# kornelski/cavif-rs

Measured on AMD Instinct MI355X. Metric: MPix/s encoded at speed=4 q=80, 1080p batch; bit-exact vs CPU oracle, higher is better.
Workload: dtype u16 samples / i32 transform / i64 RD cost

## Files before the change

### __graft_entry__.py

```python
import os
import subprocess
import sys

ROOT = os.path.dirname(os.path.abspath(__file__))
sys.path.insert(0, ROOT)

HIPCC_FLAGS = ['--offload-arch=gfx950', '-O2', '-mllvm', '-sink-insts-to-avoid-spills', '-mllvm', '-inline-threshold=1000', '-mllvm', '-disable-machine-licm', '-mllvm', '-phi-node-folding-threshold=1', '-std=c++17', '-ffp-contract=off', '-fPIC', '-shared', '-Wno-unused-variable']


def _digest(sources, flags):
    import hashlib
    h = hashlib.sha256(' '.join(flags).encode())
    for s in sorted(sources):
        with open(s, 'rb') as fh:
            h.update(os.path.basename(s).encode() + b'\0' + fh.read())
    return h.hexdigest()


def _stale(target, sources):
    if not os.path.exists(target):
        return True
    t = os.path.getmtime(target)
    return any(os.path.getmtime(s) > t for s in sources)

# ... 9 lines not shown
        subprocess.check_call([hipcc] + HIPCC_FLAGS + ['-o', out, os.path.join(csrc, 'mi_avif.hip'), '-lz'])
        with open(stamp, 'w') as fh:
            fh.write(want + '\n')
    cli_src = os.path.join(ROOT, 'cavif_rs_amd', 'cli', 'cavif_mi.cpp')
    cli = os.path.join(ROOT, 'cavif_rs_amd', 'cavif_mi')
    if force or _stale(cli, [cli_src, out, os.path.join(ROOT, 'include', 'mi_avif.h')]):
        subprocess.check_call(['g++', '-O2', '-std=c++17', '-o', cli, cli_src, '-L' + os.path.join(ROOT, 'cavif_rs_amd'), '-lmi_avif', '-lpthread', '-Wl,-rpath,$ORIGIN'])
    subprocess.check_call(['make', '-s', '-C', os.path.join(ROOT, 'oracle')])
    try:
        from tests import emu
        emu.build(force=force)
    except Exception as e:
        print('warning: tests/emu build failed (%s); the -m "not gpu" emulator tests will fail, the product library is unaffected' % e, file=sys.stderr)
    try:
        from tests.helpers import k4_harness
        k4_harness.build_all(force=force)
    except Exception as e:
        print('warning: tests/kernels harness build failed (%s); tests/test_k4_coder.py will fail, the product library is unaffected' % e, file=sys.stderr)
    try:
        from tests.helpers import filters_harness
        filters_harness.build_all(force=force)
    except Exception as e:
        print('warning: tests/kernels filter harness build failed (%s); tests/test_loopfilter_kernels.py will fail, the product library is unaffected' % e, file=sys.stderr)
    try:
        from tests.helpers import predict_harness
        predict_harness.build_all(force=force)
    except Exception as e:
        print('warning: tests/kernels prediction harness build failed (%s); tests/test_predict_kernels.py will fail, the product library is unaffected' % e, file=sys.stderr)
    try:
        from tests.helpers import k1_lookups_harness
        k1_lookups_harness.build_all(force=force)
    except Exception as e:
        print('warning: tests/kernels lookup harness build failed (%s); tests/test_k1_lookups.py will fail, the product library is unaffected' % e, file=sys.stderr)
    import cavif_rs_amd
    cavif_rs_amd.load_library()


def smoke():
    import numpy as np
    import cavif_rs_amd as m
    from cavif_rs_amd.synth import synth_image
    from tests.helpers import oracle
    assert m.device_count() >= 1, 'no HIP device visible'
    img = synth_image(256, 192, index=3)
    enc = m.Encoder().with_quality(80).with_speed(4).with_bit_depth(10)
    got = enc.encode_rgb(img)
    ref, cs, _ = oracle.ravif_encode(img, quality=80, speed=4, depth=10)
    assert got.avif_file[4:12] == b'ftypavif'
    assert got.avif_file == ref, 'HIP path and CPU oracle disagree (%d vs %d bytes)' % (len(got.avif_file), len(ref))
    print('smoke ok: %dx%d -> %d bytes (colour %d), identical to the oracle' % (img.shape[1], img.shape[0], len(got.avif_file), got.color_byte_size))


if __name__ == '__main__':
    build(force='--force' in sys.argv)
    if '--smoke' in sys.argv:
        smoke()
```

### cavif_rs_amd/csrc/dev_blk64.h

```cpp
#pragma once

struct Blk64Hbm {
  uint16_t lrec[4][64 * 64]; int32_t lqc[4][32 * 32];
  uint16_t trec[64 * 64]; int32_t tqc[64 * 64];
  uint16_t crec4[4][64 * 64]; int32_t cqc4[4][64 * 64];
  uint16_t crec[2][2][2][64 * 64]; int32_t cqc[2][2][2][4 * 32 * 32];
};
typedef unsigned int v2u_t __attribute__((vector_size(8)));
typedef unsigned int v4u_t __attribute__((vector_size(16)));
#define MI_BLK64_HBM_BYTES ((sizeof(Blk64Hbm) + 255) & ~(size_t)255)

__device__ inline void fwd_txfm64_dev(const LDS uint16_t *src, const LDS uint16_t *pred, LDS int32_t *tbuf, LDS int32_t *coef) {
  constexpr int P = 65;
  {
    const int c = LANE;
    int32_t x[64];
#pragma unroll
    for (int r = 0; r < 64; r++) x[r] = (int)src[r * 64 + c] - (int)pred[r * 64 + c];
    av1_fdct64(x);
#pragma unroll
    for (int r = 0; r < 32; r++) tbuf[r * P + c] = rshift_round_(x[r], 2);
  }
  WAVE_SYNC();
  if (LANE < 32) {
// ... 122 lines not shown
  const int ncand = Tools<TS>::FULL ? 7 : 3;
  auto dl_of = [](int q) { const int a = (q >> 1) + 1; return (q & 1) ? a : -a; };
  const int refine = Tools<TS>::fine_directional(f);
  if (refine) {
#pragma unroll 1
    for (int u = W; u < ncand * 6; u += NW) {
      const int ci = u / 6, q = u - ci * 6, m = SH->order[ci];
      if (m >= V_PRED && m <= D67_PRED) {
        predict_block(f, x, y, log2w, availL, availU, m, dl_of(q), ftype_y, ra, rl, wa, wl, S->etmp, B->pred);
        const long long sd = satd_dev(SH->x64.src64, B->pred, n);
        if (LANE == 0) SH->dsd[ci][q] = sd;
      }
    }
    PH(5);
    WG_SYNC();
    PH(2);
  }
  const bool tx_trial = Tools<TS>::tx_mode_select(f) && Tools<TS>::rdo_tx(f);
  long long my_j = J_INF; int my_e = 1 << 30, my_mode = DC_PRED, my_delta = 0; TxRes my_tr = { 0, 0, 0, 0, 0 };
  uint32_t my_mrate = 0;
#pragma unroll 1
  for (int e = W; e < ncand; e += NW) {
    const int m = SH->order[e];
    const int directional = m >= V_PRED && m <= D67_PRED;
    int delta = 0;
    if (directional && refine) {
      long long bsd = SH->satd[m];
      for (int q = 0; q < 6; q++) { const long long sd = SH->dsd[e][q]; if (sd < bsd) { bsd = sd; delta = dl_of(q); } }
    }
    predict_block(f, x, y, log2w, availL, availU, m, delta, ftype_y, ra, rl, wa, wl, S->etmp, B->pred);
    const uint32_t mode_rate = y_mode_rate(k.cost(), ycost, m, directional, delta);
    TxRes tr;
    fwd_txfm64_dev(SH->x64.src64, B->pred, B->tbuf, B->cbuf);
    const int eob = quant_rate_dev<32>(k.cc(), k.cost(), k.ls(), B->cbuf, B->qc, S->lev, 0, BS, DCT_DCT, f->dc_q[0], f->ac_q[0], f->dc_recip[0], f->ac_recip[0],
                                       f->bd, sctx_y, dctx_y, -1, 0, &tr.rate, &tr.cul, &tr.dcc);
    if (eob > 0) inv_txfm64_add_dev(B->cbuf, B->tbuf, B->pred, f->bd);
    tr.eob = eob;
    if (!Tools<TS>::tune_psnr(f)) tr.sse = psy_dist_wave<64>(SH->x64.src64, B->pred, (const LDS int *)SH->psv, (const LDS int *)SH->pact, f->bd);
    else tr.sse = sse_dev(SH->x64.src64, B->pred, nn);
    long long j = ((tr.sse * f->wq[0]) >> 5) + (((long long)tr.rate * f->rdmult + 256) >> 9);
    j += ((long long)mode_rate * f->rdmult + 256) >> 9;
    if (j < my_j) {
      my_j = j; my_e = e; my_mode = m; my_delta = delta; my_tr = tr; my_mrate = mode_rate;
      for (int i = LANE; i < nn / 4; i += 64) ((v2u_t *)H->lrec[W])[i] = ((const LDS v2u_t *)B->pred)[i];
      for (int i = LANE; i < 256; i += 64) ((v4u_t *)H->lqc[W])[i] = ((const LDS v4u_t *)B->qc)[i];
      WAVE_SYNC();
    }
  }
  if (LANE == 0) { SH->wbest_j[W] = my_j; SH->wbest_e[W] = my_e; }
  PH(6);
  WG_SYNC();
  PH(2);
  int win = 0;
  for (int w2 = 1; w2 < NW; w2++) if (SH->wbest_j[w2] < SH->wbest_j[win] || (SH->wbest_j[w2] == SH->wbest_j[win] && SH->wbest_e[w2] < SH->wbest_e[win])) win = w2;
  const long long best_j = SH->wbest_j[win];
  {
    uint16_t *gr = f->rec[0] + (size_t)y * f->stride + x;
    int32_t *gc = f->coef[0] + (size_t)y * f->stride + x;
    const uint2 *sr = (const uint2 *)H->lrec[win]; const uint4 *sq = (const uint4 *)H->lqc[win];
    for (int u = threadIdx.x; u < nn / 4; u += 64 * NW) *(uint2 *)(gr + (u >> 4) * f->stride + 4 * (u & 15)) = sr[u];
    for (int u = threadIdx.x; u < 256; u += 64 * NW) *(uint4 *)(gc + (u >> 3) * f->stride + 4 * (u & 7)) = sq[u];
  }
  if (W == win) {
    fill_map_dev(f->m_lvl[0], ms, r, c, n4, my_tr.cul);
    fill_map_dev(f->m_dc[0], ms, r, c, n4, my_tr.dcc);
    if (LANE == 0) f->m_eob[0][mi] = (uint16_t)my_tr.eob;
    fill_map_dev(f->m_ymode, ms, r, c, n4, my_mode);
// ... 309 lines not shown
```

### cavif_rs_amd/csrc/dev_common.h

```cpp
#pragma once
#include <hip/hip_runtime.h>
#include <stdint.h>
#include <stddef.h>
#include "av1_tables.h"

#define MI_TX_DEPTH_MAX 2
#define MI_MAX_TILE_COLS 64
#define MI_MAX_TILE_ROWS 64

enum { BS_4 = 0, BS_8 = 1, BS_16 = 2, BS_32 = 3, BS_64 = 4 };
enum { BS_4X8 = 5, BS_8X4 = 6 };
enum { DC_PRED = 0, V_PRED, H_PRED, D45_PRED, D135_PRED, D113_PRED, D157_PRED, D203_PRED, D67_PRED,
       SMOOTH_PRED, SMOOTH_V_PRED, SMOOTH_H_PRED, PAETH_PRED, UV_CFL_PRED };
enum { DCT_DCT = 0, ADST_DCT, DCT_ADST, ADST_ADST, FLIPADST_DCT, DCT_FLIPADST, FLIPADST_FLIPADST,
       ADST_FLIPADST, FLIPADST_ADST, IDTX, V_DCT, H_DCT, V_ADST, H_ADST, V_FLIPADST, H_FLIPADST };
enum { TXC_2D = 0, TXC_HORIZ = 1, TXC_VERT = 2 };

#define MI_SEG_BINS 4096
struct SegTab {
  int n, mean, thr[7], qidx[8], pad_[3];
  struct Q { int dc_q[3], ac_q[3]; uint32_t dc_recip[3], ac_recip[3]; } q[8];
};
struct FrameDev {
  int w, h, bd, np;
// ... 124 lines not shown
  return d;
}

__device__ __forceinline__ uint32_t psy_isqrt46(unsigned long long n, float nf) {
  uint32_t x = (uint32_t)__builtin_amdgcn_sqrtf(nf);
  while ((unsigned long long)x * x > n) x--;
  while ((unsigned long long)(x + 1) * (x + 1) <= n) x++;
  return x;
}
__device__ inline uint32_t psy_boost_q14(uint32_t sv, uint32_t dv) {
  const unsigned long long num = 4033ull * ((unsigned long long)sv + dv + 16384);
  const uint32_t den = psy_isqrt46(16265089ull + (unsigned long long)sv * dv, __builtin_fmaf((float)sv, (float)dv, 16265089.0f));
  const unsigned long long t = num + den / 2;
  const float tf = __builtin_fmaf(4033.0f, (float)sv + (float)dv + 16384.0f, (float)(den >> 1));
  uint32_t q = (uint32_t)(tf * __builtin_amdgcn_rcpf((float)den));
  while ((unsigned long long)q * den > t) q--;
  while ((unsigned long long)(q + 1) * den <= t) q++;
  return q;
}
__device__ __forceinline__ uint32_t psy_cell_var(uint32_t sum, uint32_t sum2, int w, int bd) {
  int v = w == 8 ? (int)sum2 - (int)((sum * sum + 32u) >> 6) : ((int)sum2 - (int)((sum * sum + 8u) >> 4)) << 2;
  if (v < 0) v = 0;
  return (uint32_t)v >> (2 * (bd - 8));
}
__device__ __forceinline__ int psy_cell_dist(uint32_t sse, uint32_t sd, uint32_t qd, uint32_t svar, uint32_t act, int w, int bd) {
  const uint32_t b = psy_boost_q14(svar, psy_cell_var(sd, qd, w, bd));
  unsigned long long d = ((unsigned long long)sse * b + 8192) >> 14;
  d = (d * act + 8192) >> 14;
  return (int)d;
}

template <typename FP> __device__ __forceinline__ long long rd_dist32(FP f, int plane, int sse) { return (long long)(((unsigned long long)(uint32_t)sse * (unsigned long long)f->wq[plane]) >> 5); }
template <typename FP> __device__ __forceinline__ long long rd_rate32(FP f, uint32_t rate) { return (long long)(((unsigned long long)rate * (unsigned long long)f->rdmult + 256) >> 9); }
__device__ __forceinline__ int tx_set_of(int txs, int reduced) { return txs >= 3 ? 0 : (reduced ? 2 : (txs == 2 ? 2 : 1)); }
__device__ __forceinline__ int tx_set_count(int set) { return set == 0 ? 1 : (set == 1 ? 7 : 5); }
__device__ __forceinline__ int sym_to_txtype(int set, int s) {
  if (set == 0) return DCT_DCT;
  if (set == 1) return lut4(0x213ba09ULL, s);
  return lut4(0x21309ULL, s);
}
__device__ __forceinline__ int txtype_to_sym(int set, int t) {
  const unsigned long long inv12 = set == 1 ? 0xffff320fffff4651ULL : 0xffffff0fffff2431ULL, inv = set == 0 ? 0xfffffffffffffff0ULL : inv12;
  const int s = lut4(inv, t);
  return s == 15 ? -1 : s;
}
__device__ __forceinline__ int mode_to_txtype(int m) {
  return lut4(0x3213122130210ULL, m);
}
__device__ __forceinline__ int tx_class_of(int t) {
  if (t == V_DCT || t == V_ADST || t == V_FLIPADST) return TXC_VERT;
  if (t == H_DCT || t == H_ADST || t == H_FLIPADST) return TXC_HORIZ;
  return TXC_2D;
}
#define SCAN_LDS_ENTRIES(maxn) ((maxn) >= 32 ? 1360 : 336)
__device__ inline void load_scans_to_lds(LDS uint16_t *ls, int maxn) {
  for (int i = LANE; i < 16; i += 64) ls[i] = av1_default_scan_4x4[i];
  for (int i = LANE; i < 64; i += 64) ls[16 + i] = av1_default_scan_8x8[i];
  for (int i = LANE; i < 256; i += 64) ls[80 + i] = av1_default_scan_16x16[i];
  if (maxn >= 32) for (int i = LANE; i < 1024; i += 64) ls[336 + i] = av1_default_scan_32x32[i];
}
__device__ __forceinline__ int scan_pos(const LDS uint16_t *ls, int n, int cls, int i) {
  if (cls == TXC_2D) return ls[(n == 4 ? 0 : n == 8 ? 16 : n == 16 ? 80 : 336) + i];
  if (cls == TXC_VERT) return i;
  const int c = i / n, r = i - c * n; return r * n + c;
}
static __device__ const uint8_t rect_scan_4x8[32] = { 0, 1, 4, 2, 5, 8, 3, 6, 9, 12, 7, 10, 13, 16, 11, 14, 17, 20, 15, 18, 21, 24, 19, 22, 25, 28, 23, 26, 29, 27, 30, 31 };
static __device__ const uint8_t rect_scan_8x4[32] = { 0, 8, 1, 16, 9, 2, 24, 17, 10, 3, 25, 18, 11, 4, 26, 19, 12, 5, 27, 20, 13, 6, 28, 21, 14, 7, 29, 22, 15, 30, 23, 31 };
__device__ __forceinline__ int rect_scan_pos(int wl, int hl, int cls, int i) {
  const int w = 1 << wl, h = 1 << hl;
  if (cls == TXC_2D) return hl > wl ? rect_scan_4x8[i] : rect_scan_8x4[i];
  if (cls == TXC_VERT) return i;
  const int c = i / h, r = i - c * h; return r * w + c;
}
template <typename FP> __device__ __forceinline__ int intra_tx_cdf_r(FP f, bool reduced, int txs, int ymode, int *nsyms, int *set_out) {
  const int set = tx_set_of(txs, reduced);
  *set_out = set;
  if (set == 0 || f->base_q_idx == 0) { *nsyms = 0; return -1; }
  if (set == 1) { *nsyms = 7; return CDF_INTRA_TX1 + (txs * 13 + ymode) * CDF_INTRA_TX1_STRIDE; }
  *nsyms = 5; return CDF_INTRA_TX2 + (txs * 13 + ymode) * CDF_INTRA_TX2_STRIDE;
}
template <typename FP> __device__ __forceinline__ int intra_tx_cdf(FP f, int txs, int ymode, int *nsyms, int *set_out) { return intra_tx_cdf_r(f, f->reduced_tx_set != 0, txs, ymode, nsyms, set_out); }
template <typename FP> __device__ __forceinline__ int rect_tx_cdf(FP f, bool reduced, int ymode, int *nsyms, int *set_out) {
  const int set = reduced ? 2 : 1;
  *set_out = set;
  if (f->base_q_idx == 0) { *nsyms = 0; return -1; }
  if (set == 1) { *nsyms = 7; return CDF_INTRA_TX1 + ymode * CDF_INTRA_TX1_STRIDE; }
  *nsyms = 5; return CDF_INTRA_TX2 + ymode * CDF_INTRA_TX2_STRIDE;
}
```

### cavif_rs_amd/csrc/dev_group.h

```cpp
#pragma once
#include "dev_predict.h"
#include "dev_txfm.h"
#include "dev_rate.h"

struct GroupBuf8 {
  int32_t tbuf[8 * 9];
  int32_t cbuf[64];
  int32_t qc[64];
  uint16_t rec[64];
  uint8_t lev[144];
};
#define GROUP_LANE (LANE & 15)
#define GROUP_ID (LANE >> 4)

template <int CTRL> __device__ __forceinline__ int dpp_row_(int v) { return __builtin_amdgcn_update_dpp(0, v, CTRL, 0xF, 0xF, false); }
__device__ __forceinline__ int row_sum_i32(int v) { v += dpp_row_<0x128>(v); v += dpp_row_<0x124>(v); v += dpp_row_<0x122>(v); v += dpp_row_<0x121>(v); return v; }
__device__ __forceinline__ int row_max_i32(int v) {
  v = imax_(v, dpp_row_<0x128>(v)); v = imax_(v, dpp_row_<0x124>(v)); v = imax_(v, dpp_row_<0x122>(v)); v = imax_(v, dpp_row_<0x121>(v)); return v;
}

static __device__ const int tx4_tab[2][3][4][8] = {
  { { { 2896, 2896, 2896, 2896, 0, 0, 0, 0 }, { 3784, 1567, -1567, -3784, 0, 0, 0, 0 }, { 2896, -2896, -2896, 2896, 0, 0, 0, 0 }, { 1567, -3784, 3784, -1567, 0, 0, 0, 0 } },
    { { 1321, 2482, 3344, 3803, 0, 0, 0, 0 }, { 3344, 3344, 0, -3344, 0, 0, 0, 0 }, { 3803, -1321, -3344, 2482, 0, 0, 0, 0 }, { 2482, -3803, 3344, -1321, 0, 0, 0, 0 } },
    { { 5793, 0, 0, 0, 0, 0, 0, 0 }, { 0, 5793, 0, 0, 0, 0, 0, 0 }, { 0, 0, 5793, 0, 0, 0, 0, 0 }, { 0, 0, 0, 5793, 0, 0, 0, 0 } } },
  { { { 2896, 0, 2896, 0, 0, 3784, 0, 1567 }, { 2896, 0, -2896, 0, 0, 1567, 0, -3784 }, { 2896, 0, -2896, 0, 0, 1567, 0, -3784 }, { 2896, 0, 2896, 0, 0, 3784, 0, 1567 } },
    { { 1321, 3344, 3803, 2482, 0, 0, 0, 0 }, { 2482, 3344, -1321, -3803, 0, 0, 0, 0 }, { 3344, 0, -3344, 3344, 0, 0, 0, 0 }, { 3803, -3344, 2482, -1321, 0, 0, 0, 0 } },
    { { 5793, 0, 0, 0, 0, 0, 0, 0 }, { 0, 5793, 0, 0, 0, 0, 0, 0 }, { 0, 0, 5793, 0, 0, 0, 0, 0 }, { 0, 0, 0, 5793, 0, 0, 0, 0 } } } };
__device__ __forceinline__ int tx4_dot(int v, const int *m) {
  int acc = __mul24(m[0], dpp_row_<0x00>(v)) + 2048;
  acc += __mul24(m[1], dpp_row_<0x55>(v));
  acc += __mul24(m[2], dpp_row_<0xAA>(v));
  acc += __mul24(m[3], dpp_row_<0xFF>(v));
  return acc >> 12;
}
__device__ __forceinline__ int tx4_fwd(int v, int kind) { return tx4_dot(v, tx4_tab[0][kind][LANE & 3]); }
__device__ __forceinline__ int tx4_inv(int v, int kind) {
  const int *m = tx4_tab[1][kind][LANE & 3];
  const int e = tx4_dot(v, m), o = tx4_dot(v, m + 4);
  return (LANE & 2) ? e - o : e + o;
}
__device__ __forceinline__ int group_transpose4(int v) { return __shfl(v, (LANE & 48) | ((LANE & 3) << 2) | ((LANE >> 2) & 3)); }

struct GroupRes { int eob, cul, dcc, sse; uint32_t rate; };

template <int CTRL> __device__ __forceinline__ int dpp_row_z(int v) { return __builtin_amdgcn_update_dpp(0, v, CTRL, 0xF, 0xF, false); }
template <typename FP>
__device__ __forceinline__ void eval_group4_tail(const CoefCost &cc, FP f, LDS GroupBuf8 *gb, int coef, int t_src, int t_rec, int tidx, int plane, int txs, int txtype, int ck, int rk,
                                                 int skip_ctx, int dc_ctx, int tx_off, uint32_t tx_cost, int psy_sv, int psy_act, GroupRes *res) {
  constexpr int N = 4, nc = 16;
  const int gl = GROUP_LANE, row = gl >> 2, col = gl & 3, bd = f->bd;
  const int dcq = f->dc_q[plane], acq = f->ac_q[plane];
  const uint32_t dc_recip = f->dc_recip[plane], ac_recip = f->ac_recip[plane];
  const int cls = tx_class_of(txtype), pt = plane > 0, txs_ctx = txs;
  const uint32_t dc_off = (uint32_t)(dcq * 109 / 256), off0 = (uint32_t)(acq * 98 / 256), off1 = (uint32_t)(acq * 109 / 256), off_eob = (uint32_t)(acq * 88 / 256);
  const uint32_t thr = (uint32_t)acq - off_eob, uq = (uint32_t)acq;
  const int c = cls == TXC_2D ? lut4(0xFEA9DB83C7426510ULL, gl) : (cls == TXC_VERT ? gl : col * 4 + row);
  const uint32_t mag = (uint32_t)iabs_(coef); const int neg = coef < 0;
  const int last = row_max_i32((c >= 1 && mag >= thr) ? c + 1 : 0);
  int l0 = 0;
  if (gl == 0) {
    const uint32_t x0 = mag + dc_off;
    uint32_t l0u = __umulhi(x0, dc_recip);
    if (x0 - l0u * (uint32_t)dcq >= (uint32_t)dcq) l0u++;
    l0 = (int)l0u;
  }
  l0 = row_max_i32(l0);
  int eob = last;
  if (eob == 0) eob = l0 ? 1 : 0;
  int lv = 0;
  if (c < eob) {
    if (c == 0) lv = l0;
    else {
      uint32_t lv0 = __umulhi(mag, ac_recip);
      if (mag - lv0 * uq >= uq) lv0++;
      const uint32_t off = lv0 > 0 ? off1 : off0;
      lv = (int)lv0 + ((mag + off) >= (lv0 + 1) * uq);
    }
  }
  gb->qc[gl] = neg ? -lv : lv;
  int dq;
  {
    const int dmx = (1 << (7 + bd)) - 1, dmn = -(1 << (7 + bd));
    uint32_t m = (uint32_t)lv * (uint32_t)(gl == 0 ? dcq : acq);
    m &= 0xFFFFFF;
    const int v = neg ? -(int)m : (int)m;
    dq = v < dmn ? dmn : (v > dmx ? dmx : v);
  }
  const int l15 = imin_(lv, 15);
  const int s1 = dpp_row_z<0x101>(l15), s2 = dpp_row_z<0x102>(l15), s3 = dpp_row_z<0x103>(l15), s5 = dpp_row_z<0x105>(l15);
  const int b1 = dpp_row_z<0x104>(l15), b2 = dpp_row_z<0x108>(l15), b3 = dpp_row_z<0x10C>(l15);
  const int r1 = col < 3 ? s1 : 0, r2 = col < 2 ? s2 : 0, r3 = col < 1 ? s3 : 0, d1 = col < 3 ? s5 : 0;
  uint32_t head = cc.txb[(txs_ctx * 13 + skip_ctx) * CDF_TXB_SKIP_STRIDE + (eob == 0)];
  int bits = 0, cul = 0, dcc = 0;
  if (eob > 0) {
    if (tx_off >= 0) head += tx_cost;
    const int eob_pt = eob_to_pt(eob);
    head += cc.eobpt[0][(pt * 2 + (cls == TXC_2D ? 0 : 1)) * CDF_EOB_PT_16_STRIDE + eob_pt - 1];
    if (eob_pt >= 3) {
      const int nb = eob_pt - 2, rem = eob - ((1 << (eob_pt - 2)) + 1), hi = (rem >> (nb - 1)) & 1;
      head += cc.eobx[((txs_ctx * 2 + pt) * 9 + (eob_pt - 3)) * CDF_EOB_EXTRA_STRIDE + hi];
      head += 512u * (uint32_t)(nb - 1);
    }
    if (c < eob) {
      const int level = lv;
      if (c == eob - 1) {
        const int ctx = c == 0 ? 0 : (c <= nc / 8 ? 1 : (c <= nc / 4 ? 2 : 3));
        bits += cc.beob[((txs_ctx * 2 + pt) * 4 + ctx) * CDF_COEFF_BASE_EOB_STRIDE + imin_(level, 3) - 1];
      } else {
        int mag2 = imin_(r1, 3) + imin_(b1, 3), ctx;
        if (cls == TXC_2D) {
          mag2 += imin_(d1, 3) + imin_(r2, 3) + imin_(b2, 3);
          const int m = imin_((mag2 + 1) >> 1, 4);
          ctx = (row == 0 && col == 0) ? 0 : (row + col < 2 ? m + 1 : (row + col < 4 ? m + 6 : m + 21));
        } else if (cls == TXC_VERT) {
          mag2 += imin_(b2, 3) + imin_(b3, 3);
          const int m = imin_((mag2 + 1) >> 1, 4);
          ctx = m + (row == 0 ? 26 : (row == 1 ? 31 : 36));
        } else {
          mag2 += imin_(r2, 3) + imin_(r3, 3);
          const int m = imin_((mag2 + 1) >> 1, 4);
          ctx = m + (col == 0 ? 26 : (col == 1 ? 31 : 36));
        }
        bits += cc.base[((txs_ctx * 2 + pt) * 42 + ctx) * CDF_COEFF_BASE_STRIDE + imin_(level, 3)];
      }
      if (level > 2) {
        int mg = r1 + b1, ctx;
        if (cls == TXC_2D) { mg = imin_((mg + d1 + 1) >> 1, 6); ctx = c == 0 ? mg : ((row < 2 && col < 2) ? mg + 7 : mg + 14); }
        else if (cls == TXC_HORIZ) { mg = imin_((mg + r2 + 1) >> 1, 6); ctx = c == 0 ? mg : (col == 0 ? mg + 7 : mg + 14); }
        else { mg = imin_((mg + b2 + 1) >> 1, 6); ctx = c == 0 ? mg : (row == 0 ? mg + 7 : mg + 14); }
        const int off = ((imin_(txs_ctx, 3) * 2 + pt) * 21 + ctx) * CDF_COEFF_BR_STRIDE;
        int rem = level - 3;
        for (int idx = 0; idx < 4; idx++) { const int s2 = imin_(rem, 3); bits += cc.br[off + s2]; rem -= s2; if (s2 < 3) break; }
      }
      if (level) {
        if (c == 0) { bits += cc.dcs[(pt * 3 + dc_ctx) * CDF_DC_SIGN_STRIDE + neg]; dcc = neg ? 1 : 2; }
        else bits += 512;
        if (level > 14) { const int len = 32 - __clz(level - 14); bits += 512 * (2 * len - 1); }
      }
      cul += level;
    }
  }
  bits = row_sum_i32(bits);
  const int cd = row_sum_i32(imin_(cul, 63) | (dcc << 16));
  res->eob = eob; res->cul = imin_(cd & 0xFFFF, 63); res->dcc = cd >> 16; res->rate = head + (uint32_t)bits;
  if (eob > 0) {
    const int cbits = imax_(bd + 6, 16), cmax = (1 << (cbits - 1)) - 1, cmin = -(1 << (cbits - 1));
    int v = iclamp_(tx4_inv(dq, rk), cmin, cmax);
    v = group_transpose4(v);
    t_rec = iclamp_(t_rec + round2_(tx4_inv(v, ck), 4), 0, (1 << bd) - 1);
  }
  gb->rec[tidx] = (uint16_t)t_rec;
  WAVE_SYNC();
  const int d = t_src - t_rec;
  const int s = row_sum_i32(__mul24(d, d));
  if (psy_sv >= 0) { const int sd = row_sum_i32(t_rec), qd = row_sum_i32(__mul24(t_rec, t_rec)); res->sse = psy_cell_dist((uint32_t)s, (uint32_t)sd, (uint32_t)qd, (uint32_t)psy_sv, (uint32_t)psy_act, 4, bd); }
  else res->sse = (int)(((unsigned long long)(uint32_t)s * (uint32_t)psy_act + 8192) >> 14);
}

template <int N, typename CostPtr>
__device__ inline void eval_group(const CoefCost &cc, CostPtr cost, const LDS uint16_t *ls, const LDS FrameDev *f, LDS GroupBuf8 *gb,
                                  const LDS uint16_t *src, const LDS uint16_t *pred, int plane, int txs, int txtype,
                                  int skip_ctx, int dc_ctx, int tx_off, int tx_sym, int psy_sv, int psy_act, GroupRes *res) {
  constexpr int P = N + 1, nc = N * N, IT = nc / 16, bwl = N == 4 ? 2 : 3, st = N + 4;
  const int gl = GROUP_LANE;
  const int bd = f->bd;
  const uint32_t tx_cost = cost[tx_off >= 0 ? tx_off + tx_sym : 0];
  int ck, rk; tx_kinds(txtype, &ck, &rk);
  [[maybe_unused]] int t_src = 0, t_rec = 0;
  [[maybe_unused]] const int tidx = ((gl & 3) << 2) | (gl >> 2);
  if constexpr (N == 4) {
    t_src = src[tidx]; t_rec = pred[tidx];
    int v = tx4_fwd((int)((uint32_t)(t_src - t_rec) << 2), ck);
    v = group_transpose4(v);
    const int coef = tx4_fwd(v, rk);
    eval_group4_tail(cc, f, gb, coef, t_src, t_rec, tidx, plane, txs, txtype, ck, rk, skip_ctx, dc_ctx, tx_off, tx_cost, psy_sv, psy_act, res);
    return;
  } else {
#pragma unroll
  for (int k = 0; k < IT; k++) {
    const int idx = gl + 16 * k, i = idx / N, j = idx % N;
    const int pv = pred[idx];
    gb->tbuf[i * P + j] = (int)src[idx] - pv;
    gb->rec[idx] = (uint16_t)pv;
  }
  for (int i = gl; i < 36; i += 16) ((LDS uint32_t *)gb->lev)[i] = 0;
  WAVE_SYNC();
  if (gl < N) {
    int32_t x[N];
#pragma unroll
    for (int r = 0; r < N; r++) x[r] = (int32_t)((uint32_t)gb->tbuf[r * P + gl] << 2);
    tx1d<N>(x, ck, true);
#pragma unroll
    for (int r = 0; r < N; r++) gb->tbuf[r * P + gl] = N == 8 ? rshift_round_(x[r], 1) : x[r];
  }
  WAVE_SYNC();
  if (gl < N) {
    int32_t x[N];
#pragma unroll
    for (int c = 0; c < N; c++) x[c] = gb->tbuf[gl * P + c];
    tx1d<N>(x, rk, true);
#pragma unroll
    for (int c = 0; c < N; c++) gb->cbuf[gl * N + c] = x[c];
  }
  WAVE_SYNC();
  }
  const int dcq = f->dc_q[plane], acq = f->ac_q[plane];
  const uint32_t dc_recip = f->dc_recip[plane], ac_recip = f->ac_recip[plane];
  const int cls = tx_class_of(txtype), pt = plane > 0, txs_ctx = txs;
  const uint32_t dc_off = (uint32_t)(dcq * 109 / 256), off0 = (uint32_t)(acq * 98 / 256), off1 = (uint32_t)(acq * 109 / 256), off_eob = (uint32_t)(acq * 88 / 256);
  const uint32_t thr = (uint32_t)acq - off_eob, uq = (uint32_t)acq;
  int pos[IT]; uint32_t mag[IT]; int neg[IT];
  int last = 0;
#pragma unroll
  for (int k = 0; k < IT; k++) {
    const int i = gl + 16 * k;
    pos[k] = scan_pos(ls, N, cls, i);
    const int c = gb->cbuf[pos[k]];
    mag[k] = (uint32_t)iabs_(c); neg[k] = c < 0;
    if (i >= 1 && mag[k] >= thr) last = i + 1;
  }
  last = row_max_i32(last);
  const uint32_t x0 = (uint32_t)iabs_(gb->cbuf[0]) + dc_off;
  uint32_t l0u = __umulhi(x0, dc_recip);
  if (x0 - l0u * (uint32_t)dcq >= (uint32_t)dcq) l0u++;
  const int l0 = (int)l0u;
  int eob = last;
  if (eob == 0) eob = l0 ? 1 : 0;
  const int dmx = (1 << (7 + bd)) - 1, dmn = -(1 << (7 + bd));
  int lvl[IT];
  WAVE_SYNC();
#pragma unroll
  for (int k = 0; k < IT; k++) {
    const int i = gl + 16 * k;
    int lv = 0;
    if (i < eob) {
      if (i == 0) lv = l0;
      else {
        const uint32_t a = mag[k];
        uint32_t lv0 = __umulhi(a, ac_recip);
        if (a - lv0 * uq >= uq) lv0++;
        const uint32_t off = lv0 > 0 ? off1 : off0;
        lv = (int)lv0 + ((a + off) >= (lv0 + 1) * uq);
      }
    }
    lvl[k] = lv;
    const int pp = pos[k];
    gb->qc[pp] = neg[k] ? -lv : lv;
    gb->lev[(pp >> bwl) * st + (pp & (N - 1))] = (uint8_t)imin_(lv, 127);
    uint32_t m = (uint32_t)lv * (uint32_t)(pp == 0 ? dcq : acq);
    m &= 0xFFFFFF;
    const int v = neg[k] ? -(int)m : (int)m;
    gb->cbuf[pp] = v < dmn ? dmn : (v > dmx ? dmx : v);
  }
  WAVE_SYNC();
  uint32_t head = cc.txb[(txs_ctx * 13 + skip_ctx) * CDF_TXB_SKIP_STRIDE + (eob == 0)];
  int bits = 0, cul = 0, dcc = 0;
  if (eob > 0) {
    if (tx_off >= 0) head += tx_cost;
    const int eob_pt = eob_to_pt(eob);
    head += cc.eobpt[N == 4 ? 0 : 1][(pt * 2 + (cls == TXC_2D ? 0 : 1)) * (N == 4 ? CDF_EOB_PT_16_STRIDE : CDF_EOB_PT_64_STRIDE) + eob_pt - 1];
    if (eob_pt >= 3) {
      const int nb = eob_pt - 2, rem = eob - ((1 << (eob_pt - 2)) + 1), hi = (rem >> (nb - 1)) & 1;
      head += cc.eobx[((txs_ctx * 2 + pt) * 9 + (eob_pt - 3)) * CDF_EOB_EXTRA_STRIDE + hi];
      head += 512u * (uint32_t)(nb - 1);
    }
#pragma unroll
    for (int k = 0; k < IT; k++) {
      const int c = gl + 16 * k;
      if (c < eob) {
        const int pp = pos[k], row = pp >> bwl, col = pp & (N - 1), level = lvl[k];
        const LDS uint8_t *L = gb->lev + row * st + col;
        if (c == eob - 1) {
          const int ctx = c == 0 ? 0 : (c <= nc / 8 ? 1 : (c <= nc / 4 ? 2 : 3));
          bits += cc.beob[((txs_ctx * 2 + pt) * 4 + ctx) * CDF_COEFF_BASE_EOB_STRIDE + imin_(level, 3) - 1];
        } else {
          const int ctx = base_ctx(L, st, cls, row, col);
          bits += cc.base[((txs_ctx * 2 + pt) * 42 + ctx) * CDF_COEFF_BASE_STRIDE + imin_(level, 3)];
        }
        if (level > 2) {
          const int ctx = br_ctx(L, st, cls, row, col, c);
          const int off = ((imin_(txs_ctx, 3) * 2 + pt) * 21 + ctx) * CDF_COEFF_BR_STRIDE;
          int rem = level - 3;
          for (int idx = 0; idx < 4; idx++) { const int s2 = imin_(rem, 3); bits += cc.br[off + s2]; rem -= s2; if (s2 < 3) break; }
        }
        if (level) {
          if (c == 0) { bits += cc.dcs[(pt * 3 + dc_ctx) * CDF_DC_SIGN_STRIDE + neg[k]]; dcc = neg[k] ? 1 : 2; }
          else bits += 512;
          if (level > 14) { const int len = 32 - __clz(level - 14); bits += 512 * (2 * len - 1); }
        }
        cul += level;
      }
    }
  }
  bits = row_sum_i32(bits);
  const int cd = row_sum_i32(imin_(cul, 63) | (dcc << 16));
  res->eob = eob; res->cul = imin_(cd & 0xFFFF, 63); res->dcc = cd >> 16; res->rate = head + (uint32_t)bits;
  {
    constexpr int ROWSH = N == 4 ? 0 : 1;
    const int cbits = imax_(bd + 6, 16), cmax = (1 << (cbits - 1)) - 1, cmin = -(1 << (cbits - 1));
    if constexpr (N == 4) {
      if (eob > 0) {
        int v = iclamp_(tx4_inv(gb->cbuf[gl], rk), cmin, cmax);
        v = group_transpose4(v);
        t_rec = iclamp_(t_rec + round2_(tx4_inv(v, ck), 4), 0, (1 << bd) - 1);
        gb->rec[tidx] = (uint16_t)t_rec;
      }
      WAVE_SYNC();
    } else {
      const bool act = gl < N && eob > 0;
      if (act) {
        int32_t x[N];
  #pragma unroll
        for (int j = 0; j < N; j++) x[j] = gb->cbuf[gl * N + j];
        tx1d<N>(x, rk, false);
  #pragma unroll
        for (int j = 0; j < N; j++) gb->tbuf[gl * P + j] = iclamp_(round2_(x[j], ROWSH), cmin, cmax);
      }
      WAVE_SYNC();
      const int mx = (1 << bd) - 1;
      if (act) {
        int32_t x[N];
  #pragma unroll
        for (int i = 0; i < N; i++) x[i] = gb->tbuf[i * P + gl];
        tx1d<N>(x, ck, false);
  #pragma unroll
        for (int i = 0; i < N; i++) gb->rec[i * N + gl] = (uint16_t)iclamp_((int)gb->rec[i * N + gl] + round2_(x[i], 4), 0, mx);
      }
      WAVE_SYNC();
    }
  }
  int s = 0, sd = 0, qd = 0;
  if constexpr (N == 4) { const int d = t_src - t_rec; s = __mul24(d, d); sd = t_rec; qd = __mul24(t_rec, t_rec); }
  else
#pragma unroll
  for (int k = 0; k < IT; k++) { const int idx = gl + 16 * k; const int rv = gb->rec[idx], d = (int)src[idx] - rv; s += __mul24(d, d); sd += rv; qd += __mul24(rv, rv); }
  s = row_sum_i32(s);
  if (psy_sv >= 0) { sd = row_sum_i32(sd); qd = row_sum_i32(qd); res->sse = psy_cell_dist((uint32_t)s, (uint32_t)sd, (uint32_t)qd, (uint32_t)psy_sv, (uint32_t)psy_act, N == 4 ? 4 : 8, bd); }
  else res->sse = (int)(((unsigned long long)(uint32_t)s * (uint32_t)psy_act + 8192) >> 14);
}

struct GroupPredBuf { uint16_t wa[48], wl[48], tmp[32], pred[64]; };

__device__ __forceinline__ void edge_filter_group(LDS uint16_t *buf, int sz, int strength, LDS uint16_t *tmp, int gl) {
  if (strength) for (int i = gl; i < sz; i += 16) tmp[i] = buf[i - 1];
  WAVE_SYNC();
  if (strength) for (int i = 1 + gl; i < sz; i += 16) {
    int s = 0;
#pragma unroll
    for (int j = 0; j < 5; j++) {
      const int k = iclamp_(i - 2 + j, 0, sz - 1);
      const int kw = strength == 1 ? (j == 0 || j == 4 ? 0 : (j == 2 ? 8 : 4)) : (strength == 2 ? (j == 0 || j == 4 ? 0 : (j == 2 ? 6 : 5)) : (j == 0 || j == 4 ? 2 : 4));
      s += kw * tmp[k];
    }
    buf[i - 1] = (uint16_t)((s + 8) >> 4);
  }
  WAVE_SYNC();
}
__device__ __forceinline__ void edge_upsample_group(LDS uint16_t *buf, int num_px, int on, int bd, LDS uint16_t *tmp, int gl) {
  if (on) for (int i = gl; i < num_px + 3; i += 16) {
    uint16_t v;
    if (i == 0) v = buf[-1]; else if (i == num_px + 2) v = buf[num_px - 1]; else v = buf[i - 2];
    tmp[i] = v;
  }
  WAVE_SYNC();
  const int mx = (1 << bd) - 1;
  if (on) {
    if (gl == 0) buf[-2] = tmp[0];
    for (int i = gl; i < num_px; i += 16) {
      int s = -(int)tmp[i] + 9 * (int)tmp[i + 1] + 9 * (int)tmp[i + 2] - (int)tmp[i + 3];
      s = iclamp_(round2_(s, 4), 0, mx);
      buf[2 * i - 1] = (uint16_t)s;
// ... 121 lines not shown
```

### cavif_rs_amd/csrc/dev_rate.h

```cpp
#pragma once
#include "dev_common.h"

template <typename FP, typename TP> __device__ inline void txb_ctx_dev(FP f, TP t, int plane, int r4, int c4, int txs, int bs, int *skip_ctx, int *dc_ctx) {
  const int w4 = 1 << txs, ms = f->mi_stride;
  int top = 0, left = 0, dcs = 0, any_a = 0, any_l = 0;
  const int k = LANE;
  if (k < w4) {
    const bool ha = r4 - 1 >= t->mi_row_start && c4 + k < f->mi_cols, hl = c4 - 1 >= t->mi_col_start && r4 + k < f->mi_rows;
    const int ia = ha ? (r4 - 1) * ms + c4 + k : r4 * ms + c4, il = hl ? (r4 + k) * ms + c4 - 1 : r4 * ms + c4;
    const int la = f->m_lvl[plane][ia], da = f->m_dc[plane][ia], ll = f->m_lvl[plane][il], dl = f->m_dc[plane][il];
    if (ha) { top = la; any_a = la | da; dcs += da == 1 ? -1 : (da == 2 ? 1 : 0); }
    if (hl) { left = ll; any_l = ll | dl; dcs += dl == 1 ? -1 : (dl == 2 ? 1 : 0); }
  }
  top = wave_max_i32(top); left = wave_max_i32(left); dcs = wave_sum_i32(dcs);
  any_a = wave_or_i32(any_a); any_l = wave_or_i32(any_l);
  *dc_ctx = dcs < 0 ? 1 : (dcs > 0 ? 2 : 0);
  if (plane == 0) {
    int ctx;
    if (bs == txs) ctx = 0;
    else if (top == 0 && left == 0) ctx = 1;
    else if (top == 0 || left == 0) ctx = 2 + (imax_(top, left) > 3);
    else if (imax_(top, left) <= 3) ctx = 4;
    else if (imin_(top, left) <= 3) ctx = 5;
    else ctx = 6;
    *skip_ctx = ctx;
  } else {
    *skip_ctx = 7 + (any_a != 0) + (any_l != 0) + (bs > txs ? 3 : 0);
  }
}
template <typename FP, typename TP> __device__ inline void txb_ctx_wh(FP f, TP t, int plane, int r4, int c4, int w4, int h4, int whole, int *skip_ctx, int *dc_ctx) {
  const int ms = f->mi_stride;
  int top = 0, left = 0, dcs = 0, any_a = 0, any_l = 0;
  const int k = LANE;
  if (k < imax_(w4, h4)) {
// ... 20 lines not shown

__device__ __forceinline__ int eob_to_pt(int eob) { return eob < 3 ? eob : (32 - __clz(eob - 1) + 1); }
__device__ __forceinline__ int eob_pt_cdf(int eob_multi, int pt, int cls) {
  const int off[7] = { CDF_EOB_PT_16, CDF_EOB_PT_32, CDF_EOB_PT_64, CDF_EOB_PT_128, CDF_EOB_PT_256, CDF_EOB_PT_512, CDF_EOB_PT_1024 };
  const int str[7] = { CDF_EOB_PT_16_STRIDE, CDF_EOB_PT_32_STRIDE, CDF_EOB_PT_64_STRIDE, CDF_EOB_PT_128_STRIDE,
                       CDF_EOB_PT_256_STRIDE, CDF_EOB_PT_512_STRIDE, CDF_EOB_PT_1024_STRIDE };
  return off[eob_multi] + (pt * 2 + (cls == TXC_2D ? 0 : 1)) * str[eob_multi];
}
__device__ __forceinline__ int base_ctx(const LDS uint8_t *L, int st, int cls, int row, int col) {
  int mag = imin_(L[1], 3) + imin_(L[st], 3);
  if (cls == TXC_2D) {
    mag += imin_(L[st + 1], 3) + imin_(L[2], 3) + imin_(L[2 * st], 3);
    const int m = imin_((mag + 1) >> 1, 4);
    if (row == 0 && col == 0) return 0;
    if (row + col < 2) return m + 1;
    if (row + col < 4) return m + 6;
    return m + 21;
  } else if (cls == TXC_VERT) {
    mag += imin_(L[2 * st], 3) + imin_(L[3 * st], 3) + imin_(L[4 * st], 3);
    const int m = imin_((mag + 1) >> 1, 4);
    return m + (row == 0 ? 26 : (row == 1 ? 31 : 36));
  }
  mag += imin_(L[2], 3) + imin_(L[3], 3) + imin_(L[4], 3);
  const int m = imin_((mag + 1) >> 1, 4);
  return m + (col == 0 ? 26 : (col == 1 ? 31 : 36));
}
__device__ __forceinline__ int br_ctx(const LDS uint8_t *L, int st, int cls, int row, int col, int c) {
  int mag = imin_(L[1], 15) + imin_(L[st], 15);
  if (cls == TXC_2D) { mag += imin_(L[st + 1], 15); mag = imin_((mag + 1) >> 1, 6); return c == 0 ? mag : ((row < 2 && col < 2) ? mag + 7 : mag + 14); }
  if (cls == TXC_HORIZ) { mag += imin_(L[2], 15); mag = imin_((mag + 1) >> 1, 6); return c == 0 ? mag : (col == 0 ? mag + 7 : mag + 14); }
  mag += imin_(L[2 * st], 15); mag = imin_((mag + 1) >> 1, 6); return c == 0 ? mag : (row == 0 ? mag + 7 : mag + 14);
}

__device__ inline void build_level_map(const LDS int32_t *qc, LDS uint8_t *lev, int n) {
  const int st = n + 4, words = (st * st + 3) >> 2, bwl = n == 4 ? 2 : n == 8 ? 3 : n == 16 ? 4 : 5;
  LDS uint32_t *lw = (LDS uint32_t *)lev;
  for (int i = LANE; i < words; i += 64) lw[i] = 0;
  WAVE_SYNC();
  for (int i = LANE; i < n * n; i += 64) lev[(i >> bwl) * st + (i & (n - 1))] = (uint8_t)imin_(iabs_(qc[i]), 127);
  WAVE_SYNC();
}

struct CoefCost { const LDS uint16_t *txb, *eobx, *dcs, *br, *base, *beob, *eobpt[4]; };
__device__ __forceinline__ int coef_cost_entries(int maxtxs) {
  const int t = maxtxs + 1, tb = imin_(maxtxs, 3) + 1;
  return t * 13 * CDF_TXB_SKIP_STRIDE + t * 18 * CDF_EOB_EXTRA_STRIDE + 6 * CDF_DC_SIGN_STRIDE + tb * 42 * CDF_COEFF_BR_STRIDE +
         t * 84 * CDF_COEFF_BASE_STRIDE + t * 8 * CDF_COEFF_BASE_EOB_STRIDE + 4 * (CDF_EOB_PT_16_STRIDE + CDF_EOB_PT_64_STRIDE + CDF_EOB_PT_256_STRIDE + CDF_EOB_PT_1024_STRIDE);
}
#define COEF_COST_MAX_ENTRIES(maxtxs) (((maxtxs) + 1) * (13 * 3 + 18 * 3 + 84 * 5 + 8 * 4) + 18 + ((maxtxs) < 3 ? (maxtxs) + 1 : 4) * 42 * 5 + 4 * (6 + 8 + 10 + 12))
__device__ __forceinline__ CoefCost coef_cost_layout(const LDS uint16_t *dst, int maxtxs, int *src_off = nullptr, int *count = nullptr) {
  const int t = maxtxs + 1, tb = imin_(maxtxs, 3) + 1;
  const int src[10] = { CDF_TXB_SKIP, CDF_EOB_EXTRA, CDF_DC_SIGN, CDF_COEFF_BR, CDF_COEFF_BASE, CDF_COEFF_BASE_EOB, CDF_EOB_PT_16, CDF_EOB_PT_64, CDF_EOB_PT_256, CDF_EOB_PT_1024 };
  const int cnt[10] = { t * 13 * CDF_TXB_SKIP_STRIDE, t * 18 * CDF_EOB_EXTRA_STRIDE, 6 * CDF_DC_SIGN_STRIDE, tb * 42 * CDF_COEFF_BR_STRIDE, t * 84 * CDF_COEFF_BASE_STRIDE,
                        t * 8 * CDF_COEFF_BASE_EOB_STRIDE, 4 * CDF_EOB_PT_16_STRIDE, 4 * CDF_EOB_PT_64_STRIDE, 4 * CDF_EOB_PT_256_STRIDE, 4 * CDF_EOB_PT_1024_STRIDE };
  int o[10]; int acc = 0;
#pragma unroll
  for (int i = 0; i < 10; i++) { o[i] = acc; acc += cnt[i]; if (src_off) src_off[i] = src[i]; if (count) count[i] = cnt[i]; }
  CoefCost cc;
  cc.txb = dst + o[0]; cc.eobx = dst + o[1]; cc.dcs = dst + o[2]; cc.br = dst + o[3]; cc.base = dst + o[4]; cc.beob = dst + o[5];
  cc.eobpt[0] = dst + o[6]; cc.eobpt[1] = dst + o[7]; cc.eobpt[2] = dst + o[8]; cc.eobpt[3] = dst + o[9];
  return cc;
}
__device__ inline void load_coef_cost(LDS uint16_t *dst, const uint16_t *cost, int maxtxs, int tid, int nthreads) {
  int src[10], cnt[10];
  coef_cost_layout(dst, maxtxs, src, cnt);
  int o = 0;
  for (int k = 0; k < 10; k++) { for (int i = tid; i < cnt[k]; i += nthreads) dst[o + i] = cost[src[k] + i]; o += cnt[k]; }
}

template <typename CostPtr> __device__ inline uint32_t coef_rate_dev(const CoefCost &cc, CostPtr cost, const LDS uint16_t *ls, const LDS int32_t *qc, int eob, int plane, int txs, int txtype,
                                         int skip_ctx, int dc_ctx, int tx_off, int tx_sym, LDS uint8_t *lev, int *cul_out, int *dc_cat) {
  const int n = imin_(32, 4 << txs), bwl = n == 4 ? 2 : n == 8 ? 3 : n == 16 ? 4 : 5;
  const int pt = plane > 0, cls = tx_class_of(txtype), txs_ctx = txs;
  *cul_out = 0; *dc_cat = 0;
  uint32_t head = cc.txb[(txs_ctx * 13 + skip_ctx) * CDF_TXB_SKIP_STRIDE + (eob == 0)];
  if (eob == 0) return head;
  if (tx_off >= 0) head += cost[tx_off + tx_sym];
  const int eob_pt = eob_to_pt(eob), eob_multi = 2 * bwl - 4;
  {
    static_assert(CDF_EOB_PT_16_STRIDE == 6 && CDF_EOB_PT_64_STRIDE == 8 && CDF_EOB_PT_256_STRIDE == 10 && CDF_EOB_PT_1024_STRIDE == 12, "stride = 6 + 2 sq");
    const int sq = eob_multi >> 1;
    head += cc.eobpt[sq][(pt * 2 + (cls == TXC_2D ? 0 : 1)) * (6 + 2 * sq) + eob_pt - 1];
  }
  if (eob_pt >= 3) {
    const int nb = eob_pt - 2, rem = eob - ((1 << (eob_pt - 2)) + 1), hi = (rem >> (nb - 1)) & 1;
    head += cc.eobx[((txs_ctx * 2 + pt) * 9 + (eob_pt - 3)) * CDF_EOB_EXTRA_STRIDE + hi];
    head += 512u * (uint32_t)(nb - 1);
  }
  build_level_map(qc, lev, n);
  const int st = n + 4, area = n * n;
  int bits = 0; int cul = 0, dcc = 0;
  for (int c = LANE; c < eob; c += 64) {
    const int p = scan_pos(ls, n, cls, c), row = p >> bwl, col = p & (n - 1);
    const int v = qc[p], level = iabs_(v);
    const LDS uint8_t *L = lev + row * st + col;
    if (c == eob - 1) {
      const int ctx = c == 0 ? 0 : (c <= area / 8 ? 1 : (c <= area / 4 ? 2 : 3));
      bits += cc.beob[((txs_ctx * 2 + pt) * 4 + ctx) * CDF_COEFF_BASE_EOB_STRIDE + imin_(level, 3) - 1];
    } else {
      const int ctx = base_ctx(L, st, cls, row, col);
      bits += cc.base[((txs_ctx * 2 + pt) * 42 + ctx) * CDF_COEFF_BASE_STRIDE + imin_(level, 3)];
    }
    if (level > 2) {
      const int ctx = br_ctx(L, st, cls, row, col, c);
      const int off = ((imin_(txs_ctx, 3) * 2 + pt) * 21 + ctx) * CDF_COEFF_BR_STRIDE;
      int rem = level - 3;
      for (int idx = 0; idx < 4; idx++) { const int s = imin_(rem, 3); bits += cc.br[off + s]; rem -= s; if (s < 3) break; }
    }
    if (level) {
      if (c == 0) { bits += cc.dcs[(pt * 3 + dc_ctx) * CDF_DC_SIGN_STRIDE + (v < 0)]; dcc = v < 0 ? 1 : 2; }
      else bits += 512;
      if (level > 14) { const int len = 32 - __clz(level - 14); bits += 512 * (2 * len - 1); }
    }
    cul += level;
  }
  bits = wave_sum_i32(bits);
  cul = wave_sum_i32(imin_(cul, 1 << 20));
  dcc = __builtin_amdgcn_readfirstlane(dcc);
  *cul_out = imin_(cul, 63); *dc_cat = dcc;
  return head + (uint32_t)bits;
}

#define LEV_OFF(cs) ((cs) == 4 ? 0 : (cs) == 8 ? 64 : (cs) == 16 ? 64 + 144 : 64 + 144 + 400)
#define LEV_BYTES(maxcs) ((maxcs) == 4 ? 64 : (maxcs) == 8 ? 64 + 144 : (maxcs) == 16 ? 64 + 144 + 400 : 64 + 144 + 400 + 1296)

template <int CS, typename CostPtr>
__device__ inline int quant_rate_dev(const CoefCost &cc, CostPtr cost, const LDS uint16_t *ls, LDS int32_t *cbuf, LDS int32_t *qc, LDS uint8_t *levbase,
                                     int plane, int txs, int txtype, int dcq, int acq, uint32_t dc_recip, uint32_t ac_recip, int bd,
                                     int skip_ctx, int dc_ctx, int tx_off, int tx_sym, uint32_t *rate_out, int *cul_out, int *dc_cat) {
  constexpr int n = CS, nc = CS * CS, IT = nc < 64 ? 1 : nc / 64, bwl = CS == 4 ? 2 : CS == 8 ? 3 : CS == 16 ? 4 : 5, st = CS + 4;
  LDS uint8_t *lev = levbase + LEV_OFF(CS);
  const uint32_t tx_cost = cost[tx_off >= 0 ? tx_off + tx_sym : 0];
  const int cls = tx_class_of(txtype), pt = plane > 0, txs_ctx = txs;
  const int lsh = txs == 3 ? 1 : (txs == 4 ? 2 : 0);
  const uint32_t dc_off = (uint32_t)(dcq * 109 / 256), off0 = (uint32_t)(acq * 98 / 256), off1 = (uint32_t)(acq * 109 / 256), off_eob = (uint32_t)(acq * 88 / 256);
  const uint32_t thr = (uint32_t)acq - off_eob, uq = (uint32_t)acq;
  int pos[IT]; uint32_t mag[IT]; int neg[IT];
  int last = 0;
#pragma unroll
  for (int k = 0; k < IT; k++) {
    const int i = LANE + 64 * k;
    const bool valid = nc >= 64 || i < nc;
    pos[k] = valid ? scan_pos(ls, n, cls, i) : 0;
    const int c = valid ? cbuf[pos[k]] : 0;
    mag[k] = (uint32_t)iabs_(c) << lsh; neg[k] = c < 0;
    if (valid && i >= 1 && mag[k] >= thr) last = i + 1;
  }
  last = wave_max_i32(last);
  const uint32_t x0 = ((uint32_t)iabs_(cbuf[0]) << lsh) + dc_off;
  uint32_t l0u = __umulhi(x0, dc_recip);
  if (x0 - l0u * (uint32_t)dcq >= (uint32_t)dcq) l0u++;
  const int l0 = (int)l0u;
  int eob = last;
  if (eob == 0) eob = l0 ? 1 : 0;
  const int sh = lsh, dmx = (1 << (7 + bd)) - 1, dmn = -(1 << (7 + bd));
  int lvl[IT];
  WAVE_SYNC();
#pragma unroll
  for (int k = 0; k < IT; k++) {
    const int i = LANE + 64 * k;
    const bool valid = nc >= 64 || i < nc;
    int lv = 0;
    if (valid && i < eob) {
      if (i == 0) lv = l0;
      else {
        const uint32_t a = mag[k];
        uint32_t lv0 = __umulhi(a, ac_recip);
        if (a - lv0 * uq >= uq) lv0++;
        const uint32_t off = lv0 > 0 ? off1 : off0;
        lv = (int)lv0 + ((a + off) >= (lv0 + 1) * uq);
      }
    }
    lvl[k] = lv;
    if (valid) {
      const int pp = pos[k];
      qc[pp] = neg[k] ? -lv : lv;
      lev[(pp >> bwl) * st + (pp & (n - 1))] = (uint8_t)imin_(lv, 127);
      uint32_t m = (uint32_t)lv * (uint32_t)(pp == 0 ? dcq : acq);
      m &= 0xFFFFFF; m >>= sh;
      const int v = neg[k] ? -(int)m : (int)m;
      cbuf[pp] = v < dmn ? dmn : (v > dmx ? dmx : v);
    }
  }
  WAVE_SYNC();
  *cul_out = 0; *dc_cat = 0;
  uint32_t head = cc.txb[(txs_ctx * 13 + skip_ctx) * CDF_TXB_SKIP_STRIDE + (eob == 0)];
  if (eob == 0) { *rate_out = head; return 0; }
  if (tx_off >= 0) head += tx_cost;
  const int eob_pt = eob_to_pt(eob), eob_multi = 2 * bwl - 4;
  {
    static_assert(CDF_EOB_PT_16_STRIDE == 6 && CDF_EOB_PT_64_STRIDE == 8 && CDF_EOB_PT_256_STRIDE == 10 && CDF_EOB_PT_1024_STRIDE == 12, "stride = 6 + 2 sq");
    const int sq = eob_multi >> 1;
    head += cc.eobpt[sq][(pt * 2 + (cls == TXC_2D ? 0 : 1)) * (6 + 2 * sq) + eob_pt - 1];
  }
  if (eob_pt >= 3) {
    const int nb = eob_pt - 2, rem = eob - ((1 << (eob_pt - 2)) + 1), hi = (rem >> (nb - 1)) & 1;
    head += cc.eobx[((txs_ctx * 2 + pt) * 9 + (eob_pt - 3)) * CDF_EOB_EXTRA_STRIDE + hi];
    head += 512u * (uint32_t)(nb - 1);
  }
  constexpr int area = nc;
  int bits = 0, cul = 0, dcc = 0;
#pragma unroll
  for (int k = 0; k < IT; k++) {
    const int c = LANE + 64 * k;
    if (c < eob) {
      const int pp = pos[k], row = pp >> bwl, col = pp & (n - 1), level = lvl[k];
      const LDS uint8_t *L = lev + row * st + col;
      if (c == eob - 1) {
        const int ctx = c == 0 ? 0 : (c <= area / 8 ? 1 : (c <= area / 4 ? 2 : 3));
        bits += cc.beob[((txs_ctx * 2 + pt) * 4 + ctx) * CDF_COEFF_BASE_EOB_STRIDE + imin_(level, 3) - 1];
      } else {
        const int ctx = base_ctx(L, st, cls, row, col);
        bits += cc.base[((txs_ctx * 2 + pt) * 42 + ctx) * CDF_COEFF_BASE_STRIDE + imin_(level, 3)];
      }
      if (level > 2) {
        const int ctx = br_ctx(L, st, cls, row, col, c);
        const int off = ((imin_(txs_ctx, 3) * 2 + pt) * 21 + ctx) * CDF_COEFF_BR_STRIDE;
        int rem = level - 3;
        for (int idx = 0; idx < 4; idx++) { const int s2 = imin_(rem, 3); bits += cc.br[off + s2]; rem -= s2; if (s2 < 3) break; }
      }
      if (level) {
        if (c == 0) { bits += cc.dcs[(pt * 3 + dc_ctx) * CDF_DC_SIGN_STRIDE + neg[k]]; dcc = neg[k] ? 1 : 2; }
        else bits += 512;
        if (level > 14) { const int len = 32 - __clz(level - 14); bits += 512 * (2 * len - 1); }
      }
      cul += level;
    }
  }
  bits = wave_sum_i32(bits);
  cul = wave_sum_i32(imin_(cul, 1 << 20));
  dcc = __builtin_amdgcn_readfirstlane(dcc);
  *cul_out = imin_(cul, 63); *dc_cat = dcc;
  *rate_out = head + (uint32_t)bits;
  return eob;
}
```

### cavif_rs_amd/csrc/dev_rect.h

```cpp
#pragma once

__device__ inline void load_edges_wh(const LDS FrameDev *f, int plane, int x, int y, int w, int h, int have_left, int have_above, int have_ar, int have_bl,
                                     LDS uint16_t *above, LDS uint16_t *left) {
  const int bd = f->bd, rs = f->stride, tot = w + h;
  const uint16_t *rec = f->rec[plane];
  const int max_x = f->mi_cols * 4 - 1, max_y = f->mi_rows * 4 - 1;
  const int lim_a = imin_(max_x, x + (have_ar ? 2 * w : w) - 1), lim_l = imin_(max_y, y + (have_bl ? 2 * h : h) - 1);
  for (int i = LANE; i <= tot; i += 64) {
    const bool corner = i == tot;
    int ia, il;
    if (have_above) ia = (y - 1) * rs + (corner ? (have_left ? x - 1 : x) : imin_(lim_a, x + i));
    else ia = y * rs + (have_left ? x - 1 : x);
    if (have_left) il = imin_(lim_l, y + i) * rs + x - 1;
    else il = (have_above ? y - 1 : y) * rs + x;
    uint16_t a = rec[ia], l = rec[il];
    if (!have_above && !have_left) { a = (uint16_t)(corner ? (1 << (bd - 1)) : (1 << (bd - 1)) - 1); l = (uint16_t)((1 << (bd - 1)) + 1); }
    if (corner) { above[-1] = a; left[-1] = a; } else { above[i] = a; left[i] = l; }
  }
  WAVE_SYNC();
}

__device__ inline void predict_block_wh(const LDS FrameDev *f, int x, int y, int wl, int hl, int have_left, int have_above, int mode, int angle_delta, int ftype,
                                        const LDS uint16_t *ra, const LDS uint16_t *rl, LDS uint16_t *wa, LDS uint16_t *wl_, LDS uint16_t *tmp, LDS uint16_t *pred) {
  const int w = 1 << wl, h = 1 << hl, bd = f->bd, nn = w * h;
// ... 155 lines not shown
  WAVE_SYNC();
  int lv = 0;
  if (valid && i < eob) {
    if (i == 0) lv = l0;
    else {
      uint32_t lv0 = __umulhi(mag, ac_recip);
      if (mag - lv0 * uq >= uq) lv0++;
      const uint32_t off = lv0 > 0 ? off1 : off0;
      lv = (int)lv0 + ((mag + off) >= (lv0 + 1) * uq);
    }
  }
  for (int q = LANE; q < st * (h + 4); q += 64) lev[q] = 0;
  WAVE_SYNC();
  const int dmx = (1 << (7 + bd)) - 1, dmn = -(1 << (7 + bd));
  if (valid) {
    qc[pos] = neg ? -lv : lv;
    lev[(pos >> wl) * st + (pos & (w - 1))] = (uint8_t)imin_(lv, 127);
    uint32_t m = (uint32_t)lv * (uint32_t)(pos == 0 ? dcq : acq);
    m &= 0xFFFFFF;
    const int v = neg ? -(int)m : (int)m;
    cbuf[pos] = v < dmn ? dmn : (v > dmx ? dmx : v);
  }
  WAVE_SYNC();
  *cul_out = 0; *dc_cat = 0;
  uint32_t head = cost[CDF_TXB_SKIP + (txs_ctx * 13 + skip_ctx) * CDF_TXB_SKIP_STRIDE + (eob == 0)];
  if (eob == 0) { *rate_out = head; for (int q = LANE; q < st * (h + 4); q += 64) lev[q] = 0; WAVE_SYNC(); return 0; }
  if (tx_off >= 0) head += cost[tx_off + tx_sym];
  const int eob_pt = eob_to_pt(eob);
  head += cost[eob_pt_cdf(1, pt, cls) + eob_pt - 1];
  if (eob_pt >= 3) {
    const int nb = eob_pt - 2, rem = eob - ((1 << (eob_pt - 2)) + 1), hi = (rem >> (nb - 1)) & 1;
    head += cost[CDF_EOB_EXTRA + ((txs_ctx * 2 + pt) * 9 + (eob_pt - 3)) * CDF_EOB_EXTRA_STRIDE + hi] + 512u * (uint32_t)(nb - 1);
  }
  uint32_t mine = 0;
  if (valid && i < eob) {
    const int row = pos >> wl, col = pos & (w - 1), level = lv;
    const LDS uint8_t *L = lev + row * st + col;
    if (i == eob - 1) {
      const int ctx = i == 0 ? 0 : (i <= nc / 8 ? 1 : (i <= nc / 4 ? 2 : 3));
      mine += cost[CDF_COEFF_BASE_EOB + ((txs_ctx * 2 + pt) * 4 + ctx) * CDF_COEFF_BASE_EOB_STRIDE + imin_(level, 3) - 1];
    } else {
      int ctx = base_ctx(L, st, cls, row, col);
      if (cls == TXC_2D && !(row == 0 && col == 0)) {
        int mg = imin_(L[1], 3) + imin_(L[st], 3) + imin_(L[st + 1], 3) + imin_(L[2], 3) + imin_(L[2 * st], 3);
        const int m = imin_((mg + 1) >> 1, 4);
        if (hl > wl) ctx = m + (row < 2 ? 11 : (row + col < 4 ? 6 : 21));
        else ctx = m + (col < 2 ? 16 : (row + col < 4 ? 6 : 21));
      }
      mine += cost[CDF_COEFF_BASE + ((txs_ctx * 2 + pt) * 42 + ctx) * CDF_COEFF_BASE_STRIDE + imin_(level, 3)];
    }
    if (level > 2) {
      const int off = CDF_COEFF_BR + ((txs_ctx * 2 + pt) * 21 + br_ctx(L, st, cls, row, col, i)) * CDF_COEFF_BR_STRIDE;
      int rem = level - 3;
      for (int idx = 0; idx < 4; idx++) { const int s = imin_(rem, 3); mine += cost[off + s]; rem -= s; if (s < 3) break; }
    }
    if (level) {
      if (i == 0) mine += cost[CDF_DC_SIGN + (pt * 3 + dc_ctx) * CDF_DC_SIGN_STRIDE + neg];
      else mine += 512u;
      if (level > 14) { const uint32_t xg = (uint32_t)(level - 14); const int len = 32 - __clz(xg); mine += 512u * (uint32_t)(2 * len - 1); }
    }
  }
  const int cul = imin_(wave_sum_i32((valid && i < eob) ? lv : 0), 63);
  const int dcneg = __builtin_amdgcn_readlane(neg, 0), dclv = __builtin_amdgcn_readlane(lv, 0);
  *cul_out = cul; *dc_cat = dclv ? (dcneg ? 1 : 2) : 0;
  *rate_out = head + (uint32_t)wave_sum_i32((int)mine);
  for (int q = LANE; q < st * (h + 4); q += 64) lev[q] = 0;
  WAVE_SYNC();
  return eob;
}

template <int MAXN, int WL, int HL, int NW, int TS>
__device__ inline long long eval_rect(const Ctx<MAXN, NW, TS> k, int plane, int sctx, int dctx, const LDS uint16_t *src, const LDS uint16_t *pred, int txtype, int tx_off, int tx_sym,
                                      LDS uint16_t *rec_out, LDS int32_t *qc_out, TxRes *tr, int psv_a, int psv_b, int act) {
  constexpr int W = 1 << WL, H = 1 << HL, P = W + 1, NN = W * H;
  const LDS FrameDev *f = k.f(); LDS WaveScratch<MAXN> *S = k.s();
  for (int idx = LANE; idx < NN; idx += 64) { S->tbuf[(idx >> WL) * P + (idx & (W - 1))] = (int)src[idx] - (int)pred[idx]; rec_out[idx] = pred[idx]; }
  WAVE_SYNC();
  fwd_txfm_rect<W, H>(S->tbuf, S->cbuf, txtype);
  const int eob = rect_quant_rate(k.cost(), S->cbuf, qc_out, S->lev, plane, WL, HL, txtype, f->dc_q[plane], f->ac_q[plane], f->dc_recip[plane], f->ac_recip[plane], f->bd,
                                  sctx, dctx, tx_off, tx_sym, &tr->rate, &tr->cul, &tr->dcc);
  if (eob > 0) inv_txfm_rect_add<W, H>(S->cbuf, S->tbuf, rec_out, txtype, f->bd);
  tr->eob = eob;
  int sd[2] = { 0, 0 }, qd[2] = { 0, 0 }, se[2] = { 0, 0 };
  if (LANE < NN) {
    const int i = LANE >> WL, j = LANE & (W - 1), cell = W == 8 ? (j >> 2) : (i >> 2);
    const int d = rec_out[LANE], e = (int)src[LANE] - d;
    sd[cell] = d; qd[cell] = d * d; se[cell] = e * e;
  }
  long long dist;
  if (plane == 0 && !Tools<TS>::tune_psnr(f)) {
    dist = 0;
#pragma unroll
    for (int cell = 0; cell < 2; cell++) {
      const uint32_t s1 = (uint32_t)wave_sum_i32(sd[cell]), s2 = (uint32_t)wave_sum_i32(qd[cell]), s3 = (uint32_t)wave_sum_i32(se[cell]);
      dist += psy_cell_dist(s3, s1, s2, (uint32_t)(cell ? psv_b : psv_a), (uint32_t)act, 4, f->bd);
    }
  } else {
    const long long e = (long long)wave_sum_i32(se[0] + se[1]);
    dist = plane == 0 ? e : (e * act + 8192) >> 14;
  }
  tr->sse = dist;
  return ((dist * f->wq[plane]) >> 5) + (((long long)tr->rate * f->rdmult + 256) >> 9);
}

template <int WL, int HL, typename CostPtr>
__device__ inline void eval_group_wh(const CoefCost &cc, CostPtr cost, const LDS FrameDev *f, LDS GroupBuf8 *gb, const LDS uint16_t *src, const LDS uint16_t *pred, int plane, int txtype,
                                     int skip_ctx, int dc_ctx, int tx_off, int tx_sym, int psv_a, int psv_b, int psy_act, GroupRes *res) {
  constexpr int W = 1 << WL, H = 1 << HL, P = W + 1, nc = 32, IT = 2, st = W + 4, txs_ctx = 1;
  const int gl = GROUP_LANE, bd = f->bd;
  const int cls = tx_class_of(txtype), pt = plane > 0;
  const uint32_t tx_cost = cost[tx_off >= 0 ? tx_off + tx_sym : 0];
  const uint32_t ep_cost = cost[eob_pt_cdf(1, pt, cls) + imin_(gl, 5)];
#pragma unroll
  for (int k = 0; k < IT; k++) {
    const int idx = gl + 16 * k, i = idx >> WL, j = idx & (W - 1);
    const int pv = pred[idx];
    gb->tbuf[i * P + j] = (int)src[idx] - pv;
    gb->rec[idx] = (uint16_t)pv;
  }
  for (int i = gl; i < (st * (H + 4) + 3) / 4; i += 16) ((LDS uint32_t *)gb->lev)[i] = 0;
  WAVE_SYNC();
  int ck, rk; tx_kinds(txtype, &ck, &rk);
  if (gl < W) {
    int32_t x[H];
#pragma unroll
    for (int r = 0; r < H; r++) x[r] = (int32_t)((uint32_t)gb->tbuf[r * P + gl] << 2);
    tx1d<H>(x, ck, true);
#pragma unroll
    for (int r = 0; r < H; r++) gb->tbuf[r * P + gl] = rshift_round_(x[r], 1);
  }
  WAVE_SYNC();
  if (gl < H) {
    int32_t x[W];
#pragma unroll
    for (int c = 0; c < W; c++) x[c] = gb->tbuf[gl * P + c];
    tx1d<W>(x, rk, true);
#pragma unroll
    for (int c = 0; c < W; c++) gb->cbuf[gl * W + c] = (int32_t)(((long long)x[c] * 5793 + 2048) >> 12);
  }
  WAVE_SYNC();
  const int dcq = f->dc_q[plane], acq = f->ac_q[plane];
  const uint32_t dc_recip = f->dc_recip[plane], ac_recip = f->ac_recip[plane];
  const uint32_t dc_off = (uint32_t)(dcq * 109 / 256), off0 = (uint32_t)(acq * 98 / 256), off1 = (uint32_t)(acq * 109 / 256), off_eob = (uint32_t)(acq * 88 / 256);
  const uint32_t thr = (uint32_t)acq - off_eob, uq = (uint32_t)acq;
  int pos[IT]; uint32_t mag[IT]; int neg[IT];
  int last = 0;
#pragma unroll
  for (int k = 0; k < IT; k++) {
    const int i = gl + 16 * k;
    pos[k] = rect_scan_pos(WL, HL, cls, i);
    const int c = gb->cbuf[pos[k]];
    mag[k] = (uint32_t)iabs_(c); neg[k] = c < 0;
    if (i >= 1 && mag[k] >= thr) last = i + 1;
  }
  last = row_max_i32(last);
  const uint32_t x0 = (uint32_t)iabs_(gb->cbuf[0]) + dc_off;
  uint32_t l0u = __umulhi(x0, dc_recip);
  if (x0 - l0u * (uint32_t)dcq >= (uint32_t)dcq) l0u++;
  const int l0 = (int)l0u;
  int eob = last;
  if (eob == 0) eob = l0 ? 1 : 0;
  const int dmx = (1 << (7 + bd)) - 1, dmn = -(1 << (7 + bd));
  int lvl[IT];
  WAVE_SYNC();
#pragma unroll
  for (int k = 0; k < IT; k++) {
    const int i = gl + 16 * k;
    int lv = 0;
    if (i < eob) {
      if (i == 0) lv = l0;
      else {
        const uint32_t a = mag[k];
        uint32_t lv0 = __umulhi(a, ac_recip);
        if (a - lv0 * uq >= uq) lv0++;
        const uint32_t off = lv0 > 0 ? off1 : off0;
        lv = (int)lv0 + ((a + off) >= (lv0 + 1) * uq);
      }
    }
    lvl[k] = lv;
    const int pp = pos[k];
    gb->qc[pp] = neg[k] ? -lv : lv;
    gb->lev[(pp >> WL) * st + (pp & (W - 1))] = (uint8_t)imin_(lv, 127);
    uint32_t m = (uint32_t)lv * (uint32_t)(pp == 0 ? dcq : acq);
    m &= 0xFFFFFF;
    const int v = neg[k] ? -(int)m : (int)m;
    gb->cbuf[pp] = v < dmn ? dmn : (v > dmx ? dmx : v);
  }
  WAVE_SYNC();
  uint32_t head = cc.txb[(txs_ctx * 13 + skip_ctx) * CDF_TXB_SKIP_STRIDE + (eob == 0)];
  int bits = 0, cul = 0, dcc = 0;
  const int eob_pt = eob_to_pt(imax_(eob, 1));
  const uint32_t ep = (uint32_t)__shfl((int)ep_cost, (LANE & 48) + eob_pt - 1);
  if (eob > 0) {
    if (tx_off >= 0) head += tx_cost;
    head += ep;
    if (eob_pt >= 3) {
      const int nb = eob_pt - 2, rem = eob - ((1 << (eob_pt - 2)) + 1), hi = (rem >> (nb - 1)) & 1;
      head += cc.eobx[((txs_ctx * 2 + pt) * 9 + (eob_pt - 3)) * CDF_EOB_EXTRA_STRIDE + hi];
      head += 512u * (uint32_t)(nb - 1);
    }
#pragma unroll
    for (int k = 0; k < IT; k++) {
      const int c = gl + 16 * k;
      if (c < eob) {
        const int pp = pos[k], row = pp >> WL, col = pp & (W - 1), level = lvl[k];
        const LDS uint8_t *L = gb->lev + row * st + col;
        if (c == eob - 1) {
          const int ctx = c == 0 ? 0 : (c <= nc / 8 ? 1 : (c <= nc / 4 ? 2 : 3));
          bits += cc.beob[((txs_ctx * 2 + pt) * 4 + ctx) * CDF_COEFF_BASE_EOB_STRIDE + imin_(level, 3) - 1];
        } else {
          int ctx = base_ctx(L, st, cls, row, col);
          if (cls == TXC_2D && !(row == 0 && col == 0)) {
            const int mg = imin_(L[1], 3) + imin_(L[st], 3) + imin_(L[st + 1], 3) + imin_(L[2], 3) + imin_(L[2 * st], 3), m = imin_((mg + 1) >> 1, 4);
            ctx = HL > WL ? m + (row < 2 ? 11 : (row + col < 4 ? 6 : 21)) : m + (col < 2 ? 16 : (row + col < 4 ? 6 : 21));
          }
          bits += cc.base[((txs_ctx * 2 + pt) * 42 + ctx) * CDF_COEFF_BASE_STRIDE + imin_(level, 3)];
        }
        if (level > 2) {
          const int off = ((txs_ctx * 2 + pt) * 21 + br_ctx(L, st, cls, row, col, c)) * CDF_COEFF_BR_STRIDE;
          int rem = level - 3;
          for (int idx = 0; idx < 4; idx++) { const int s2 = imin_(rem, 3); bits += cc.br[off + s2]; rem -= s2; if (s2 < 3) break; }
        }
        if (level) {
          if (c == 0) { bits += cc.dcs[(pt * 3 + dc_ctx) * CDF_DC_SIGN_STRIDE + neg[k]]; dcc = neg[k] ? 1 : 2; }
          else bits += 512;
          if (level > 14) { const int len = 32 - __clz(level - 14); bits += 512 * (2 * len - 1); }
        }
        cul += level;
      }
    }
  }
  bits = row_sum_i32(bits);
  cul = row_sum_i32(imin_(cul, 1 << 20));
  dcc = row_max_i32(dcc);
  res->eob = eob; res->cul = imin_(cul, 63); res->dcc = dcc; res->rate = head + (uint32_t)bits;
  {
    const int cbits = imax_(bd + 6, 16), cmax = (1 << (cbits - 1)) - 1, cmin = -(1 << (cbits - 1));
    const bool act_r = gl < H && eob > 0, act_c = gl < W && eob > 0;
    if (act_r) {
      int32_t x[W];
#pragma unroll
      for (int j = 0; j < W; j++) x[j] = round2_(gb->cbuf[gl * W + j] * 2896, 12);
      tx1d<W>(x, rk, false);
#pragma unroll
      for (int j = 0; j < W; j++) gb->tbuf[gl * P + j] = iclamp_(x[j], cmin, cmax);
    }
    WAVE_SYNC();
    const int mx = (1 << bd) - 1;
    if (act_c) {
      int32_t x[H];
#pragma unroll
      for (int i = 0; i < H; i++) x[i] = gb->tbuf[i * P + gl];
      tx1d<H>(x, ck, false);
#pragma unroll
      for (int i = 0; i < H; i++) gb->rec[i * W + gl] = (uint16_t)iclamp_((int)gb->rec[i * W + gl] + round2_(x[i], 4), 0, mx);
    }
    WAVE_SYNC();
  }
  int se[2] = { 0, 0 }, sd[2] = { 0, 0 }, qd[2] = { 0, 0 };
#pragma unroll
  for (int k = 0; k < IT; k++) {
    const int idx = gl + 16 * k, i = idx >> WL, j = idx & (W - 1), cell = W == 8 ? (j >> 2) : (i >> 2);
    const int rv = gb->rec[idx], d = (int)src[idx] - rv;
    se[cell] += __mul24(d, d); sd[cell] += rv; qd[cell] += __mul24(rv, rv);
  }
  if (psv_a >= 0) {
    int dist = 0;
#pragma unroll
    for (int cell = 0; cell < 2; cell++)
      dist += psy_cell_dist((uint32_t)row_sum_i32(se[cell]), (uint32_t)row_sum_i32(sd[cell]), (uint32_t)row_sum_i32(qd[cell]), (uint32_t)(cell ? psv_b : psv_a), (uint32_t)psy_act, 4, bd);
    res->sse = dist;
  } else res->sse = (int)(((unsigned long long)(uint32_t)row_sum_i32(se[0] + se[1]) * (uint32_t)psy_act + 8192) >> 14);
}

template <int WL, int HL> __device__ inline void commit_rect(const LDS FrameDev *f, int plane, int r, int c, const LDS uint16_t *rec, const LDS int32_t *qc, int eob, int cul, int dcc) {
  constexpr int W = 1 << WL, H = 1 << HL;
  uint16_t *gr = f->rec[plane] + (size_t)(r * 4) * f->stride + c * 4;
  int32_t *gc = f->coef[plane] + (size_t)(r * 4) * f->stride + c * 4;
  for (int idx = LANE; idx < W * H; idx += 64) { gr[(idx >> WL) * f->stride + (idx & (W - 1))] = rec[idx]; gc[(idx >> WL) * f->stride + (idx & (W - 1))] = qc[idx]; }
  if (LANE < 2) { const int rr = r + (H == 8 ? LANE : 0), cc = c + (W == 8 ? LANE : 0); f->m_lvl[plane][rr * f->mi_stride + cc] = (uint8_t)cul; f->m_dc[plane][rr * f->mi_stride + cc] = (uint8_t)dcc; }
  if (LANE == 0) f->m_eob[plane][r * f->mi_stride + c] = (uint16_t)eob;
}
template <int WL, int HL> __device__ __forceinline__ void fill_rect(uint8_t *m, int ms, int r, int c, int v) {
  if (LANE < 2) m[(r + (HL == 3 ? LANE : 0)) * ms + c + (WL == 3 ? LANE : 0)] = (uint8_t)v;
}

template <int MAXN, int BSR, int NW, int TS>
__device__ MI_K1_TRY_ATTR long long try_block_rect(const Ctx<MAXN, NW, TS> k, int r, int c, long long budget = J_INF) {
  static_assert(NW == 4 && MAXN <= 32, "the 2:1 block search deals its candidates to four wavefronts (its chroma stages hard-code the wave roles; no one-candidate-per-wave fallback is left)");
  constexpr int WL = BSR == BS_4X8 ? 2 : 3, HL = BSR == BS_4X8 ? 3 : 2, W_ = 1 << WL, H_ = 1 << HL, NN = W_ * H_, w4 = W_ >> 2, h4 = H_ >> 2;
  const LDS FrameDev *f = k.f(); const LDS TileB *t = k.t(); LDS WaveScratch<MAXN> *S = k.s(); LDS SharedScratch<MAXN> *SH = k.sh();
  const int W = NW > 1 ? WAVE_ID : 0;
  const int ms = f->mi_stride, mi = r * ms + c, x = c * 4, y = r * 4;
  const int availU = r > t->mi_row_start, availL = c > t->mi_col_start;
  const int can_ar = availU && (c + w4 < t->mi_col_end), can_bl = availL && (r + h4 < t->mi_row_end);
  const int iU = availU ? mi - ms : mi, iL = availL ? mi - 1 : mi;
  constexpr int SHAPE = BSR == BS_8X4 ? 1 : 2;
  const int have_ar = can_ar && decoded_before(r, c, SHAPE, r - 1, c + w4), have_bl = can_bl && decoded_before(r, c, SHAPE, r + h4, c - 1);
  const int amode = availU ? uni32(f->m_ymode[iU]) : DC_PRED, lmode = availL ? uni32(f->m_ymode[iL]) : DC_PRED;
  const int uvU = f->np > 1 ? uni32(f->m_uvmode[iU]) : 0, uvL = f->np > 1 ? uni32(f->m_uvmode[iL]) : 0;
  const int v_skU = f->m_skip[iU], v_skL = f->m_skip[iL], v_skUL = f->m_skip[availU && availL ? mi - ms - 1 : mi];
  const int nb_skip = (availU ? uni32(v_skU) & 1 : 0) + (availL ? uni32(v_skL) & 1 : 0);
  const int seg_nb = (availU && availL ? (uni32(v_skUL) >> 1) + 1 : 0) | ((availU ? (uni32(v_skU) >> 1) + 1 : 0) << 4) | ((availL ? (uni32(v_skL) >> 1) + 1 : 0) << 8);
  const int nb_txU = availU ? uni32(f->m_txsize[iU]) : -1, nb_txL = availL ? uni32(f->m_txsize[iL]) : -1;
  const uint16_t *ycost = k.cost() + CDF_KF_Y + (intra_mode_ctx(amode) * 5 + intra_mode_ctx(lmode)) * CDF_KF_Y_STRIDE;
// ... 35 lines not shown
    int rank = 0;
    for (int j = 0; j < 13; j++) { const long long o = SH->satd[j]; rank += (o < mine) || (o == mine && j < LANE); }
    SH->order[rank] = LANE;
  }
  WG_SYNC();
  const int ncand = Tools<TS>::FULL ? 7 : 3;
  int tx_ns = 0, tx_set = 0;
  const int tx_off0 = rect_tx_cdf(f, Tools<TS>::reduced_tx_set(f), 0, &tx_ns, &tx_set);
  const int ntx = (Tools<TS>::rdo_tx(f) && tx_off0 >= 0) ? tx_ns : 1;
  LDS uint16_t *pcache = MAXN <= 16 ? (LDS uint16_t *)SH->lpred : (LDS uint16_t *)SH->split_rec;
  for (int ci = W; ci < ncand; ci += NW) predict_block_wh(f, x, y, WL, HL, availL, availU, SH->order[ci], 0, ftype_y, ra, rl, wa, wl, S->etmp, pcache + ci * NN);
  PH(12);
  WG_SYNC();
  long long my_j = J_INF; int my_e = 1 << 30, my_mode = DC_PRED, my_tx = DCT_DCT, cur = 0; TxRes my_tr = { 0, 0, 0, 0, 0 }; uint32_t my_mrate = 0;
  constexpr bool CAN_GROUP = NW == 4 && MAXN <= 32;
  bool grouped = false, parked = false; int my_g = 0;
  if constexpr (CAN_GROUP) grouped = true;
  if constexpr (CAN_GROUP) if (grouped) {
    const int g = GROUP_ID, total = ncand * ntx, rounds = (total + 15) >> 4;
    LDS uint16_t *park_rec = (LDS uint16_t *)S->dcp; LDS int32_t *park_qc = (LDS int32_t *)(S->dcp + 64);
    for (int rd = 0; rd < rounds; rd++) {
      int e;
      if (ncand == 3 && ntx == 5) e = g < 3 ? g * 5 + W : (W < 3 ? W * 5 + 4 : -1);
      else e = rd * 16 + W * 4 + g;
      const bool live = e >= 0 && e < total;
      const int ee = live ? e : 0, ci = ee / ntx, ti = ee - ci * ntx, m = SH->order[ci];
      const uint32_t mode_rate = ycost[m];
      int ns2, set2;
      const int tx_off = rect_tx_cdf(f, Tools<TS>::reduced_tx_set(f), m, &ns2, &set2);
      int txtype;
      if (ntx > 1) txtype = sym_to_txtype(tx_set, ti);
      else { txtype = mode_to_txtype(m); if (tx_off < 0 || txtype_to_sym(tx_set, txtype) < 0) txtype = DCT_DCT; }
      GroupRes gr;
      eval_group_wh<WL, HL>(k.cc(), k.cost(), f, &S->grp[g], SH->srcb[0], pcache + ci * NN, 0, txtype, sctx_y, dctx_y, tx_off, tx_off >= 0 ? txtype_to_sym(tx_set, txtype) : 0,
                            Tools<TS>::tune_psnr(f) ? -1 : psv_a, psv_b, act, &gr);
      long long j = rd_dist32(f, 0, gr.sse) + rd_rate32(f, gr.rate) + rd_rate32(f, mode_rate);
      if (!live) j = J_INF;
      bool improved = false;
#pragma unroll
      for (int gg = 0; gg < 4; gg++) {
        const long long jg = ((long long)__builtin_amdgcn_readlane((int)(j >> 32), gg * 16) << 32) | (unsigned int)__builtin_amdgcn_readlane((int)j, gg * 16);
        const int eg = __builtin_amdgcn_readlane(e, gg * 16);
        if (jg < my_j || (jg == my_j && eg < my_e)) {
          my_j = jg; my_e = eg; my_g = gg; improved = true;
          my_mode = __builtin_amdgcn_readlane(m, gg * 16); my_tx = __builtin_amdgcn_readlane(txtype, gg * 16);
          my_tr.eob = __builtin_amdgcn_readlane(gr.eob, gg * 16); my_tr.cul = __builtin_amdgcn_readlane(gr.cul, gg * 16); my_tr.dcc = __builtin_amdgcn_readlane(gr.dcc, gg * 16);
          my_mrate = (uint32_t)__builtin_amdgcn_readlane((int)mode_rate, gg * 16);
        }
      }
      if (rounds > 1 && improved) {
        for (int i = LANE; i < NN; i += 64) { park_rec[i] = S->grp[my_g].rec[i]; park_qc[i] = S->grp[my_g].qc[i]; }
        parked = true;
        WAVE_SYNC();
      }
    }
  }
  if (!grouped)
  for (int e = W; e < ncand * ntx; e += NW) {
    const int ci = e / ntx, ti = e - ci * ntx, m = SH->order[ci];
    const LDS uint16_t *cpred = pcache + ci * NN;
    const uint32_t mode_rate = ycost[m];
    int ns2, set2;
    const int tx_off = rect_tx_cdf(f, Tools<TS>::reduced_tx_set(f), m, &ns2, &set2);
    int txtype;
    if (ntx > 1) txtype = sym_to_txtype(tx_set, ti);
    else { txtype = mode_to_txtype(m); if (tx_off < 0 || txtype_to_sym(tx_set, txtype) < 0) txtype = DCT_DCT; }
    TxRes tr;
// ... 83 lines not shown
                const int xr = ax - x, yr = ay - y;
                if (xr >= 0 && xr < W_ && yr >= 0 && yr < H_) return (int)canvas[yr * W_ + xr];
                if (yr == -1 && xr >= -1 && xr < W_ + H_) return (int)ra[xr];
                if (xr == -1 && yr >= 0 && yr < W_ + H_) return (int)rl[yr];
                return (int)grec[(size_t)ay * rs + ax];
              };
              for (int i = gl; i <= 8; i += 16) {
                const bool corner = i == 8;
                int a, l;
                if (sU) a = px(corner ? (sL ? sx - 1 : sx) : imin_(lim_a, sx + i), sy - 1); else a = px(sL ? sx - 1 : sx, sy);
                if (sL) l = px(sx - 1, imin_(lim_l, sy + i)); else l = px(sx, sU ? sy - 1 : sy);
                if (!sU && !sL) { a = corner ? (1 << (bd - 1)) : (1 << (bd - 1)) - 1; l = (1 << (bd - 1)) + 1; }
                if (corner) { A[-1] = (uint16_t)a; Lf[-1] = (uint16_t)a; } else { A[i] = (uint16_t)a; Lf[i] = (uint16_t)l; }
              }
            }
            WAVE_SYNC();
            if (dirm) predict_dir_group<4>(f, sx, sy, sL, sU, pa, ftype_y, A, Lf, &S->gpred[g], ppred);
            else predict_nondir_group<4>(best_mode, sL, sU, bd, A, Lf, ppred);
            int ssc, sdc;
            {
              const uint32_t m0 = q ? cmeta[0] : 0u;
              const int inner = (int)(((m0 >> 16) & 0xFF) | ((m0 >> 24) << 8) | (1u << 16));
              const int nt = (q == 1 && H_ == 8) ? inner : sub[8 + 2 * q], nl = (q == 1 && W_ == 8) ? inner : sub[8 + 2 * q + 1];
              const int top = (nt >> 16) ? (nt & 0xFF) : 0, left = (nl >> 16) ? (nl & 0xFF) : 0, dt = (nt >> 16) ? ((nt >> 8) & 0xFF) : 0, dl = (nl >> 16) ? ((nl >> 8) & 0xFF) : 0;
              const int dcs = (dt == 1 ? -1 : (dt == 2 ? 1 : 0)) + (dl == 1 ? -1 : (dl == 2 ? 1 : 0));
              sdc = dcs < 0 ? 1 : (dcs > 0 ? 2 : 0);
              if (top == 0 && left == 0) ssc = 1;
              else if (top == 0 || left == 0) ssc = 2 + (imax_(top, left) > 3);
              else if (imax_(top, left) <= 3) ssc = 4;
              else if (imin_(top, left) <= 3) ssc = 5;
              else ssc = 6;
            }
            GroupRes gr;
            eval_group<4>(k.cc(), k.cost(), k.ls(), f, &S->grp[g], SH->ssrc + q * 16, ppred, 0, 0, txtype, ssc, sdc, stx_off, tx_sym, Tools<TS>::tune_psnr(f) ? -1 : SH->psv4[q], SH->pact[0], &gr);
            if (has_chain) jc += rd_dist32(f, 0, gr.sse) + rd_rate32(f, gr.rate);
            {
              const LDS uint16_t *srec = S->grp[g].rec; const LDS int32_t *sqc = S->grp[g].qc;
              canvas[(bi * 4 + (gl >> 2)) * W_ + bj * 4 + (gl & 3)] = srec[gl]; cqc[q * 16 + gl] = sqc[gl];
              cmeta[q] = (uint32_t)gr.eob | ((uint32_t)gr.cul << 16) | ((uint32_t)gr.dcc << 24);
            }
            any |= gr.eob > 0;
            WAVE_SYNC();
          }
          const int slot = sntx == 5 ? (W == 0 ? g + 1 : (g == 0 ? 0 : 4 + g)) : W * 4 + g;
          cres_j[slot] = (has_chain && jc < thr) ? jc : J_INF; cres_any[slot] = any;
        }
        WG_SYNC();
        int be = -1; long long bjc = J_INF;
        for (int e2 = 0; e2 < sntx; e2++) { const long long v = cres_j[e2]; if (v < bjc) { bjc = v; be = e2; } }
        j_split = bjc;
        if (be >= 0) {
          const int ow = sntx == 5 ? (be == 0 ? 1 : 0) : be >> 2, og = sntx == 5 ? (be == 0 ? 0 : be - 1) : be & 3;
          if (W == ow) {
            const LDS uint8_t *cst = (const LDS uint8_t *)k.wave(2 + W) + og * CH_BYTES;
            const LDS uint16_t *canvas = (const LDS uint16_t *)cst; const LDS int32_t *cqc = (const LDS int32_t *)(cst + NN * 2); const LDS uint32_t *cmeta = (const LDS uint32_t *)(cst + NN * 2 + NN * 4);
            if (LANE < NN) { split_rec[LANE] = canvas[LANE]; split_qc[LANE] = cqc[LANE]; }
            int btx;
            if (sntx > 1) btx = sym_to_txtype(stx_set, be);
            else { btx = mode_to_txtype(best_mode); if (stx_off < 0 || txtype_to_sym(stx_set, btx) < 0) btx = DCT_DCT; }
            if (LANE < 2) { const uint32_t m = cmeta[LANE]; const int eob = (int)(m & 0xFFFF); sub[LANE * 4 + 0] = eob ? btx : DCT_DCT; sub[LANE * 4 + 1] = eob; sub[LANE * 4 + 2] = (int)((m >> 16) & 0xFF); sub[LANE * 4 + 3] = (int)(m >> 24); }
          }
          sub_any = cres_any[be];
          WG_SYNC();
        }
      }
      if (j_split < luma_j) {
        luma_j = j_split; any_coef = sub_any;
// ... 51 lines not shown
    int alpha_u = 0, alpha_v = 0;
#pragma unroll
    for (int pp = 0; pp < 2; pp++) {
      const int idx = SH->ca_sse[pp][1] < SH->ca_sse[pp][0] ? SH->ca_idx[pp][1] : SH->ca_idx[pp][0];
      const int al = idx < 0 ? 0 : ((idx & 1) ? -((idx >> 1) + 1) : ((idx >> 1) + 1));
      if (pp == 0) alpha_u = al; else alpha_v = al;
    }
    const int cfl_ok = alpha_u != 0 || alpha_v != 0;
    GroupRes gr = { 0, 0, 0, 0, 0 };
    const int cw = (W & 1) == 0;
    if (!cw && nplain == 2) {
      const int p = (W >> 1) + 1;
      predict_block_wh(f, x, y, WL, HL, availL, availU, best_mode, 0, ftype_uv, SH->ra[p] + EDGE_OFF, SH->rl[p] + EDGE_OFF, wa, wl, S->etmp, k.wave(W - 1)->pred + NN);
    }
    if (cw) {
      const int p = (W >> 1) + 1;
      {
        const int al = p == 1 ? alpha_u : alpha_v;
        LDS uint16_t *cp = S->pred + (nc - 1) * NN;
        int lsum = LANE < NN ? (int)SH->luma_rec[LANE] << 3 : 0;
        lsum = wave_sum_i32(lsum);
        const int avg = round2_(lsum, WL + HL);
        if (LANE < NN) { const int l = ((int)SH->luma_rec[LANE] << 3) - avg, v = al * l, sc = v >= 0 ? round2_(v, 6) : -round2_(-v, 6); cp[LANE] = (uint16_t)iclamp_((int)S->dcp[LANE] + sc, 0, mx); }
      }
      WAVE_SYNC();
    }
    WG_SYNC();
    if (cw) {
      const int p = (W >> 1) + 1;
      const int g = GROUP_ID, cand = imin_(g, nc - 1);
      const int um = cand == nc - 1 ? UV_CFL_PRED : (cand == 0 ? DC_PRED : best_mode);
      int txtype = mode_to_txtype(um);
      if (txtype_to_sym(uvset, txtype) < 0) txtype = DCT_DCT;
      eval_group_wh<WL, HL>(k.cc(), k.cost(), f, &S->grp[g], SH->srcb[p], cand == 0 ? (const LDS uint16_t *)S->dcp : (const LDS uint16_t *)(S->pred + cand * NN), p, txtype,
                            SH->sctx[p], SH->dctx[p], -1, 0, -1, 0, SH->cact, &gr);
      const long long jp = rd_dist32(f, p, gr.sse) + rd_rate32(f, gr.rate);
      if (GROUP_LANE == 0 && g < nc) SH->cj[g][p - 1] = jp;
    }
    WG_SYNC();
    long long best_uv = J_INF; int bc = 0, b_sign = 0;
#pragma unroll
    for (int cnd = 0; cnd < 3; cnd++) {
      if (cnd < nc) {
        const int is_cfl = cnd == nc - 1, um = is_cfl ? UV_CFL_PRED : (cnd == 0 ? DC_PRED : best_mode);
        int jsign = 0;
        const uint32_t mode_rate = uv_mode_rate(k.cost(), uvcost, um, false, 0, is_cfl && cfl_ok, alpha_u, alpha_v, &jsign);
        if (!is_cfl || cfl_ok) {
          const long long j = SH->cj[cnd][0] + SH->cj[cnd][1] + rd_rate32(f, mode_rate);
          if (j < best_uv) { best_uv = j; bc = cnd; b_sign = jsign; }
        }
      }
    }
    if (cw) {
      const int p = (W >> 1) + 1, chose_cfl = bc == nc - 1;
      const int beob = __builtin_amdgcn_readlane(gr.eob, bc * 16), bcul = __builtin_amdgcn_readlane(gr.cul, bc * 16), bdcc = __builtin_amdgcn_readlane(gr.dcc, bc * 16);
      commit_rect<WL, HL>(f, p, r, c, S->grp[bc].rec, S->grp[bc].qc, beob, bcul, bdcc);
      if (LANE == 0) SH->ceob[p - 1] = beob;
      if (p == 1) {
        fill_rect<WL, HL>(f->m_uvmode, ms, r, c, chose_cfl ? UV_CFL_PRED : (bc == 0 ? DC_PRED : best_mode));
        fill_rect<WL, HL>((uint8_t *)f->m_angle_uv, ms, r, c, 0);
        fill_rect<WL, HL>(f->m_cfl_sign, ms, r, c, chose_cfl ? b_sign : 0);
        fill_rect<WL, HL>(f->m_cfl_au, ms, r, c, (chose_cfl && alpha_u) ? iabs_(alpha_u) - 1 : 0);
        fill_rect<WL, HL>(f->m_cfl_av, ms, r, c, (chose_cfl && alpha_v) ? iabs_(alpha_v) - 1 : 0);
      }
    }
    WG_SYNC();
    any_coef |= (SH->ceob[0] > 0) | (SH->ceob[1] > 0);
// ... 37 lines not shown
    int alpha_u = 0, alpha_v = 0;
#pragma unroll
    for (int pp = 0; pp < 2; pp++) {
      const int idx = SH->ca_sse[pp][1] < SH->ca_sse[pp][0] ? SH->ca_idx[pp][1] : SH->ca_idx[pp][0];
      const int al = idx < 0 ? 0 : ((idx & 1) ? -((idx >> 1) + 1) : ((idx >> 1) + 1));
      if (pp == 0) alpha_u = al; else alpha_v = al;
    }
    const int cfl_ok = alpha_u != 0 || alpha_v != 0;
    LDS uint16_t *park_rec = (LDS uint16_t *)SH->lpred + (p - 1) * 96; LDS int32_t *park_qc = (LDS int32_t *)(park_rec + 32); LDS int *park_meta = (LDS int *)SH->order + (p - 1) * 3;
    long long best_uv = J_INF; int b_ci = 1 << 30, b_sign = 0, b_round = 0;
    const int ns = nc <= 4 ? 1 : 2, nrounds = nc > 4 * ns ? 2 : 1, dealt = half < ns;
    GroupRes gr = { 0, 0, 0, 0, 0 };
    const int g = GROUP_ID;
#pragma unroll 1
    for (int rd = 0; rd < nrounds; rd++) {
      const int base = nrounds == 2 && rd == 0 ? 4 * ns : 0;
#pragma unroll 1
      for (int g2 = 0; g2 < 4; g2++) {
        const int ci = base + half + ns * g2;
        if (dealt && ci < nc) {
          const int um = lut4(cand_pack, ci);
          LDS uint16_t *cp = S->pred + g2 * NN;
          if (um == UV_CFL_PRED) {
            const int al = p == 1 ? alpha_u : alpha_v;
            if (LANE < NN) { const int l = ((int)SH->luma_rec[LANE] << 3) - lavg, v = al * l, sc = v >= 0 ? round2_(v, 6) : -round2_(-v, 6); cp[LANE] = (uint16_t)iclamp_((int)S->dcp[LANE] + sc, 0, mx); }
            WAVE_SYNC();
          } else if (um != DC_PRED) predict_block_wh(f, x, y, WL, HL, availL, availU, um, 0, ftype_uv, pra, prl, wa, wl, S->etmp, cp);
        }
      }
      const int ci = base + half + ns * g, live = dealt && ci < nc;
      const int um = lut4(cand_pack, live ? ci : 0);
      int txtype = mode_to_txtype(um);
      if (txtype_to_sym(uvset, txtype) < 0) txtype = DCT_DCT;
      if (dealt) eval_group_wh<WL, HL>(k.cc(), k.cost(), f, &S->grp[g], SH->srcb[p], um == DC_PRED ? (const LDS uint16_t *)S->dcp : (const LDS uint16_t *)(S->pred + g * NN), p, txtype,
                            SH->sctx[p], SH->dctx[p], -1, 0, -1, 0, SH->cact, &gr);
      const long long jp = rd_dist32(f, p, gr.sse) + rd_rate32(f, gr.rate);
      if (GROUP_LANE == 0 && live) SH->cj[ci][p - 1] = jp;
      WG_SYNC();
      long long r_best = J_INF; int r_ci = 1 << 30, r_sign = 0;
      for (int cc = base; cc < imin_(nc, base + 4 * ns); cc++) {
        const int um2 = lut4(cand_pack, cc), is_cfl = um2 == UV_CFL_PRED;
        if (is_cfl && !cfl_ok) continue;
        int jsign = 0;
        const uint32_t mode_rate = uv_mode_rate(k.cost(), uvcost, um2, false, 0, is_cfl, alpha_u, alpha_v, &jsign);
        const long long j = SH->cj[cc][0] + SH->cj[cc][1] + rd_rate32(f, mode_rate);
        if (j < r_best) { r_best = j; r_ci = cc; r_sign = jsign; }
      }
      if (r_best < best_uv || (r_best == best_uv && r_ci < b_ci)) { best_uv = r_best; b_ci = r_ci; b_sign = r_sign; b_round = rd; }
      if (nrounds == 2 && rd == 0 && r_ci < nc && (r_ci - base) % ns == half) {
        const int gg = (r_ci - base) / ns;
        if (LANE < NN) { park_rec[LANE] = S->grp[gg].rec[LANE]; park_qc[LANE] = S->grp[gg].qc[LANE]; }
        const int e_ = __builtin_amdgcn_readlane(gr.eob, gg * 16), c_ = __builtin_amdgcn_readlane(gr.cul, gg * 16), d_ = __builtin_amdgcn_readlane(gr.dcc, gg * 16);
        if (LANE == 0) { park_meta[0] = e_; park_meta[1] = c_; park_meta[2] = d_; }
      }
    }
    const int b_um = lut4(cand_pack, b_ci), chose_cfl = b_um == UV_CFL_PRED;
    const int from_park = nrounds == 2 && b_round == 0;
    if (from_park ? half == 0 : b_ci % ns == half) {
      int beob, bcul, bdcc;
      if (from_park) {
        beob = park_meta[0]; bcul = park_meta[1]; bdcc = park_meta[2];
        commit_rect<WL, HL>(f, p, r, c, (const LDS uint16_t *)park_rec, (const LDS int32_t *)park_qc, beob, bcul, bdcc);
      } else {
        const int gg = b_ci / ns;
        beob = __builtin_amdgcn_readlane(gr.eob, gg * 16); bcul = __builtin_amdgcn_readlane(gr.cul, gg * 16); bdcc = __builtin_amdgcn_readlane(gr.dcc, gg * 16);
        commit_rect<WL, HL>(f, p, r, c, S->grp[gg].rec, S->grp[gg].qc, beob, bcul, bdcc);
      }
// ... 28 lines not shown
```

### cavif_rs_amd/csrc/tile_search.h

```cpp
#pragma once
#include "dev_common.h"
#include "dev_predict.h"
#include "dev_txfm.h"
#include "dev_rate.h"
#include "dev_group.h"

#ifndef MI_BALLOT64
#define MI_BALLOT64(p) __builtin_amdgcn_ballot_w64(p)
#endif
#define MI_K1_TRY_ATTR __attribute__((noinline, not_tail_called))
#define MI_K1_WG_PER_CU 4
#define WAVE_ID ((int)(threadIdx.x >> 6))
#ifndef MI_PROFILE
#define MI_PROFILE 0
#endif
#ifndef MI_PROF_MAXN
#define MI_PROF_MAXN 16
#endif
#ifndef MI_DEBUG_HOOKS
#define MI_DEBUG_HOOKS 0
#endif
#if MI_DEBUG_HOOKS
#define DBG_IS(f, v) ((f)->dbg == (v))
#else
#define DBG_IS(f, v) false
#endif
#if MI_PROFILE
#define PH_BEGIN() unsigned long long ph_t_ = clock64()
#define PH(i) do { const unsigned long long n_ = clock64(); if (LANE == 0 && !(MI_PROFILE == 3 && (i) >= 16 && (i) <= 21)) SH->prof[W][i] += n_ - ph_t_; ph_t_ = n_; } while (0)
#define PH_SIZE(slot, call) [&]() { const unsigned long long t0_ = clock64(); const long long r_ = (call); if (MI_PROFILE == 3 && LANE == 0) k.sh()->prof[WAVE_ID][16 + (slot)] += clock64() - t0_; return r_; }()
#else
#define PH_SIZE(slot, call) (call)
#define PH_BEGIN() do {} while (0)
#define PH(i) do {} while (0)
#endif

#define MI_SNAP_BYTES(n) (3 * (n) * (n) * 6 + 18 * ((n) / 4) * ((n) / 4) + 3 * ((n) / 4) * ((n) / 4) * 2 + 64)
#define MI_SNAP_BYTES_SQ(n) (2 * MI_SNAP_BYTES(n))
#define MI_SNAP_BYTES_ALL(n) (MI_SNAP_BYTES_SQ(n) + 2 * MI_SNAP_BYTES(8))

struct Blk64Wave { uint16_t pred[64 * 64]; int32_t tbuf[32 * 65]; int32_t cbuf[32 * 32]; int32_t qc[32 * 32]; };
struct Blk64None { uint8_t none_; };
struct Blk64Shared { uint16_t src64[64 * 64], bnd[2048];      uint8_t cnb_top[2][16][2], cnb_left[2][16][2]; };
template <int N> struct WaveScratch {
  static constexpr int CS = N < 32 ? N : 32, NBUF = 2, DCP_LEN = N * N, E = N == 32 ? 64 : N;
  uint16_t wa[EDGE_LEN(E)], wl[EDGE_LEN(E)], etmp[2 * E + 16];
  union {
    struct {
      uint16_t pred[N * N], dcp[N * N];
      union {
        struct {
          uint16_t rec[2][N * N];
          int32_t tbuf[N * (N + 1)], cbuf[CS * CS], qc[2][CS * CS];
        };
        GroupBuf8 grp[4];
        GroupPredBuf gpred[4];
      };
    };
    typename std::conditional<N == 32, Blk64Wave, Blk64None>::type b64;
  };
  uint8_t lev[LEV_BYTES(CS)];
};
template <int N> struct SharedScratch {
  static constexpr int E = N == 32 ? 64 : N, NC = E >= 16 ? (E / 8) * (E / 8) : 1, SNC = E >= 32 ? (E / 16) * (E / 16) : 1;
  uint16_t ra[3][EDGE_LEN(E)], rl[3][EDGE_LEN(E)];
  uint16_t srcb[3][N * N];
  uint16_t luma_rec[N * N];
  long long satd[13], dsd[7][6];
  long long wbest_j[4], cj[16][2], pbest_j[2];
  int order[13], wbest_e[4], pbest_c[2], calpha[2][2], ldelta[7];
  uint16_t part_cost[40];
  uint16_t lpred[N <= 32 ? 768 : 4];
  long long ca_sse[2][2]; int ca_idx[2][2];
  int lm_mode, lm_delta, lm_tx, lm_eob, ceob[2], sctx[3], dctx[3];
  long long lm_mode_j;
  int psv[NC], pact[NC], psv4[4], spsv[SNC], spact[SNC], cact, seg, seg_nb;
  uint16_t ssrc[N * N], spred[(E / 2) * (E / 2)];
  uint8_t nb_top[16][2], nb_left[16][2];
  int32_t split_qc[N <= 16 ? 1 : (N >= 64 ? 4096 : N * N)];
  uint16_t split_rec[N <= 16 ? 1 : N * N];
  typename std::conditional<N == 32, Blk64Shared, Blk64None>::type x64;
  TileB tile; uint8_t *snap;
  int q_item;
  int fine;
#if MI_PROFILE
  unsigned long long prof[4][32];
#endif
};

struct TxRes { int eob, cul, dcc; long long sse; uint32_t rate; };
#if MI_PROFILE
extern __shared__ __align__(16) uint8_t mi_prof_smem_[];
template <int N> __device__ __forceinline__ LDS unsigned long long &mi_prof_slot_n(int w, int i) { return ((LDS SharedScratch<N> *)mi_prof_smem_)->prof[w][i]; }
#endif

template <int TS> struct Tools {
  static constexpr bool FULL = (TS & 1) != 0, FIXED = (TS & 2) != 0;
  template <typename F> static __device__ __forceinline__ bool rdo_tx(F f) { return FIXED ? true : f->rdo_tx != 0; }
  template <typename F> static __device__ __forceinline__ bool reduced_tx_set(F f) { return FIXED ? true : f->reduced_tx_set != 0; }
  template <typename F> static __device__ __forceinline__ bool fine_directional(F f) { return FIXED ? true : f->fine_directional != 0; }
  template <typename F> static __device__ __forceinline__ bool tx_mode_select(F f) { return FIXED ? true : f->tx_mode_select != 0; }
  template <typename F> static __device__ __forceinline__ bool tune_psnr(F f) { return FIXED ? false : f->tune_psnr != 0; }
};
template <int MAXN, int NW, int TS_ = 0> struct Ctx {
  static constexpr int TS = TS_;
  static constexpr int MAXBS = MAXN == 16 ? 2 : 4;
  static constexpr size_t SH_BYTES = (sizeof(SharedScratch<MAXN>) + 15) & ~(size_t)15, WS_BYTES = (sizeof(WaveScratch<MAXN>) + 15) & ~(size_t)15;
  static constexpr size_t SC_BYTES = SCAN_LDS_ENTRIES(MAXN) * 2, CC_BYTES = (COEF_COST_MAX_ENTRIES(MAXBS) * 2 + 15) & ~(size_t)15;
  static constexpr size_t LS_OFF = SH_BYTES + NW * WS_BYTES, CC_OFF = LS_OFF + SC_BYTES, F_OFF = CC_OFF + CC_BYTES;
  LDS uint8_t *base;
  LDS WaveScratch<MAXN> *ws;
  __device__ __forceinline__ LDS SharedScratch<MAXN> *sh() const { return (LDS SharedScratch<MAXN> *)base; }
  __device__ __forceinline__ LDS WaveScratch<MAXN> *s() const { return ws; }
  __device__ __forceinline__ LDS WaveScratch<MAXN> *wave(int w) const { return (LDS WaveScratch<MAXN> *)(base + SH_BYTES + (size_t)w * WS_BYTES); }
  __device__ __forceinline__ const LDS uint16_t *ls() const { return (const LDS uint16_t *)(base + LS_OFF); }
  __device__ __forceinline__ LDS uint16_t *cc_base() const { return (LDS uint16_t *)(base + CC_OFF); }
  __device__ __forceinline__ CoefCost cc() const { return coef_cost_layout(cc_base(), MAXBS); }
  __device__ __forceinline__ const LDS FrameDev *f() const { return (const LDS FrameDev *)(base + F_OFF); }
  __device__ __forceinline__ const LDS TileB *t() const { return &sh()->tile; }
  __device__ __forceinline__ uint8_t *snap() const { return sh()->snap; }
  __device__ __forceinline__ const uint16_t *cost() const { return f()->cost; }
};

static_assert(offsetof(FrameDev, ac_recip) - offsetof(FrameDev, dc_q) == 36 && sizeof(SegTab::Q) == 48, "a SegTab entry is copied over FrameDev::dc_q .. ac_recip");
template <typename SHT> __device__ __forceinline__ void seg_select(const LDS FrameDev *f, LDS SHT *SH, int scale) {
  if (!f->seg_n) return;
  const SegTab *st = f->seg;
  const int b = seg_bucket((uint32_t)uni32(scale));
  int a = 0;
  for (int j = 0; j + 1 < f->seg_n; j++) a += b >= st->thr[j];
  const int seg = f->seg_n - 1 - a;
  if (LANE < 12) ((LDS uint32_t *)((LDS FrameDev *)f)->dc_q)[LANE] = ((const uint32_t *)&st->q[seg])[LANE];
  if (LANE == 0) SH->seg = seg;
}

#define IS_SMOOTH_(m) ((m) == SMOOTH_PRED || (m) == SMOOTH_V_PRED || (m) == SMOOTH_H_PRED)
// ... 107 lines not shown
}
__device__ __forceinline__ uint32_t uv_mode_rate(const uint16_t *cost, const uint16_t *uvcost, int um, bool angle_coded, int delta, bool cfl, int alpha_u, int alpha_v, int *jsign) {
  const int su = alpha_u == 0 ? 0 : (alpha_u < 0 ? 1 : 2), sv = alpha_v == 0 ? 0 : (alpha_v < 0 ? 1 : 2);
  const int js = cfl ? su * 3 + sv - 1 : 0;
  const uint32_t r_mode = uvcost[um];
  const uint32_t r_ang = cost[CDF_ANGLE + (angle_coded ? (um - V_PRED) * CDF_ANGLE_STRIDE + delta + 3 : 0)];
  const uint32_t r_sign = cost[CDF_CFL_SIGN + js];
  const uint32_t r_au = cost[CDF_CFL_ALPHA + ((cfl && su) ? ((su - 1) * 3 + sv) * CDF_CFL_ALPHA_STRIDE + iabs_(alpha_u) - 1 : 0)];
  const uint32_t r_av = cost[CDF_CFL_ALPHA + ((cfl && sv) ? ((sv - 1) * 3 + su) * CDF_CFL_ALPHA_STRIDE + iabs_(alpha_v) - 1 : 0)];
  *jsign = js;
  return r_mode + (angle_coded ? r_ang : 0u) + (cfl ? r_sign + (su ? r_au : 0u) + (sv ? r_av : 0u) : 0u);
}

template <int MAXN, int BS, int NW, int TS>
__device__ inline long long eval_tx(const Ctx<MAXN, NW, TS> k, int plane, int sctx, int dctx, const LDS uint16_t *pred, int txtype, int tx_off, int tx_sym,
                                    LDS uint16_t *rec_out, LDS int32_t *qc_out, TxRes *tr, const LDS uint16_t *src_override = nullptr,
                                    const LDS int *psv = nullptr, const LDS int *pact = nullptr) {
  constexpr int n = 4 << BS, P = n + 1, CS = n < 32 ? n : 32;
  const LDS FrameDev *f = k.f(); LDS WaveScratch<MAXN> *S = k.s();
  const LDS uint16_t *src = src_override ? src_override : k.sh()->srcb[plane];
#if MI_PROFILE
  LDS SharedScratch<MAXN> *SH = k.sh(); const int W = WAVE_ID;
#endif
  PH_BEGIN();
  for (int idx = LANE; idx < n * n; idx += 64) {
    const int i = idx / n, j = idx % n;
    S->tbuf[i * P + j] = (int)src[idx] - (int)pred[idx];
    rec_out[idx] = pred[idx];
  }
  WAVE_SYNC();
  PH(16);
  fwd_txfm2d_dev<n>(S->tbuf, S->cbuf, txtype);
  PH(17);
  const int eob = quant_rate_dev<CS>(k.cc(), k.cost(), k.ls(), S->cbuf, qc_out, S->lev, plane, BS, txtype, f->dc_q[plane], f->ac_q[plane], f->dc_recip[plane], f->ac_recip[plane],
                                     f->bd, sctx, dctx, tx_off, tx_sym, &tr->rate, &tr->cul, &tr->dcc);
  PH(19);
  if (eob > 0) inv_txfm2d_add_dev<n>(S->cbuf, S->tbuf, rec_out, txtype, f->bd);
  tr->eob = eob;
  PH(20);
  if (plane == 0 && !Tools<TS>::tune_psnr(f)) tr->sse = psy_dist_wave<n>(src, rec_out, psv ? psv : (const LDS int *)k.sh()->psv, pact ? pact : (const LDS int *)k.sh()->pact, f->bd);
  else { const long long e = sse_dev(src, rec_out, n * n); tr->sse = plane == 0 ? e : (e * k.sh()->cact + 8192) >> 14; }
  PH(21);
  return ((tr->sse * f->wq[plane]) >> 5) + (((long long)tr->rate * f->rdmult + 256) >> 9);
}

template <int BS, typename RecPtr, typename QcPtr>
__device__ inline void commit_plane(const LDS FrameDev *f, int plane, int r, int c, RecPtr rec, QcPtr qc, int eob, int cul, int dcc) {
  constexpr int n = 4 << BS, CS = n < 32 ? n : 32, n4 = 1 << BS;
  uint16_t *gr = f->rec[plane] + (size_t)(r * 4) * f->stride + c * 4;
  int32_t *gc = f->coef[plane] + (size_t)(r * 4) * f->stride + c * 4;
  for (int idx = LANE; idx < n * n; idx += 64) gr[(idx / n) * f->stride + (idx % n)] = rec[idx];
  for (int idx = LANE; idx < CS * CS; idx += 64) gc[(idx / CS) * f->stride + (idx % CS)] = qc[idx];
  fill_map_dev(f->m_lvl[plane], f->mi_stride, r, c, n4, cul);
  fill_map_dev(f->m_dc[plane], f->mi_stride, r, c, n4, dcc);
  if (LANE == 0) f->m_eob[plane][r * f->mi_stride + c] = (uint16_t)eob;
}

#include "dev_rect.h"

template <int MAXN, int BS, int NW, int TS>
__device__ MI_K1_TRY_ATTR long long try_block(const Ctx<MAXN, NW, TS> k, int r, int c, long long budget = J_INF) {
  constexpr int n = 4 << BS, n4 = 1 << BS, log2w = 2 + BS, nn = n * n, CS = n < 32 ? n : 32, qn = CS * CS;
  const LDS FrameDev *f = k.f(); const LDS TileB *t = k.t(); LDS WaveScratch<MAXN> *S = k.s(); LDS SharedScratch<MAXN> *SH = k.sh();
  const int W = NW > 1 ? WAVE_ID : 0;
  const int ms = f->mi_stride, mi = r * ms + c, x = c * 4, y = r * 4;
  const int availU = r > t->mi_row_start, availL = c > t->mi_col_start;
  const int can_ar = availU && (c + n4 < t->mi_col_end), can_bl = availL && (r + n4 < t->mi_row_end);
// ... 141 lines not shown
      if (m >= V_PRED && m <= D67_PRED && refine) {
        long long bsd = SH->satd[m];
        for (int q = 0; q < 6; q++) { const long long sd = SH->dsd[ci][q]; if (sd < bsd) { bsd = sd; delta = dl_of(q); } }
      }
      predict_block(f, x, y, log2w, availL, availU, m, delta, ftype_y, ra, rl, wa, wl, S->etmp, SH->lpred + ci * nn);
      if (LANE == 0) SH->ldelta[ci] = delta;
    }
    PH(12);
    WG_SYNC();
    PH(2);
  }
  long long my_j = J_INF; int my_e = 1 << 30, my_mode = DC_PRED, my_delta = 0, my_tx = DCT_DCT, cur = 0; TxRes my_tr = { 0, 0, 0, 0, 0 };
  uint32_t my_mrate = 0;
  bool grouped = false, parked = false; int my_g = 0;
  if constexpr (SMALL_GROUPED) {
    grouped = pred_cached;
    if (grouped) {
      const int g = GROUP_ID, total = ncand * ntx, rounds = (total + 15) >> 4;
      LDS uint16_t *park_rec = (LDS uint16_t *)S->dcp; LDS int32_t *park_qc = (LDS int32_t *)(S->dcp + 64);
      for (int rd = 0; rd < rounds; rd++) {
        int e;
        if (ncand == 3 && ntx == 5) e = g < 3 ? g * 5 + W + 1 : (W < 3 ? W * 5 : -1);
        else e = rd * 16 + W * 4 + g;
        const bool live = e >= 0 && e < total;
        const int ee = live ? e : 0, ci = ee / ntx, ti = ee - ci * ntx, m = SH->order[ci];
        const int delta = SH->ldelta[ci];
        const uint32_t mode_rate = y_mode_rate(k.cost(), ycost, m, m >= V_PRED && m <= D67_PRED && BS >= BS_8, delta);
        int ns2, set2;
        const int tx_off = intra_tx_cdf_r(f, Tools<TS>::reduced_tx_set(f), BS, m, &ns2, &set2);
        int txtype;
        if (ntx > 1) txtype = sym_to_txtype(tx_set, ti);
        else { txtype = mode_to_txtype(m); if (tx_off < 0 || txtype_to_sym(tx_set, txtype) < 0) txtype = DCT_DCT; }
        GroupRes gr;
        eval_group<n>(k.cc(), k.cost(), k.ls(), f, &S->grp[g], SH->srcb[0], SH->lpred + ci * nn, 0, BS, txtype, sctx_y, dctx_y, tx_off,
                      tx_off >= 0 ? txtype_to_sym(tx_set, txtype) : 0, Tools<TS>::tune_psnr(f) ? -1 : SH->psv[0], SH->pact[0], &gr);
        long long j = rd_dist32(f, 0, gr.sse) + rd_rate32(f, gr.rate) + rd_rate32(f, mode_rate);
        if (!live) j = J_INF;
        bool improved = false;
#pragma unroll
        for (int gg = 0; gg < 4; gg++) {
          const long long jg = ((long long)__builtin_amdgcn_readlane((int)(j >> 32), gg * 16) << 32) | (unsigned int)__builtin_amdgcn_readlane((int)j, gg * 16);
          const int eg = __builtin_amdgcn_readlane(e, gg * 16);
          if (jg < my_j || (jg == my_j && eg < my_e)) {
            my_j = jg; my_e = eg; my_g = gg; improved = true;
            my_mode = __builtin_amdgcn_readlane(m, gg * 16); my_delta = __builtin_amdgcn_readlane(delta, gg * 16); my_tx = __builtin_amdgcn_readlane(txtype, gg * 16);
            my_tr.eob = __builtin_amdgcn_readlane(gr.eob, gg * 16); my_tr.cul = __builtin_amdgcn_readlane(gr.cul, gg * 16); my_tr.dcc = __builtin_amdgcn_readlane(gr.dcc, gg * 16);
            my_mrate = (uint32_t)__builtin_amdgcn_readlane((int)mode_rate, gg * 16);
          }
        }
        if (rounds > 1 && improved) {
          for (int i = LANE; i < nn; i += 64) { park_rec[i] = S->grp[my_g].rec[i]; park_qc[i] = S->grp[my_g].qc[i]; }
          parked = true;
          WAVE_SYNC();
        }
      }
    }
  }
  if (!grouped)
  for (int e = W; e < ncand * ntx; e += NW) {
    const int ci = e / ntx, ti = e - ci * ntx, m = SH->order[ci];
    const int directional = m >= V_PRED && m <= D67_PRED;
    int delta = 0;
    const LDS uint16_t *lpred = S->pred;
    if (pred_cached) { delta = SH->ldelta[ci]; lpred = SH->lpred + ci * nn; }
    else {
      if (directional && refine) {
        long long bsd = SH->satd[m];
// ... 163 lines not shown
                  if (sL) l = px(sx - 1, imin_(lim_l, sy + ii)); else l = px(sx, sU ? sy - 1 : sy);
                  if (!sU && !sL) { a = corner ? (1 << (bd - 1)) : (1 << (bd - 1)) - 1; l = (1 << (bd - 1)) + 1; }
                  if (act && corner) { A[-1] = (uint16_t)a; Lf[-1] = (uint16_t)a; }
                  if (act && !corner) { A[ii] = (uint16_t)a; Lf[ii] = (uint16_t)l; }
                }
              }
              WAVE_SYNC();
              if (dirm) predict_dir_group<hn>(f, sx, sy, sL, sU, pa, ftype_y, A, Lf, &S->gpred[g], ppred);
              else predict_nondir_group<hn>(best_mode, sL, sU, bd, A, Lf, ppred);
              PH(23);
              int ssc, sdc;
              {
                int top = 0, left = 0, dcs = 0;
                const uint32_t mt = bi ? cmeta[q - G] : 0u, ml = bj ? cmeta[q - 1] : 0u;
#pragma unroll
                for (int k2 = 0; k2 < half; k2++) {
                  int l, d;
                  if (bi == 0) { l = SH->nb_top[bj * half + k2][0]; d = SH->nb_top[bj * half + k2][1]; } else { l = (int)((mt >> 16) & 0xFF); d = (int)(mt >> 24); if (n >= 32 && c + bj * half + k2 >= f->mi_cols) l = d = 0; }
                  top = imax_(top, l); dcs += d == 1 ? -1 : (d == 2 ? 1 : 0);
                  if (bj == 0) { l = SH->nb_left[bi * half + k2][0]; d = SH->nb_left[bi * half + k2][1]; } else { l = (int)((ml >> 16) & 0xFF); d = (int)(ml >> 24); if (n >= 32 && r + bi * half + k2 >= f->mi_rows) l = d = 0; }
                  left = imax_(left, l); dcs += d == 1 ? -1 : (d == 2 ? 1 : 0);
                }
                sdc = dcs < 0 ? 1 : (dcs > 0 ? 2 : 0);
                if (top == 0 && left == 0) ssc = 1;
                else if (top == 0 || left == 0) ssc = 2 + (imax_(top, left) > 3);
                else if (imax_(top, left) <= 3) ssc = 4;
                else if (imin_(top, left) <= 3) ssc = 5;
                else ssc = 6;
              }
              constexpr int pcp = n >= 8 ? n / 8 : 1;
              const int psv_q = hn == 4 ? (n == 8 ? SH->psv4[q] : psv16[q]) : SH->psv[bi * pcp + bj];
              const int pact_q = hn == 4 ? SH->pact[(bi >> 1) * pcp + (bj >> 1)] : SH->pact[bi * pcp + bj];
              GroupRes gr;
              eval_group<hn>(k.cc(), k.cost(), k.ls(), f, &S->grp[g], ssrc + q * hnn, ppred, 0, SBS, txtype, ssc, sdc, stx_off, tx_sym, Tools<TS>::tune_psnr(f) ? -1 : psv_q, pact_q, &gr);
              {
                const long long j = rd_dist32(f, 0, gr.sse) + rd_rate32(f, gr.rate);
                long long jslot = j;
                if (paired) {
                  const long long jo = ((long long)__shfl((int)(j >> 32), LANE ^ 16) << 32) | (unsigned int)__shfl((int)j, LANE ^ 16);
                  jslot = q1 >= 0 ? j + jo : (mem == 0 ? j : jo);
                }
                if (has_chain) jc += jslot;
              }
              if (has_chain) {
                const LDS uint16_t *srec = S->grp[g].rec; const LDS int32_t *sqc = S->grp[g].qc;
                const int ro = bi * hn * n + bj * hn;
#pragma unroll
                for (int i = gl; i < hnn; i += 16) canvas[ro + (i / hn) * n + (i % hn)] = srec[i];
#pragma unroll
                for (int i = gl; i < sqn; i += 16) cqc[q * sqn + i] = sqc[i];
                cmeta[q] = (uint32_t)gr.eob | ((uint32_t)gr.cul << 16) | ((uint32_t)gr.dcc << 24);
              }
              any |= gr.eob > 0;
              WAVE_SYNC();
              PH(25);
            }
            if (paired) any |= __shfl(any, LANE ^ 16);
            const int rslot = paired ? (has_chain ? e : 5 + (g & 1)) : (sntx == 5 ? (W == 0 ? g + 1 : (g == 0 ? 0 : 4 + g)) : W * 4 + g);
            cres_j[rslot] = (has_chain && jc < thr) ? jc : J_INF; cres_any[rslot] = any;
          }
          __builtin_amdgcn_s_setprio(0);
          WG_SYNC();
          PH(26);
          int be = -1; long long bjc = J_INF;
          for (int e2 = 0; e2 < sntx; e2++) { const long long v = cres_j[e2]; if (v < bjc) { bjc = v; be = e2; } }
          j_split = bjc;
          if (be >= 0) {
// ... 208 lines not shown
      const int al = idx < 0 ? 0 : ((idx & 1) ? -((idx >> 1) + 1) : ((idx >> 1) + 1));
      if (pp == 0) alpha_u = al; else alpha_v = al;
    }
    const int cfl_ok = alpha_u != 0 || alpha_v != 0;
    GroupRes gr = { 0, 0, 0, 0, 0 };
    const int cw = (W & 1) == 0;
    if (!cw && nplain == 2) {
      const int p = (W >> 1) + 1;
      predict_block(f, x, y, log2w, availL, availU, best_mode, bdelta, ftype_uv, SH->ra[p] + EDGE_OFF, SH->rl[p] + EDGE_OFF, wa, wl, S->etmp, k.wave(W - 1)->pred + nn);
    }
    if (cw) {
      const int p = (W >> 1) + 1;
      {
        const int al = p == 1 ? alpha_u : alpha_v;
        LDS uint16_t *cp = S->pred + (nc - 1) * nn;
        int lsum = 0;
        for (int idx = LANE; idx < nn; idx += 64) lsum += SH->luma_rec[idx] << 3;
        lsum = wave_sum_i32(lsum);
        const int avg = round2_(lsum, 2 * log2w);
        for (int idx = LANE; idx < nn; idx += 64) {
          const int l = ((int)SH->luma_rec[idx] << 3) - avg, v = al * l, sc = v >= 0 ? round2_(v, 6) : -round2_(-v, 6);
          cp[idx] = (uint16_t)iclamp_((int)S->dcp[idx] + sc, 0, mx);
        }
      }
      WAVE_SYNC();
    }
    WG_SYNC();
    if (cw) {
      const int p = (W >> 1) + 1;
      const int g = GROUP_ID, cand = imin_(g, nc - 1);
      const int um = cand == nc - 1 ? UV_CFL_PRED : (cand == 0 ? DC_PRED : best_mode);
      int txtype = mode_to_txtype(um);
      if (txtype_to_sym(uvset, txtype) < 0) txtype = DCT_DCT;
      eval_group<n>(k.cc(), k.cost(), k.ls(), f, &S->grp[g], SH->srcb[p], cand == 0 ? (const LDS uint16_t *)S->dcp : (const LDS uint16_t *)(S->pred + cand * nn), p, BS, txtype, SH->sctx[p], SH->dctx[p], -1, 0, -1, SH->cact, &gr);
      const long long jp = rd_dist32(f, p, gr.sse) + rd_rate32(f, gr.rate);
      if (GROUP_LANE == 0 && g < nc) SH->cj[g][p - 1] = jp;
    }
    PH(9);
    WG_SYNC();
    PH(2);
    long long best_uv = J_INF; int bc = 0, b_sign = 0;
#pragma unroll
    for (int cnd = 0; cnd < 3; cnd++) {
      if (cnd < nc) {
        const int is_cfl = cnd == nc - 1, um = is_cfl ? UV_CFL_PRED : (cnd == 0 ? DC_PRED : best_mode);
        int jsign = 0;
        const uint32_t mode_rate = uv_mode_rate(k.cost(), uvcost, um, !is_cfl && cnd == 1 && um >= V_PRED && um <= D67_PRED && BS >= BS_8, bdelta,
                                                is_cfl && cfl_ok, alpha_u, alpha_v, &jsign);
        if (!is_cfl || cfl_ok) {
          const long long j = SH->cj[cnd][0] + SH->cj[cnd][1] + rd_rate32(f, mode_rate);
          if (j < best_uv) { best_uv = j; bc = cnd; b_sign = jsign; }
        }
      }
    }
    if (cw) {
      const int p = (W >> 1) + 1, chose_cfl = bc == nc - 1;
      const int eob = __builtin_amdgcn_readlane(gr.eob, 0), eob1 = __builtin_amdgcn_readlane(gr.eob, 16), eob2 = __builtin_amdgcn_readlane(gr.eob, 32);
      const int cul = __builtin_amdgcn_readlane(gr.cul, 0), cul1 = __builtin_amdgcn_readlane(gr.cul, 16), cul2 = __builtin_amdgcn_readlane(gr.cul, 32);
      const int dcc = __builtin_amdgcn_readlane(gr.dcc, 0), dcc1 = __builtin_amdgcn_readlane(gr.dcc, 16), dcc2 = __builtin_amdgcn_readlane(gr.dcc, 32);
      const int beob = bc == 0 ? eob : (bc == 1 ? eob1 : eob2), bcul = bc == 0 ? cul : (bc == 1 ? cul1 : cul2), bdcc = bc == 0 ? dcc : (bc == 1 ? dcc1 : dcc2);
      commit_plane<BS>(f, p, r, c, S->grp[bc].rec, S->grp[bc].qc, beob, bcul, bdcc);
      if (LANE == 0) SH->ceob[p - 1] = beob;
      if (p == 1) {
        const int buv = chose_cfl ? UV_CFL_PRED : (bc == 0 ? DC_PRED : best_mode);
        fill_map_dev(f->m_uvmode, ms, r, c, n4, buv);
        fill_map_dev((uint8_t *)f->m_angle_uv, ms, r, c, n4, (uint8_t)(int8_t)((!chose_cfl && bc == 1) ? bdelta : 0));
        fill_map_dev(f->m_cfl_sign, ms, r, c, n4, chose_cfl ? b_sign : 0);
// ... 68 lines not shown
      if (pp == 0) alpha_u = al; else alpha_v = al;
    }
    const int cfl_ok = alpha_u != 0 || alpha_v != 0;
    LDS uint16_t *park_rec = (LDS uint16_t *)SH->lpred + (p - 1) * 3 * nn; LDS int32_t *park_qc = (LDS int32_t *)(park_rec + nn); LDS int *park_meta = (LDS int *)SH->order + (p - 1) * 3;
    static_assert(2 * 3 * nn <= 768, "the parked candidates fit lpred");
    long long best_uv = J_INF; int b_ci = 1 << 30, b_sign = 0, b_round = 0, b_delta = 0;
    const int ns = nc <= 4 ? 1 : 2, nrounds = nc > 4 * ns ? 2 : 1, dealt = half < ns;
    GroupRes gr = { 0, 0, 0, 0, 0 };
    const int g = GROUP_ID;
    auto delta_of = [&](int um) { return (um == best_mode && um >= V_PRED && um <= D67_PRED && BS >= BS_8) ? best_delta : 0; };
#pragma unroll 1
    for (int rd = 0; rd < nrounds; rd++) {
      const int base = nrounds == 2 && rd == 0 ? 4 * ns : 0;
#pragma unroll 1
      for (int g2 = 0; g2 < 4; g2++) {
        const int ci = base + half + ns * g2;
        if (dealt && ci < nc) {
          const int um = lut4(cand_pack, ci);
          LDS uint16_t *cp = S->pred + g2 * nn;
          if (um == UV_CFL_PRED) {
            const int al = p == 1 ? alpha_u : alpha_v;
            for (int idx = LANE; idx < nn; idx += 64) {
              const int l = ((int)SH->luma_rec[idx] << 3) - lavg, v = al * l, sc = v >= 0 ? round2_(v, 6) : -round2_(-v, 6);
              cp[idx] = (uint16_t)iclamp_((int)S->dcp[idx] + sc, 0, mx);
            }
            WAVE_SYNC();
          } else if (um != DC_PRED) predict_block(f, x, y, log2w, availL, availU, um, delta_of(um), ftype_uv, pra, prl, wa, wl, S->etmp, cp);
        }
      }
      const int ci = base + half + ns * g, live = dealt && ci < nc;
      const int um = lut4(cand_pack, live ? ci : 0);
      int txtype = mode_to_txtype(um);
      if (txtype_to_sym(uvset, txtype) < 0) txtype = DCT_DCT;
      if (dealt) eval_group<n>(k.cc(), k.cost(), k.ls(), f, &S->grp[g], SH->srcb[p], um == DC_PRED ? (const LDS uint16_t *)S->dcp : (const LDS uint16_t *)(S->pred + g * nn), p, BS, txtype,
                    SH->sctx[p], SH->dctx[p], -1, 0, -1, SH->cact, &gr);
      const long long jp = rd_dist32(f, p, gr.sse) + rd_rate32(f, gr.rate);
      if (GROUP_LANE == 0 && live) SH->cj[ci][p - 1] = jp;
      PH(9);
      WG_SYNC();
      PH(2);
      long long r_best = J_INF; int r_ci = 1 << 30, r_sign = 0, r_delta = 0;
      for (int cc = base; cc < imin_(nc, base + 4 * ns); cc++) {
        const int um2 = lut4(cand_pack, cc), is_cfl = um2 == UV_CFL_PRED;
        if (is_cfl && !cfl_ok) continue;
        int jsign = 0;
        const int d2 = delta_of(um2);
        const uint32_t mode_rate = uv_mode_rate(k.cost(), uvcost, um2, um2 >= V_PRED && um2 <= D67_PRED && BS >= BS_8, d2, is_cfl, alpha_u, alpha_v, &jsign);
        const long long j = SH->cj[cc][0] + SH->cj[cc][1] + rd_rate32(f, mode_rate);
        if (j < r_best) { r_best = j; r_ci = cc; r_sign = jsign; r_delta = d2; }
      }
      if (r_best < best_uv || (r_best == best_uv && r_ci < b_ci)) { best_uv = r_best; b_ci = r_ci; b_sign = r_sign; b_round = rd; b_delta = r_delta; }
      if (nrounds == 2 && rd == 0 && r_ci < nc && (r_ci - base) % ns == half) {
        const int gg = (r_ci - base) / ns;
        for (int i = LANE; i < nn; i += 64) { park_rec[i] = S->grp[gg].rec[i]; park_qc[i] = S->grp[gg].qc[i]; }
        const int e_ = __builtin_amdgcn_readlane(gr.eob, gg * 16), c_ = __builtin_amdgcn_readlane(gr.cul, gg * 16), d_ = __builtin_amdgcn_readlane(gr.dcc, gg * 16);
        if (LANE == 0) { park_meta[0] = e_; park_meta[1] = c_; park_meta[2] = d_; }
      }
    }
    const int b_um = lut4(cand_pack, b_ci), chose_cfl = b_um == UV_CFL_PRED;
    const int from_park = nrounds == 2 && b_round == 0;
    if (from_park ? half == 0 : b_ci % ns == half) {
      int beob, bcul, bdcc;
      if (from_park) {
        beob = park_meta[0]; bcul = park_meta[1]; bdcc = park_meta[2];
        commit_plane<BS>(f, p, r, c, (const LDS uint16_t *)park_rec, (const LDS int32_t *)park_qc, beob, bcul, bdcc);
      } else {
        const int gg = b_ci / ns;
// ... 562 lines not shown
```

Baseline: 563.7.

## Specialize coefficient-rate evaluation for 2-D-only transform sets in fixed speed tiers

Adds an ONLY_2D template flag, enabled for fixed-tool speed settings, that drops the vertical and horizontal transform-class branches from scan, context and rate code in eval_group, the 4x4 tail and quant_rate. The per-coefficient symbol-cost logic moves into a shared coef_sym_bits helper with a precomputed neighbour struct. A wave-wide flag skips base-range cost work when no coefficient exceeds level 2. Static asserts check that the reduced transform sets hold only 2-D types. Per-stage clock64 profiling hooks are also added under MI_PROFILE==4, compiled out by default.

```diff
diff --git a/__graft_entry__.py b/__graft_entry__.py
--- a/__graft_entry__.py
+++ b/__graft_entry__.py
@@ -65,6 +65,11 @@
         k1_lookups_harness.build_all(force=force)
     except Exception as e:
         print('warning: tests/kernels lookup harness build failed (%s); tests/test_k1_lookups.py will fail, the product library is unaffected' % e, file=sys.stderr)
+    try:
+        from tests.helpers import coef_rate_harness
+        coef_rate_harness.build_all(force=force)
+    except Exception as e:
+        print('warning: tests/kernels coefficient-rate harness build failed (%s); tests/test_coef_rate.py will fail, the product library is unaffected' % e, file=sys.stderr)
     import cavif_rs_amd
     cavif_rs_amd.load_library()
 
diff --git a/cavif_rs_amd/csrc/dev_blk64.h b/cavif_rs_amd/csrc/dev_blk64.h
--- a/cavif_rs_amd/csrc/dev_blk64.h
+++ b/cavif_rs_amd/csrc/dev_blk64.h
@@ -178,7 +178,7 @@
     const uint32_t mode_rate = y_mode_rate(k.cost(), ycost, m, directional, delta);
     TxRes tr;
     fwd_txfm64_dev(SH->x64.src64, B->pred, B->tbuf, B->cbuf);
-    const int eob = quant_rate_dev<32>(k.cc(), k.cost(), k.ls(), B->cbuf, B->qc, S->lev, 0, BS, DCT_DCT, f->dc_q[0], f->ac_q[0], f->dc_recip[0], f->ac_recip[0],
+    const int eob = quant_rate_dev<32,  true>(k.cc(), k.cost(), k.ls(), B->cbuf, B->qc, S->lev, 0, BS, DCT_DCT, f->dc_q[0], f->ac_q[0], f->dc_recip[0], f->ac_recip[0],
                                        f->bd, sctx_y, dctx_y, -1, 0, &tr.rate, &tr.cul, &tr.dcc);
     if (eob > 0) inv_txfm64_add_dev(B->cbuf, B->tbuf, B->pred, f->bd);
     tr.eob = eob;
diff --git a/cavif_rs_amd/csrc/dev_common.h b/cavif_rs_amd/csrc/dev_common.h
--- a/cavif_rs_amd/csrc/dev_common.h
+++ b/cavif_rs_amd/csrc/dev_common.h
@@ -180,12 +180,19 @@
 
 template <typename FP> __device__ __forceinline__ long long rd_dist32(FP f, int plane, int sse) { return (long long)(((unsigned long long)(uint32_t)sse * (unsigned long long)f->wq[plane]) >> 5); }
 template <typename FP> __device__ __forceinline__ long long rd_rate32(FP f, uint32_t rate) { return (long long)(((unsigned long long)rate * (unsigned long long)f->rdmult + 256) >> 9); }
-__device__ __forceinline__ int tx_set_of(int txs, int reduced) { return txs >= 3 ? 0 : (reduced ? 2 : (txs == 2 ? 2 : 1)); }
+__device__ __forceinline__ constexpr int tx_set_of(int txs, int reduced) { return txs >= 3 ? 0 : (reduced ? 2 : (txs == 2 ? 2 : 1)); }
 __device__ __forceinline__ int tx_set_count(int set) { return set == 0 ? 1 : (set == 1 ? 7 : 5); }
+constexpr unsigned long long TXSET1_TYPES = 0x213ba09ULL;
+constexpr unsigned long long TXSET2_TYPES = 0x21309ULL;
+constexpr unsigned long long MODE_TXTYPES = 0x3213122130210ULL;
 __device__ __forceinline__ int sym_to_txtype(int set, int s) {
   if (set == 0) return DCT_DCT;
-  if (set == 1) return lut4(0x213ba09ULL, s);
-  return lut4(0x21309ULL, s);
+  if (set == 1) return lut4(TXSET1_TYPES, s);
+  return lut4(TXSET2_TYPES, s);
+}
+constexpr bool txtypes_all_2d(unsigned long long tab, int n) {
+  for (int i = 0; i < n; i++) if ((int)((tab >> (4 * i)) & 15) >= V_DCT) return false;
+  return true;
 }
 __device__ __forceinline__ int txtype_to_sym(int set, int t) {
   const unsigned long long inv12 = set == 1 ? 0xffff320fffff4651ULL : 0xffffff0fffff2431ULL, inv = set == 0 ? 0xfffffffffffffff0ULL : inv12;
@@ -193,7 +200,7 @@
   return s == 15 ? -1 : s;
 }
 __device__ __forceinline__ int mode_to_txtype(int m) {
-  return lut4(0x3213122130210ULL, m);
+  return lut4(MODE_TXTYPES, m);
 }
 __device__ __forceinline__ int tx_class_of(int t) {
   if (t == V_DCT || t == V_ADST || t == V_FLIPADST) return TXC_VERT;
@@ -207,16 +214,16 @@
   for (int i = LANE; i < 256; i += 64) ls[80 + i] = av1_default_scan_16x16[i];
   if (maxn >= 32) for (int i = LANE; i < 1024; i += 64) ls[336 + i] = av1_default_scan_32x32[i];
 }
-__device__ __forceinline__ int scan_pos(const LDS uint16_t *ls, int n, int cls, int i) {
-  if (cls == TXC_2D) return ls[(n == 4 ? 0 : n == 8 ? 16 : n == 16 ? 80 : 336) + i];
+template <bool ONLY_2D = false> __device__ __forceinline__ int scan_pos(const LDS uint16_t *ls, int n, int cls, int i) {
+  if (ONLY_2D || cls == TXC_2D) return ls[(n == 4 ? 0 : n == 8 ? 16 : n == 16 ? 80 : 336) + i];
   if (cls == TXC_VERT) return i;
   const int c = i / n, r = i - c * n; return r * n + c;
 }
 static __device__ const uint8_t rect_scan_4x8[32] = { 0, 1, 4, 2, 5, 8, 3, 6, 9, 12, 7, 10, 13, 16, 11, 14, 17, 20, 15, 18, 21, 24, 19, 22, 25, 28, 23, 26, 29, 27, 30, 31 };
 static __device__ const uint8_t rect_scan_8x4[32] = { 0, 8, 1, 16, 9, 2, 24, 17, 10, 3, 25, 18, 11, 4, 26, 19, 12, 5, 27, 20, 13, 6, 28, 21, 14, 7, 29, 22, 15, 30, 23, 31 };
-__device__ __forceinline__ int rect_scan_pos(int wl, int hl, int cls, int i) {
+template <bool ONLY_2D = false> __device__ __forceinline__ int rect_scan_pos(int wl, int hl, int cls, int i) {
   const int w = 1 << wl, h = 1 << hl;
-  if (cls == TXC_2D) return hl > wl ? rect_scan_4x8[i] : rect_scan_8x4[i];
+  if (ONLY_2D || cls == TXC_2D) return hl > wl ? rect_scan_4x8[i] : rect_scan_8x4[i];
   if (cls == TXC_VERT) return i;
   const int c = i / h, r = i - c * h; return r * w + c;
 }
diff --git a/cavif_rs_amd/csrc/dev_group.h b/cavif_rs_amd/csrc/dev_group.h
--- a/cavif_rs_amd/csrc/dev_group.h
+++ b/cavif_rs_amd/csrc/dev_group.h
@@ -10,6 +10,14 @@
   uint16_t rec[64];
   uint8_t lev[144];
 };
+#if defined(MI_PROFILE) && MI_PROFILE == 4
+__device__ void mi_gprof_add(int slot, unsigned long long cycles);
+#define GPH_BEGIN() unsigned long long gph_t_ = clock64()
+#define GPH(i) do { const unsigned long long n_ = clock64(); mi_gprof_add((i), n_ - gph_t_); gph_t_ = n_; } while (0)
+#else
+#define GPH_BEGIN() do {} while (0)
+#define GPH(i) do {} while (0)
+#endif
 #define GROUP_LANE (LANE & 15)
 #define GROUP_ID (LANE >> 4)
 
@@ -44,14 +52,15 @@
 struct GroupRes { int eob, cul, dcc, sse; uint32_t rate; };
 
 template <int CTRL> __device__ __forceinline__ int dpp_row_z(int v) { return __builtin_amdgcn_update_dpp(0, v, CTRL, 0xF, 0xF, false); }
-template <typename FP>
+template <bool ONLY_2D, typename FP>
 __device__ __forceinline__ void eval_group4_tail(const CoefCost &cc, FP f, LDS GroupBuf8 *gb, int coef, int t_src, int t_rec, int tidx, int plane, int txs, int txtype, int ck, int rk,
                                                  int skip_ctx, int dc_ctx, int tx_off, uint32_t tx_cost, int psy_sv, int psy_act, GroupRes *res) {
   constexpr int N = 4, nc = 16;
   const int gl = GROUP_LANE, row = gl >> 2, col = gl & 3, bd = f->bd;
+  GPH_BEGIN();
   const int dcq = f->dc_q[plane], acq = f->ac_q[plane];
   const uint32_t dc_recip = f->dc_recip[plane], ac_recip = f->ac_recip[plane];
-  const int cls = tx_class_of(txtype), pt = plane > 0, txs_ctx = txs;
+  const int cls = coef_class<ONLY_2D>(txtype), pt = plane > 0, txs_ctx = txs;
   const uint32_t dc_off = (uint32_t)(dcq * 109 / 256), off0 = (uint32_t)(acq * 98 / 256), off1 = (uint32_t)(acq * 109 / 256), off_eob = (uint32_t)(acq * 88 / 256);
   const uint32_t thr = (uint32_t)acq - off_eob, uq = (uint32_t)acq;
   const int c = cls == TXC_2D ? lut4(0xFEA9DB83C7426510ULL, gl) : (cls == TXC_VERT ? gl : col * 4 + row);
@@ -86,12 +95,14 @@
     const int v = neg ? -(int)m : (int)m;
     dq = v < dmn ? dmn : (v > dmx ? dmx : v);
   }
+  GPH(17);
   const int l15 = imin_(lv, 15);
   const int s1 = dpp_row_z<0x101>(l15), s2 = dpp_row_z<0x102>(l15), s3 = dpp_row_z<0x103>(l15), s5 = dpp_row_z<0x105>(l15);
   const int b1 = dpp_row_z<0x104>(l15), b2 = dpp_row_z<0x108>(l15), b3 = dpp_row_z<0x10C>(l15);
   const int r1 = col < 3 ? s1 : 0, r2 = col < 2 ? s2 : 0, r3 = col < 1 ? s3 : 0, d1 = col < 3 ? s5 : 0;
   uint32_t head = cc.txb[(txs_ctx * 13 + skip_ctx) * CDF_TXB_SKIP_STRIDE + (eob == 0)];
   int bits = 0, cul = 0, dcc = 0;
+  const bool with_br = coef_any(lv > 2);
   if (eob > 0) {
     if (tx_off >= 0) head += tx_cost;
     const int eob_pt = eob_to_pt(eob);
@@ -101,48 +112,17 @@
       head += cc.eobx[((txs_ctx * 2 + pt) * 9 + (eob_pt - 3)) * CDF_EOB_EXTRA_STRIDE + hi];
       head += 512u * (uint32_t)(nb - 1);
     }
-    if (c < eob) {
-      const int level = lv;
-      if (c == eob - 1) {
-        const int ctx = c == 0 ? 0 : (c <= nc / 8 ? 1 : (c <= nc / 4 ? 2 : 3));
-        bits += cc.beob[((txs_ctx * 2 + pt) * 4 + ctx) * CDF_COEFF_BASE_EOB_STRIDE + imin_(level, 3) - 1];
-      } else {
-        int mag2 = imin_(r1, 3) + imin_(b1, 3), ctx;
-        if (cls == TXC_2D) {
-          mag2 += imin_(d1, 3) + imin_(r2, 3) + imin_(b2, 3);
-          const int m = imin_((mag2 + 1) >> 1, 4);
-          ctx = (row == 0 && col == 0) ? 0 : (row + col < 2 ? m + 1 : (row + col < 4 ? m + 6 : m + 21));
-        } else if (cls == TXC_VERT) {
-          mag2 += imin_(b2, 3) + imin_(b3, 3);
-          const int m = imin_((mag2 + 1) >> 1, 4);
-          ctx = m + (row == 0 ? 26 : (row == 1 ? 31 : 36));
-        } else {
-          mag2 += imin_(r2, 3) + imin_(r3, 3);
-          const int m = imin_((mag2 + 1) >> 1, 4);
-          ctx = m + (col == 0 ? 26 : (col == 1 ? 31 : 36));
-        }
-        bits += cc.base[((txs_ctx * 2 + pt) * 42 + ctx) * CDF_COEFF_BASE_STRIDE + imin_(level, 3)];
-      }
-      if (level > 2) {
-        int mg = r1 + b1, ctx;
-        if (cls == TXC_2D) { mg = imin_((mg + d1 + 1) >> 1, 6); ctx = c == 0 ? mg : ((row < 2 && col < 2) ? mg + 7 : mg + 14); }
-        else if (cls == TXC_HORIZ) { mg = imin_((mg + r2 + 1) >> 1, 6); ctx = c == 0 ? mg : (col == 0 ? mg + 7 : mg + 14); }
-        else { mg = imin_((mg + b2 + 1) >> 1, 6); ctx = c == 0 ? mg : (row == 0 ? mg + 7 : mg + 14); }
-        const int off = ((imin_(txs_ctx, 3) * 2 + pt) * 21 + ctx) * CDF_COEFF_BR_STRIDE;
-        int rem = level - 3;
-        for (int idx = 0; idx < 4; idx++) { const int s2 = imin_(rem, 3); bits += cc.br[off + s2]; rem -= s2; if (s2 < 3) break; }
-      }
-      if (level) {
-        if (c == 0) { bits += cc.dcs[(pt * 3 + dc_ctx) * CDF_DC_SIGN_STRIDE + neg]; dcc = neg ? 1 : 2; }
-        else bits += 512;
-        if (level > 14) { const int len = 32 - __clz(level - 14); bits += 512 * (2 * len - 1); }
-      }
-      cul += level;
-    }
+    CoefNb nb = { r1, b1, d1, r2, b2 };
+    if constexpr (!ONLY_2D) {
+      nb.t3 = sel_(cls == TXC_2D, d1, sel_(cls == TXC_HORIZ, r2, b2)); nb.t4 = sel_(cls == TXC_2D, r2, sel_(cls == TXC_HORIZ, r3, b3)); nb.t5 = sel_(cls == TXC_2D, b2, 0);
+    }
+    bits = coef_sym_bits<ONLY_2D, 0>(cc.base, (int)(cc.beob - cc.base), cc.br, cc.dcs, nb, cls, row, col, c, eob, lv, neg, pt, txs_ctx, dc_ctx, nc, with_br, &dcc);
+    cul = lv;
   }
   bits = row_sum_i32(bits);
   const int cd = row_sum_i32(imin_(cul, 63) | (dcc << 16));
   res->eob = eob; res->cul = imin_(cd & 0xFFFF, 63); res->dcc = cd >> 16; res->rate = head + (uint32_t)bits;
+  GPH(18);
   if (eob > 0) {
     const int cbits = imax_(bd + 6, 16), cmax = (1 << (cbits - 1)) - 1, cmin = -(1 << (cbits - 1));
     int v = iclamp_(tx4_inv(dq, rk), cmin, cmax);
@@ -151,19 +131,22 @@
   }
   gb->rec[tidx] = (uint16_t)t_rec;
   WAVE_SYNC();
+  GPH(19);
   const int d = t_src - t_rec;
   const int s = row_sum_i32(__mul24(d, d));
   if (psy_sv >= 0) { const int sd = row_sum_i32(t_rec), qd = row_sum_i32(__mul24(t_rec, t_rec)); res->sse = psy_cell_dist((uint32_t)s, (uint32_t)sd, (uint32_t)qd, (uint32_t)psy_sv, (uint32_t)psy_act, 4, bd); }
   else res->sse = (int)(((unsigned long long)(uint32_t)s * (uint32_t)psy_act + 8192) >> 14);
-}
-
-template <int N, typename CostPtr>
+  GPH(20);
+}
+
+template <int N, bool ONLY_2D = false, typename CostPtr>
 __device__ inline void eval_group(const CoefCost &cc, CostPtr cost, const LDS uint16_t *ls, const LDS FrameDev *f, LDS GroupBuf8 *gb,
                                   const LDS uint16_t *src, const LDS uint16_t *pred, int plane, int txs, int txtype,
                                   int skip_ctx, int dc_ctx, int tx_off, int tx_sym, int psy_sv, int psy_act, GroupRes *res) {
   constexpr int P = N + 1, nc = N * N, IT = nc / 16, bwl = N == 4 ? 2 : 3, st = N + 4;
   const int gl = GROUP_LANE;
   const int bd = f->bd;
+  GPH_BEGIN();
   const uint32_t tx_cost = cost[tx_off >= 0 ? tx_off + tx_sym : 0];
   int ck, rk; tx_kinds(txtype, &ck, &rk);
   [[maybe_unused]] int t_src = 0, t_rec = 0;
@@ -173,7 +156,8 @@
     int v = tx4_fwd((int)((uint32_t)(t_src - t_rec) << 2), ck);
     v = group_transpose4(v);
     const int coef = tx4_fwd(v, rk);
-    eval_group4_tail(cc, f, gb, coef, t_src, t_rec, tidx, plane, txs, txtype, ck, rk, skip_ctx, dc_ctx, tx_off, tx_cost, psy_sv, psy_act, res);
+    GPH(16);
+    eval_group4_tail<ONLY_2D>(cc, f, gb, coef, t_src, t_rec, tidx, plane, txs, txtype, ck, rk, skip_ctx, dc_ctx, tx_off, tx_cost, psy_sv, psy_act, res);
     return;
   } else {
 #pragma unroll
@@ -203,10 +187,11 @@
     for (int c = 0; c < N; c++) gb->cbuf[gl * N + c] = x[c];
   }
   WAVE_SYNC();
+  GPH(16);
   }
   const int dcq = f->dc_q[plane], acq = f->ac_q[plane];
   const uint32_t dc_recip = f->dc_recip[plane], ac_recip = f->ac_recip[plane];
-  const int cls = tx_class_of(txtype), pt = plane > 0, txs_ctx = txs;
+  const int cls = coef_class<ONLY_2D>(txtype), pt = plane > 0, txs_ctx = txs;
   const uint32_t dc_off = (uint32_t)(dcq * 109 / 256), off0 = (uint32_t)(acq * 98 / 256), off1 = (uint32_t)(acq * 109 / 256), off_eob = (uint32_t)(acq * 88 / 256);
   const uint32_t thr = (uint32_t)acq - off_eob, uq = (uint32_t)acq;
   int pos[IT]; uint32_t mag[IT]; int neg[IT];
@@ -214,7 +199,7 @@
 #pragma unroll
   for (int k = 0; k < IT; k++) {
     const int i = gl + 16 * k;
-    pos[k] = scan_pos(ls, N, cls, i);
+    pos[k] = scan_pos<ONLY_2D>(ls, N, cls, i);
     const int c = gb->cbuf[pos[k]];
     mag[k] = (uint32_t)iabs_(c); neg[k] = c < 0;
     if (i >= 1 && mag[k] >= thr) last = i + 1;
@@ -253,8 +238,13 @@
     gb->cbuf[pp] = v < dmn ? dmn : (v > dmx ? dmx : v);
   }
   WAVE_SYNC();
+  GPH(17);
   uint32_t head = cc.txb[(txs_ctx * 13 + skip_ctx) * CDF_TXB_SKIP_STRIDE + (eob == 0)];
-  int bits = 0, cul = 0, dcc = 0;
+  int bits = 0, cul = 0, dcc = 0, lmax = 0;
+  bool live[IT];
+#pragma unroll
+  for (int k = 0; k < IT; k++) { lmax = imax_(lmax, lvl[k]); live[k] = coef_any(gl + 16 * k < eob); }
+  const bool with_br = coef_any(lmax > 2);
   if (eob > 0) {
     if (tx_off >= 0) head += tx_cost;
     const int eob_pt = eob_to_pt(eob);
@@ -264,37 +254,19 @@
       head += cc.eobx[((txs_ctx * 2 + pt) * 9 + (eob_pt - 3)) * CDF_EOB_EXTRA_STRIDE + hi];
       head += 512u * (uint32_t)(nb - 1);
     }
-#pragma unroll
-    for (int k = 0; k < IT; k++) {
-      const int c = gl + 16 * k;
-      if (c < eob) {
-        const int pp = pos[k], row = pp >> bwl, col = pp & (N - 1), level = lvl[k];
-        const LDS uint8_t *L = gb->lev + row * st + col;
-        if (c == eob - 1) {
-          const int ctx = c == 0 ? 0 : (c <= nc / 8 ? 1 : (c <= nc / 4 ? 2 : 3));
-          bits += cc.beob[((txs_ctx * 2 + pt) * 4 + ctx) * CDF_COEFF_BASE_EOB_STRIDE + imin_(level, 3) - 1];
-        } else {
-          const int ctx = base_ctx(L, st, cls, row, col);
-          bits += cc.base[((txs_ctx * 2 + pt) * 42 + ctx) * CDF_COEFF_BASE_STRIDE + imin_(level, 3)];
-        }
-        if (level > 2) {
-          const int ctx = br_ctx(L, st, cls, row, col, c);
-          const int off = ((imin_(txs_ctx, 3) * 2 + pt) * 21 + ctx) * CDF_COEFF_BR_STRIDE;
-          int rem = level - 3;
-          for (int idx = 0; idx < 4; idx++) { const int s2 = imin_(rem, 3); bits += cc.br[off + s2]; rem -= s2; if (s2 < 3) break; }
-        }
-        if (level) {
-          if (c == 0) { bits += cc.dcs[(pt * 3 + dc_ctx) * CDF_DC_SIGN_STRIDE + neg[k]]; dcc = neg[k] ? 1 : 2; }
-          else bits += 512;
-          if (level > 14) { const int len = 32 - __clz(level - 14); bits += 512 * (2 * len - 1); }
-        }
-        cul += level;
-      }
+    CoefNb nb[IT];
+#pragma unroll
+    for (int k = 0; k < IT; k++) if (live[k]) nb[k] = coef_nb_load<ONLY_2D>(gb->lev + (pos[k] >> bwl) * st + (pos[k] & (N - 1)), st, cls);
+#pragma unroll
+    for (int k = 0; k < IT; k++) if (live[k]) {
+      bits += coef_sym_bits<ONLY_2D, 0>(cc.base, (int)(cc.beob - cc.base), cc.br, cc.dcs, nb[k], cls, pos[k] >> bwl, pos[k] & (N - 1), gl + 16 * k, eob, lvl[k], neg[k], pt, txs_ctx, dc_ctx, nc, with_br, &dcc);
+      cul += lvl[k];
     }
   }
   bits = row_sum_i32(bits);
   const int cd = row_sum_i32(imin_(cul, 63) | (dcc << 16));
   res->eob = eob; res->cul = imin_(cd & 0xFFFF, 63); res->dcc = cd >> 16; res->rate = head + (uint32_t)bits;
+  GPH(18);
   {
     constexpr int ROWSH = N == 4 ? 0 : 1;
     const int cbits = imax_(bd + 6, 16), cmax = (1 << (cbits - 1)) - 1, cmin = -(1 << (cbits - 1));
@@ -329,6 +301,7 @@
       WAVE_SYNC();
     }
   }
+  GPH(19);
   int s = 0, sd = 0, qd = 0;
   if constexpr (N == 4) { const int d = t_src - t_rec; s = __mul24(d, d); sd = t_rec; qd = __mul24(t_rec, t_rec); }
   else
@@ -337,6 +310,7 @@
   s = row_sum_i32(s);
   if (psy_sv >= 0) { sd = row_sum_i32(sd); qd = row_sum_i32(qd); res->sse = psy_cell_dist((uint32_t)s, (uint32_t)sd, (uint32_t)qd, (uint32_t)psy_sv, (uint32_t)psy_act, N == 4 ? 4 : 8, bd); }
   else res->sse = (int)(((unsigned long long)(uint32_t)s * (uint32_t)psy_act + 8192) >> 14);
+  GPH(20);
 }
 
 struct GroupPredBuf { uint16_t wa[48], wl[48], tmp[32], pred[64]; };
diff --git a/cavif_rs_amd/csrc/dev_rate.h b/cavif_rs_amd/csrc/dev_rate.h
--- a/cavif_rs_amd/csrc/dev_rate.h
+++ b/cavif_rs_amd/csrc/dev_rate.h
@@ -1,5 +1,8 @@
 #pragma once
 #include "dev_common.h"
+#ifdef MI_EMU
+#include <cassert>
+#endif
 
 template <typename FP, typename TP> __device__ inline void txb_ctx_dev(FP f, TP t, int plane, int r4, int c4, int txs, int bs, int *skip_ctx, int *dc_ctx) {
   const int w4 = 1 << txs, ms = f->mi_stride;
@@ -86,6 +89,70 @@
   mag += imin_(L[2 * st], 15); mag = imin_((mag + 1) >> 1, 6); return c == 0 ? mag : (row == 0 ? mag + 7 : mag + 14);
 }
 
+__device__ __forceinline__ int sel_(bool c, int a, int b) { return c ? a : b; }
+#define COEF_NB_BATCH 4
+template <bool ONLY_2D> __device__ __forceinline__ int coef_class(int txtype) {
+  if constexpr (!ONLY_2D) return tx_class_of(txtype);
+#ifdef MI_EMU
+  assert(tx_class_of(txtype) == TXC_2D);
+#endif
+  return TXC_2D;
+}
+struct CoefNb { int a, b, t3, t4, t5; };
+template <bool ONLY_2D> __device__ __forceinline__ CoefNb coef_nb_load(const LDS uint8_t *L, int st, int cls) {
+  CoefNb nb;
+  int o3 = st + 1, o4 = 2, o5 = 2 * st;
+  if constexpr (!ONLY_2D) {
+    o3 = sel_(cls == TXC_2D, o3, sel_(cls == TXC_HORIZ, 2, 2 * st));
+    o4 = sel_(cls == TXC_2D, o4, sel_(cls == TXC_HORIZ, 3, 3 * st));
+    o5 = sel_(cls == TXC_2D, o5, sel_(cls == TXC_HORIZ, 4, 4 * st));
+  }
+  nb.a = L[1]; nb.b = L[st]; nb.t3 = L[o3]; nb.t4 = L[o4]; nb.t5 = L[o5];
+  return nb;
+}
+__device__ __forceinline__ void coef_br_split(int rem, int *k, int *r) {
+  const int rc = imin_(rem, 12), q = (rc * 11) >> 5;
+  *k = q; *r = rc - 3 * q;
+}
+#ifndef MI_BALLOT64
+#define MI_BALLOT64(p) __builtin_amdgcn_ballot_w64(p)
+#endif
+__device__ __forceinline__ bool coef_any(bool p) { return MI_BALLOT64(p) != 0ull; }
+template <bool ONLY_2D, int SHAPE, typename TabPtr>
+__device__ __forceinline__ int coef_sym_bits(TabPtr base, int beob_off, TabPtr br, TabPtr dcs, const CoefNb &nb, int cls, int row, int col, int c, int eob, int level, int neg,
+                                             int pt, int txs_ctx, int dc_ctx, int area, bool with_br, int *dcc) {
+  const bool two_d = ONLY_2D || cls == TXC_2D;
+  const int rc = row + col, l3 = imin_(level, 3), tp = txs_ctx * 2 + pt;
+  const int m = imin_((imin_(nb.a, 3) + imin_(nb.b, 3) + imin_(nb.t3, 3) + imin_(nb.t4, 3) + imin_(nb.t5, 3) + 1) >> 1, 4);
+  const int far_ = sel_(rc < 4, 6, 21);
+  const int o2 = SHAPE == 0 ? sel_(rc < 2, 1, far_) : (SHAPE == 1 ? sel_(row < 2, 11, far_) : sel_(col < 2, 16, far_));
+  int bctx = sel_(rc == 0, 0, m + o2);
+  if constexpr (!ONLY_2D) {
+    const int k1 = sel_(cls == TXC_VERT, row, col);
+    bctx = sel_(two_d, bctx, m + sel_(k1 == 0, 26, sel_(k1 == 1, 31, 36)));
+  }
+  const int ectx = sel_(c == 0, 0, sel_(c <= area / 8, 1, sel_(c <= area / 4, 2, 3)));
+  const int i_eob = beob_off + (tp * 4 + ectx) * CDF_COEFF_BASE_EOB_STRIDE + l3 - 1, i_base = (tp * 42 + bctx) * CDF_COEFF_BASE_STRIDE + l3;
+  const int r_base = base[sel_(c == eob - 1, i_eob, i_base)];
+  const int r_sign = dcs[(pt * 3 + dc_ctx) * CDF_DC_SIGN_STRIDE + neg];
+  int r_br = 0;
+  if (with_br) {
+    const int mg = imin_((imin_(nb.a, 15) + imin_(nb.b, 15) + imin_(nb.t3, 15) + 1) >> 1, 6);
+    bool near_ = (row | col) < 2;
+    if constexpr (!ONLY_2D) near_ = two_d ? near_ : (cls == TXC_HORIZ ? col == 0 : row == 0);
+    const int rctx = sel_(c == 0, mg, mg + sel_(near_, 7, 14));
+    const int off = ((imin_(txs_ctx, 3) * 2 + pt) * 21 + rctx) * CDF_COEFF_BR_STRIDE;
+    int k, r;
+    coef_br_split(imax_(level - 3, 0), &k, &r);
+    const int r_full = br[off + 3], r_last = br[off + r];
+    r_br = __mul24(k, r_full) + sel_(k < 4, r_last, 0);
+  }
+  const int len = 32 - __clz(imax_(level - 14, 1)), r_gol = sel_(level > 14, 512 * (2 * len - 1), 0);
+  const int bits = r_base + sel_(level > 2, r_br, 0) + sel_(level != 0, sel_(c == 0, r_sign, 512) + r_gol, 0);
+  *dcc = sel_(c == 0 && level != 0 && c < eob, sel_(neg != 0, 1, 2), *dcc);
+  return sel_(c < eob, bits, 0);
+}
+
 __device__ inline void build_level_map(const LDS int32_t *qc, LDS uint8_t *lev, int n) {
   const int st = n + 4, words = (st * st + 3) >> 2, bwl = n == 4 ? 2 : n == 8 ? 3 : n == 16 ? 4 : 5;
   LDS uint32_t *lw = (LDS uint32_t *)lev;
@@ -147,25 +214,8 @@
   for (int c = LANE; c < eob; c += 64) {
     const int p = scan_pos(ls, n, cls, c), row = p >> bwl, col = p & (n - 1);
     const int v = qc[p], level = iabs_(v);
-    const LDS uint8_t *L = lev + row * st + col;
-    if (c == eob - 1) {
-      const int ctx = c == 0 ? 0 : (c <= area / 8 ? 1 : (c <= area / 4 ? 2 : 3));
-      bits += cc.beob[((txs_ctx * 2 + pt) * 4 + ctx) * CDF_COEFF_BASE_EOB_STRIDE + imin_(level, 3) - 1];
-    } else {
-      const int ctx = base_ctx(L, st, cls, row, col);
-      bits += cc.base[((txs_ctx * 2 + pt) * 42 + ctx) * CDF_COEFF_BASE_STRIDE + imin_(level, 3)];
-    }
-    if (level > 2) {
-      const int ctx = br_ctx(L, st, cls, row, col, c);
-      const int off = ((imin_(txs_ctx, 3) * 2 + pt) * 21 + ctx) * CDF_COEFF_BR_STRIDE;
-      int rem = level - 3;
-      for (int idx = 0; idx < 4; idx++) { const int s = imin_(rem, 3); bits += cc.br[off + s]; rem -= s; if (s < 3) break; }
-    }
-    if (level) {
-      if (c == 0) { bits += cc.dcs[(pt * 3 + dc_ctx) * CDF_DC_SIGN_STRIDE + (v < 0)]; dcc = v < 0 ? 1 : 2; }
-      else bits += 512;
-      if (level > 14) { const int len = 32 - __clz(level - 14); bits += 512 * (2 * len - 1); }
-    }
+    const CoefNb nb = coef_nb_load<false>(lev + row * st + col, st, cls);
+    bits += coef_sym_bits<false, 0>(cc.base, (int)(cc.beob - cc.base), cc.br, cc.dcs, nb, cls, row, col, c, eob, level, v < 0, pt, txs_ctx, dc_ctx, area, true, &dcc);
     cul += level;
   }
   bits = wave_sum_i32(bits);
@@ -178,14 +228,14 @@
 #define LEV_OFF(cs) ((cs) == 4 ? 0 : (cs) == 8 ? 64 : (cs) == 16 ? 64 + 144 : 64 + 144 + 400)
 #define LEV_BYTES(maxcs) ((maxcs) == 4 ? 64 : (maxcs) == 8 ? 64 + 144 : (maxcs) == 16 ? 64 + 144 + 400 : 64 + 144 + 400 + 1296)
 
-template <int CS, typename CostPtr>
+template <int CS, bool ONLY_2D = false, typename CostPtr>
 __device__ inline int quant_rate_dev(const CoefCost &cc, CostPtr cost, const LDS uint16_t *ls, LDS int32_t *cbuf, LDS int32_t *qc, LDS uint8_t *levbase,
                                      int plane, int txs, int txtype, int dcq, int acq, uint32_t dc_recip, uint32_t ac_recip, int bd,
                                      int skip_ctx, int dc_ctx, int tx_off, int tx_sym, uint32_t *rate_out, int *cul_out, int *dc_cat) {
   constexpr int n = CS, nc = CS * CS, IT = nc < 64 ? 1 : nc / 64, bwl = CS == 4 ? 2 : CS == 8 ? 3 : CS == 16 ? 4 : 5, st = CS + 4;
   LDS uint8_t *lev = levbase + LEV_OFF(CS);
   const uint32_t tx_cost = cost[tx_off >= 0 ? tx_off + tx_sym : 0];
-  const int cls = tx_class_of(txtype), pt = plane > 0, txs_ctx = txs;
+  const int cls = coef_class<ONLY_2D>(txtype), pt = plane > 0, txs_ctx = txs;
   const int lsh = txs == 3 ? 1 : (txs == 4 ? 2 : 0);
   const uint32_t dc_off = (uint32_t)(dcq * 109 / 256), off0 = (uint32_t)(acq * 98 / 256), off1 = (uint32_t)(acq * 109 / 256), off_eob = (uint32_t)(acq * 88 / 256);
   const uint32_t thr = (uint32_t)acq - off_eob, uq = (uint32_t)acq;
@@ -195,7 +245,7 @@
   for (int k = 0; k < IT; k++) {
     const int i = LANE + 64 * k;
     const bool valid = nc >= 64 || i < nc;
-    pos[k] = valid ? scan_pos(ls, n, cls, i) : 0;
+    pos[k] = valid ? scan_pos<ONLY_2D>(ls, n, cls, i) : 0;
     const int c = valid ? cbuf[pos[k]] : 0;
     mag[k] = (uint32_t)iabs_(c) << lsh; neg[k] = c < 0;
     if (valid && i >= 1 && mag[k] >= thr) last = i + 1;
@@ -252,33 +302,22 @@
     head += cc.eobx[((txs_ctx * 2 + pt) * 9 + (eob_pt - 3)) * CDF_EOB_EXTRA_STRIDE + hi];
     head += 512u * (uint32_t)(nb - 1);
   }
-  constexpr int area = nc;
-  int bits = 0, cul = 0, dcc = 0;
-#pragma unroll
-  for (int k = 0; k < IT; k++) {
-    const int c = LANE + 64 * k;
-    if (c < eob) {
-      const int pp = pos[k], row = pp >> bwl, col = pp & (n - 1), level = lvl[k];
-      const LDS uint8_t *L = lev + row * st + col;
-      if (c == eob - 1) {
-        const int ctx = c == 0 ? 0 : (c <= area / 8 ? 1 : (c <= area / 4 ? 2 : 3));
-        bits += cc.beob[((txs_ctx * 2 + pt) * 4 + ctx) * CDF_COEFF_BASE_EOB_STRIDE + imin_(level, 3) - 1];
-      } else {
-        const int ctx = base_ctx(L, st, cls, row, col);
-        bits += cc.base[((txs_ctx * 2 + pt) * 42 + ctx) * CDF_COEFF_BASE_STRIDE + imin_(level, 3)];
-      }
-      if (level > 2) {
-        const int ctx = br_ctx(L, st, cls, row, col, c);
-        const int off = ((imin_(txs_ctx, 3) * 2 + pt) * 21 + ctx) * CDF_COEFF_BR_STRIDE;
-        int rem = level - 3;
-        for (int idx = 0; idx < 4; idx++) { const int s2 = imin_(rem, 3); bits += cc.br[off + s2]; rem -= s2; if (s2 < 3) break; }
-      }
-      if (level) {
-        if (c == 0) { bits += cc.dcs[(pt * 3 + dc_ctx) * CDF_DC_SIGN_STRIDE + neg[k]]; dcc = neg[k] ? 1 : 2; }
-        else bits += 512;
-        if (level > 14) { const int len = 32 - __clz(level - 14); bits += 512 * (2 * len - 1); }
-      }
-      cul += level;
+  constexpr int area = nc, NB = IT < COEF_NB_BATCH ? IT : COEF_NB_BATCH;
+  int bits = 0, cul = 0, dcc = 0, lmax = 0;
+#pragma unroll
+  for (int k = 0; k < IT; k++) lmax = imax_(lmax, lvl[k]);
+  const bool with_br = coef_any(lmax > 2);
+#pragma unroll
+  for (int k0 = 0; k0 < IT; k0 += NB) {
+    if (k0 * 64 >= eob) break;
+    CoefNb nb[NB];
+#pragma unroll
+    for (int j = 0; j < NB; j++) { const int pp = pos[k0 + j]; nb[j] = coef_nb_load<ONLY_2D>(lev + (pp >> bwl) * st + (pp & (n - 1)), st, cls); }
+#pragma unroll
+    for (int j = 0; j < NB; j++) {
+      const int k = k0 + j, pp = pos[k];
+      bits += coef_sym_bits<ONLY_2D, 0>(cc.base, (int)(cc.beob - cc.base), cc.br, cc.dcs, nb[j], cls, pp >> bwl, pp & (n - 1), LANE + 64 * k, eob, lvl[k], neg[k], pt, txs_ctx, dc_ctx, area, with_br, &dcc);
+      cul += lvl[k];
     }
   }
   bits = wave_sum_i32(bits);
diff --git a/cavif_rs_amd/csrc/dev_rect.h b/cavif_rs_amd/csrc/dev_rect.h
--- a/cavif_rs_amd/csrc/dev_rect.h
+++ b/cavif_rs_amd/csrc/dev_rect.h
@@ -211,34 +211,12 @@
     const int nb = eob_pt - 2, rem = eob - ((1 << (eob_pt - 2)) + 1), hi = (rem >> (nb - 1)) & 1;
     head += cost[CDF_EOB_EXTRA + ((txs_ctx * 2 + pt) * 9 + (eob_pt - 3)) * CDF_EOB_EXTRA_STRIDE + hi] + 512u * (uint32_t)(nb - 1);
   }
-  uint32_t mine = 0;
-  if (valid && i < eob) {
-    const int row = pos >> wl, col = pos & (w - 1), level = lv;
-    const LDS uint8_t *L = lev + row * st + col;
-    if (i == eob - 1) {
-      const int ctx = i == 0 ? 0 : (i <= nc / 8 ? 1 : (i <= nc / 4 ? 2 : 3));
-      mine += cost[CDF_COEFF_BASE_EOB + ((txs_ctx * 2 + pt) * 4 + ctx) * CDF_COEFF_BASE_EOB_STRIDE + imin_(level, 3) - 1];
-    } else {
-      int ctx = base_ctx(L, st, cls, row, col);
-      if (cls == TXC_2D && !(row == 0 && col == 0)) {
-        int mg = imin_(L[1], 3) + imin_(L[st], 3) + imin_(L[st + 1], 3) + imin_(L[2], 3) + imin_(L[2 * st], 3);
-        const int m = imin_((mg + 1) >> 1, 4);
-        if (hl > wl) ctx = m + (row < 2 ? 11 : (row + col < 4 ? 6 : 21));
-        else ctx = m + (col < 2 ? 16 : (row + col < 4 ? 6 : 21));
-      }
-      mine += cost[CDF_COEFF_BASE + ((txs_ctx * 2 + pt) * 42 + ctx) * CDF_COEFF_BASE_STRIDE + imin_(level, 3)];
-    }
-    if (level > 2) {
-      const int off = CDF_COEFF_BR + ((txs_ctx * 2 + pt) * 21 + br_ctx(L, st, cls, row, col, i)) * CDF_COEFF_BR_STRIDE;
-      int rem = level - 3;
-      for (int idx = 0; idx < 4; idx++) { const int s = imin_(rem, 3); mine += cost[off + s]; rem -= s; if (s < 3) break; }
-    }
-    if (level) {
-      if (i == 0) mine += cost[CDF_DC_SIGN + (pt * 3 + dc_ctx) * CDF_DC_SIGN_STRIDE + neg];
-      else mine += 512u;
-      if (level > 14) { const uint32_t xg = (uint32_t)(level - 14); const int len = 32 - __clz(xg); mine += 512u * (uint32_t)(2 * len - 1); }
-    }
-  }
+  const int row = pos >> wl, col = pos & (w - 1);
+  int dcc_unused = 0;
+  const CoefNb nbv = coef_nb_load<false>(lev + row * st + col, st, cls);
+  const uint32_t mine = hl > wl
+    ? (uint32_t)coef_sym_bits<false, 1>(cost + CDF_COEFF_BASE, CDF_COEFF_BASE_EOB - CDF_COEFF_BASE, cost + CDF_COEFF_BR, cost + CDF_DC_SIGN, nbv, cls, row, col, i, eob, lv, neg, pt, txs_ctx, dc_ctx, nc, true, &dcc_unused)
+    : (uint32_t)coef_sym_bits<false, 2>(cost + CDF_COEFF_BASE, CDF_COEFF_BASE_EOB - CDF_COEFF_BASE, cost + CDF_COEFF_BR, cost + CDF_DC_SIGN, nbv, cls, row, col, i, eob, lv, neg, pt, txs_ctx, dc_ctx, nc, true, &dcc_unused);
   const int cul = imin_(wave_sum_i32((valid && i < eob) ? lv : 0), 63);
   const int dcneg = __builtin_amdgcn_readlane(neg, 0), dclv = __builtin_amdgcn_readlane(lv, 0);
   *cul_out = cul; *dc_cat = dclv ? (dcneg ? 1 : 2) : 0;
@@ -282,12 +260,13 @@
   return ((dist * f->wq[plane]) >> 5) + (((long long)tr->rate * f->rdmult + 256) >> 9);
 }
 
-template <int WL, int HL, typename CostPtr>
+template <int WL, int HL, bool ONLY_2D = false, typename CostPtr>
 __device__ inline void eval_group_wh(const CoefCost &cc, CostPtr cost, const LDS FrameDev *f, LDS GroupBuf8 *gb, const LDS uint16_t *src, const LDS uint16_t *pred, int plane, int txtype,
                                      int skip_ctx, int dc_ctx, int tx_off, int tx_sym, int psv_a, int psv_b, int psy_act, GroupRes *res) {
   constexpr int W = 1 << WL, H = 1 << HL, P = W + 1, nc = 32, IT = 2, st = W + 4, txs_ctx = 1;
   const int gl = GROUP_LANE, bd = f->bd;
-  const int cls = tx_class_of(txtype), pt = plane > 0;
+  GPH_BEGIN();
+  const int cls = coef_class<ONLY_2D>(txtype), pt = plane > 0;
   const uint32_t tx_cost = cost[tx_off >= 0 ? tx_off + tx_sym : 0];
   const uint32_t ep_cost = cost[eob_pt_cdf(1, pt, cls) + imin_(gl, 5)];
 #pragma unroll
@@ -318,6 +297,7 @@
     for (int c = 0; c < W; c++) gb->cbuf[gl * W + c] = (int32_t)(((long long)x[c] * 5793 + 2048) >> 12);
   }
   WAVE_SYNC();
+  GPH(16);
   const int dcq = f->dc_q[plane], acq = f->ac_q[plane];
   const uint32_t dc_recip = f->dc_recip[plane], ac_recip = f->ac_recip[plane];
   const uint32_t dc_off = (uint32_t)(dcq * 109 / 256), off0 = (uint32_t)(acq * 98 / 256), off1 = (uint32_t)(acq * 109 / 256), off_eob = (uint32_t)(acq * 88 / 256);
@@ -327,7 +307,7 @@
 #pragma unroll
   for (int k = 0; k < IT; k++) {
     const int i = gl + 16 * k;
-    pos[k] = rect_scan_pos(WL, HL, cls, i);
+    pos[k] = rect_scan_pos<ONLY_2D>(WL, HL, cls, i);
     const int c = gb->cbuf[pos[k]];
     mag[k] = (uint32_t)iabs_(c); neg[k] = c < 0;
     if (i >= 1 && mag[k] >= thr) last = i + 1;
@@ -366,8 +346,10 @@
     gb->cbuf[pp] = v < dmn ? dmn : (v > dmx ? dmx : v);
   }
   WAVE_SYNC();
+  GPH(17);
   uint32_t head = cc.txb[(txs_ctx * 13 + skip_ctx) * CDF_TXB_SKIP_STRIDE + (eob == 0)];
   int bits = 0, cul = 0, dcc = 0;
+  const bool live1 = coef_any(gl + 16 < eob), with_br = coef_any(imax_(lvl[0], lvl[1]) > 2);
   const int eob_pt = eob_to_pt(imax_(eob, 1));
   const uint32_t ep = (uint32_t)__shfl((int)ep_cost, (LANE & 48) + eob_pt - 1);
   if (eob > 0) {
@@ -378,41 +360,20 @@
       head += cc.eobx[((txs_ctx * 2 + pt) * 9 + (eob_pt - 3)) * CDF_EOB_EXTRA_STRIDE + hi];
       head += 512u * (uint32_t)(nb - 1);
     }
-#pragma unroll
-    for (int k = 0; k < IT; k++) {
-      const int c = gl + 16 * k;
-      if (c < eob) {
-        const int pp = pos[k], row = pp >> WL, col = pp & (W - 1), level = lvl[k];
-        const LDS uint8_t *L = gb->lev + row * st + col;
-        if (c == eob - 1) {
-          const int ctx = c == 0 ? 0 : (c <= nc / 8 ? 1 : (c <= nc / 4 ? 2 : 3));
-          bits += cc.beob[((txs_ctx * 2 + pt) * 4 + ctx) * CDF_COEFF_BASE_EOB_STRIDE + imin_(level, 3) - 1];
-        } else {
-          int ctx = base_ctx(L, st, cls, row, col);
-          if (cls == TXC_2D && !(row == 0 && col == 0)) {
-            const int mg = imin_(L[1], 3) + imin_(L[st], 3) + imin_(L[st + 1], 3) + imin_(L[2], 3) + imin_(L[2 * st], 3), m = imin_((mg + 1) >> 1, 4);
-            ctx = HL > WL ? m + (row < 2 ? 11 : (row + col < 4 ? 6 : 21)) : m + (col < 2 ? 16 : (row + col < 4 ? 6 : 21));
-          }
-          bits += cc.base[((txs_ctx * 2 + pt) * 42 + ctx) * CDF_COEFF_BASE_STRIDE + imin_(level, 3)];
-        }
-        if (level > 2) {
-          const int off = ((txs_ctx * 2 + pt) * 21 + br_ctx(L, st, cls, row, col, c)) * CDF_COEFF_BR_STRIDE;
-          int rem = level - 3;
-          for (int idx = 0; idx < 4; idx++) { const int s2 = imin_(rem, 3); bits += cc.br[off + s2]; rem -= s2; if (s2 < 3) break; }
-        }
-        if (level) {
-          if (c == 0) { bits += cc.dcs[(pt * 3 + dc_ctx) * CDF_DC_SIGN_STRIDE + neg[k]]; dcc = neg[k] ? 1 : 2; }
-          else bits += 512;
-          if (level > 14) { const int len = 32 - __clz(level - 14); bits += 512 * (2 * len - 1); }
-        }
-        cul += level;
-      }
+    CoefNb nb[IT];
+#pragma unroll
+    for (int k = 0; k < IT; k++) if (k == 0 || live1) nb[k] = coef_nb_load<ONLY_2D>(gb->lev + (pos[k] >> WL) * st + (pos[k] & (W - 1)), st, cls);
+#pragma unroll
+    for (int k = 0; k < IT; k++) if (k == 0 || live1) {
+      bits += coef_sym_bits<ONLY_2D, (HL > WL ? 1 : 2)>(cc.base, (int)(cc.beob - cc.base), cc.br, cc.dcs, nb[k], cls, pos[k] >> WL, pos[k] & (W - 1), gl + 16 * k, eob, lvl[k], neg[k], pt, txs_ctx, dc_ctx, nc, with_br, &dcc);
+      cul += lvl[k];
     }
   }
   bits = row_sum_i32(bits);
   cul = row_sum_i32(imin_(cul, 1 << 20));
   dcc = row_max_i32(dcc);
   res->eob = eob; res->cul = imin_(cul, 63); res->dcc = dcc; res->rate = head + (uint32_t)bits;
+  GPH(18);
   {
     const int cbits = imax_(bd + 6, 16), cmax = (1 << (cbits - 1)) - 1, cmin = -(1 << (cbits - 1));
     const bool act_r = gl < H && eob > 0, act_c = gl < W && eob > 0;
@@ -436,6 +397,7 @@
     }
     WAVE_SYNC();
   }
+  GPH(19);
   int se[2] = { 0, 0 }, sd[2] = { 0, 0 }, qd[2] = { 0, 0 };
 #pragma unroll
   for (int k = 0; k < IT; k++) {
@@ -450,6 +412,7 @@
       dist += psy_cell_dist((uint32_t)row_sum_i32(se[cell]), (uint32_t)row_sum_i32(sd[cell]), (uint32_t)row_sum_i32(qd[cell]), (uint32_t)(cell ? psv_b : psv_a), (uint32_t)psy_act, 4, bd);
     res->sse = dist;
   } else res->sse = (int)(((unsigned long long)(uint32_t)row_sum_i32(se[0] + se[1]) * (uint32_t)psy_act + 8192) >> 14);
+  GPH(20);
 }
 
 template <int WL, int HL> __device__ inline void commit_rect(const LDS FrameDev *f, int plane, int r, int c, const LDS uint16_t *rec, const LDS int32_t *qc, int eob, int cul, int dcc) {
@@ -551,7 +514,7 @@
       if (ntx > 1) txtype = sym_to_txtype(tx_set, ti);
       else { txtype = mode_to_txtype(m); if (tx_off < 0 || txtype_to_sym(tx_set, txtype) < 0) txtype = DCT_DCT; }
       GroupRes gr;
-      eval_group_wh<WL, HL>(k.cc(), k.cost(), f, &S->grp[g], SH->srcb[0], pcache + ci * NN, 0, txtype, sctx_y, dctx_y, tx_off, tx_off >= 0 ? txtype_to_sym(tx_set, txtype) : 0,
+      eval_group_wh<WL, HL, Tools<TS>::ONLY_2D>(k.cc(), k.cost(), f, &S->grp[g], SH->srcb[0], pcache + ci * NN, 0, txtype, sctx_y, dctx_y, tx_off, tx_off >= 0 ? txtype_to_sym(tx_set, txtype) : 0,
                             Tools<TS>::tune_psnr(f) ? -1 : psv_a, psv_b, act, &gr);
       long long j = rd_dist32(f, 0, gr.sse) + rd_rate32(f, gr.rate) + rd_rate32(f, mode_rate);
       if (!live) j = J_INF;
@@ -701,7 +664,7 @@
               else ssc = 6;
             }
             GroupRes gr;
-            eval_group<4>(k.cc(), k.cost(), k.ls(), f, &S->grp[g], SH->ssrc + q * 16, ppred, 0, 0, txtype, ssc, sdc, stx_off, tx_sym, Tools<TS>::tune_psnr(f) ? -1 : SH->psv4[q], SH->pact[0], &gr);
+            eval_group<4, Tools<TS>::ONLY_2D>(k.cc(), k.cost(), k.ls(), f, &S->grp[g], SH->ssrc + q * 16, ppred, 0, 0, txtype, ssc, sdc, stx_off, tx_sym, Tools<TS>::tune_psnr(f) ? -1 : SH->psv4[q], SH->pact[0], &gr);
             if (has_chain) jc += rd_dist32(f, 0, gr.sse) + rd_rate32(f, gr.rate);
             {
               const LDS uint16_t *srec = S->grp[g].rec; const LDS int32_t *sqc = S->grp[g].qc;
@@ -819,7 +782,7 @@
       const int um = cand == nc - 1 ? UV_CFL_PRED : (cand == 0 ? DC_PRED : best_mode);
       int txtype = mode_to_txtype(um);
       if (txtype_to_sym(uvset, txtype) < 0) txtype = DCT_DCT;
-      eval_group_wh<WL, HL>(k.cc(), k.cost(), f, &S->grp[g], SH->srcb[p], cand == 0 ? (const LDS uint16_t *)S->dcp : (const LDS uint16_t *)(S->pred + cand * NN), p, txtype,
+      eval_group_wh<WL, HL, Tools<TS>::ONLY_2D>(k.cc(), k.cost(), f, &S->grp[g], SH->srcb[p], cand == 0 ? (const LDS uint16_t *)S->dcp : (const LDS uint16_t *)(S->pred + cand * NN), p, txtype,
                             SH->sctx[p], SH->dctx[p], -1, 0, -1, 0, SH->cact, &gr);
       const long long jp = rd_dist32(f, p, gr.sse) + rd_rate32(f, gr.rate);
       if (GROUP_LANE == 0 && g < nc) SH->cj[g][p - 1] = jp;
@@ -923,7 +886,7 @@
       const int um = lut4(cand_pack, live ? ci : 0);
       int txtype = mode_to_txtype(um);
       if (txtype_to_sym(uvset, txtype) < 0) txtype = DCT_DCT;
-      if (dealt) eval_group_wh<WL, HL>(k.cc(), k.cost(), f, &S->grp[g], SH->srcb[p], um == DC_PRED ? (const LDS uint16_t *)S->dcp : (const LDS uint16_t *)(S->pred + g * NN), p, txtype,
+      if (dealt) eval_group_wh<WL, HL, Tools<TS>::ONLY_2D>(k.cc(), k.cost(), f, &S->grp[g], SH->srcb[p], um == DC_PRED ? (const LDS uint16_t *)S->dcp : (const LDS uint16_t *)(S->pred + g * NN), p, txtype,
                             SH->sctx[p], SH->dctx[p], -1, 0, -1, 0, SH->cact, &gr);
       const long long jp = rd_dist32(f, p, gr.sse) + rd_rate32(f, gr.rate);
       if (GROUP_LANE == 0 && live) SH->cj[ci][p - 1] = jp;
diff --git a/cavif_rs_amd/csrc/tile_search.h b/cavif_rs_amd/csrc/tile_search.h
--- a/cavif_rs_amd/csrc/tile_search.h
+++ b/cavif_rs_amd/csrc/tile_search.h
@@ -27,7 +27,7 @@
 #endif
 #if MI_PROFILE
 #define PH_BEGIN() unsigned long long ph_t_ = clock64()
-#define PH(i) do { const unsigned long long n_ = clock64(); if (LANE == 0 && !(MI_PROFILE == 3 && (i) >= 16 && (i) <= 21)) SH->prof[W][i] += n_ - ph_t_; ph_t_ = n_; } while (0)
+#define PH(i) do { const unsigned long long n_ = clock64(); if (LANE == 0 && !((MI_PROFILE == 3 || MI_PROFILE == 4) && (i) >= 16 && (i) <= 21)) SH->prof[W][i] += n_ - ph_t_; ph_t_ = n_; } while (0)
 #define PH_SIZE(slot, call) [&]() { const unsigned long long t0_ = clock64(); const long long r_ = (call); if (MI_PROFILE == 3 && LANE == 0) k.sh()->prof[WAVE_ID][16 + (slot)] += clock64() - t0_; return r_; }()
 #else
 #define PH_SIZE(slot, call) (call)
@@ -92,6 +92,9 @@
 #if MI_PROFILE
 extern __shared__ __align__(16) uint8_t mi_prof_smem_[];
 template <int N> __device__ __forceinline__ LDS unsigned long long &mi_prof_slot_n(int w, int i) { return ((LDS SharedScratch<N> *)mi_prof_smem_)->prof[w][i]; }
+#if MI_PROFILE == 4
+__device__ inline void mi_gprof_add(int slot, unsigned long long cycles) { if (LANE == 0) mi_prof_slot_n<MI_PROF_MAXN>(WAVE_ID, slot) += cycles; }
+#endif
 #endif
 
 template <int TS> struct Tools {
@@ -101,7 +104,11 @@
   template <typename F> static __device__ __forceinline__ bool fine_directional(F f) { return FIXED ? true : f->fine_directional != 0; }
   template <typename F> static __device__ __forceinline__ bool tx_mode_select(F f) { return FIXED ? true : f->tx_mode_select != 0; }
   template <typename F> static __device__ __forceinline__ bool tune_psnr(F f) { return FIXED ? false : f->tune_psnr != 0; }
+  static constexpr bool ONLY_2D = FIXED;
+  static_assert((tx_set_of(0, 1) | tx_set_of(1, 1) | tx_set_of(2, 1)) == 2 && (tx_set_of(3, 1) | tx_set_of(4, 1)) == 0, "Tools::ONLY_2D: the reduced sets are 2 and 0");
+  static_assert(txtypes_all_2d(TXSET2_TYPES, 5) && txtypes_all_2d(MODE_TXTYPES, 14) && DCT_DCT < V_DCT, "Tools::ONLY_2D: a 1-D transform type in the reduced set or in mode_to_txtype");
 };
+static_assert(!txtypes_all_2d(TXSET1_TYPES, 7), "txtypes_all_2d must see V_DCT / H_DCT of the full set");
 template <int MAXN, int NW, int TS_ = 0> struct Ctx {
   static constexpr int TS = TS_;
   static constexpr int MAXBS = MAXN == 16 ? 2 : 4;
@@ -275,7 +282,7 @@
   PH(16);
   fwd_txfm2d_dev<n>(S->tbuf, S->cbuf, txtype);
   PH(17);
-  const int eob = quant_rate_dev<CS>(k.cc(), k.cost(), k.ls(), S->cbuf, qc_out, S->lev, plane, BS, txtype, f->dc_q[plane], f->ac_q[plane], f->dc_recip[plane], f->ac_recip[plane],
+  const int eob = quant_rate_dev<CS, Tools<TS>::ONLY_2D>(k.cc(), k.cost(), k.ls(), S->cbuf, qc_out, S->lev, plane, BS, txtype, f->dc_q[plane], f->ac_q[plane], f->dc_recip[plane], f->ac_recip[plane],
                                      f->bd, sctx, dctx, tx_off, tx_sym, &tr->rate, &tr->cul, &tr->dcc);
   PH(19);
   if (eob > 0) inv_txfm2d_add_dev<n>(S->cbuf, S->tbuf, rec_out, txtype, f->bd);
@@ -483,7 +490,7 @@
         if (ntx > 1) txtype = sym_to_txtype(tx_set, ti);
         else { txtype = mode_to_txtype(m); if (tx_off < 0 || txtype_to_sym(tx_set, txtype) < 0) txtype = DCT_DCT; }
         GroupRes gr;
-        eval_group<n>(k.cc(), k.cost(), k.ls(), f, &S->grp[g], SH->srcb[0], SH->lpred + ci * nn, 0, BS, txtype, sctx_y, dctx_y, tx_off,
+        eval_group<n, Tools<TS>::ONLY_2D>(k.cc(), k.cost(), k.ls(), f, &S->grp[g], SH->srcb[0], SH->lpred + ci * nn, 0, BS, txtype, sctx_y, dctx_y, tx_off,
                       tx_off >= 0 ? txtype_to_sym(tx_set, txtype) : 0, Tools<TS>::tune_psnr(f) ? -1 : SH->psv[0], SH->pact[0], &gr);
         long long j = rd_dist32(f, 0, gr.sse) + rd_rate32(f, gr.rate) + rd_rate32(f, mode_rate);
         if (!live) j = J_INF;
@@ -713,7 +720,7 @@
               const int psv_q = hn == 4 ? (n == 8 ? SH->psv4[q] : psv16[q]) : SH->psv[bi * pcp + bj];
               const int pact_q = hn == 4 ? SH->pact[(bi >> 1) * pcp + (bj >> 1)] : SH->pact[bi * pcp + bj];
               GroupRes gr;
-              eval_group<hn>(k.cc(), k.cost(), k.ls(), f, &S->grp[g], ssrc + q * hnn, ppred, 0, SBS, txtype, ssc, sdc, stx_off, tx_sym, Tools<TS>::tune_psnr(f) ? -1 : psv_q, pact_q, &gr);
+              eval_group<hn, Tools<TS>::ONLY_2D>(k.cc(), k.cost(), k.ls(), f, &S->grp[g], ssrc + q * hnn, ppred, 0, SBS, txtype, ssc, sdc, stx_off, tx_sym, Tools<TS>::tune_psnr(f) ? -1 : psv_q, pact_q, &gr);
               {
                 const long long j = rd_dist32(f, 0, gr.sse) + rd_rate32(f, gr.rate);
                 long long jslot = j;
@@ -988,7 +995,7 @@
       const int um = cand == nc - 1 ? UV_CFL_PRED : (cand == 0 ? DC_PRED : best_mode);
       int txtype = mode_to_txtype(um);
       if (txtype_to_sym(uvset, txtype) < 0) txtype = DCT_DCT;
-      eval_group<n>(k.cc(), k.cost(), k.ls(), f, &S->grp[g], SH->srcb[p], cand == 0 ? (const LDS uint16_t *)S->dcp : (const LDS uint16_t *)(S->pred + cand * nn), p, BS, txtype, SH->sctx[p], SH->dctx[p], -1, 0, -1, SH->cact, &gr);
+      eval_group<n, Tools<TS>::ONLY_2D>(k.cc(), k.cost(), k.ls(), f, &S->grp[g], SH->srcb[p], cand == 0 ? (const LDS uint16_t *)S->dcp : (const LDS uint16_t *)(S->pred + cand * nn), p, BS, txtype, SH->sctx[p], SH->dctx[p], -1, 0, -1, SH->cact, &gr);
       const long long jp = rd_dist32(f, p, gr.sse) + rd_rate32(f, gr.rate);
       if (GROUP_LANE == 0 && g < nc) SH->cj[g][p - 1] = jp;
     }
@@ -1123,7 +1130,7 @@
       const int um = lut4(cand_pack, live ? ci : 0);
       int txtype = mode_to_txtype(um);
       if (txtype_to_sym(uvset, txtype) < 0) txtype = DCT_DCT;
-      if (dealt) eval_group<n>(k.cc(), k.cost(), k.ls(), f, &S->grp[g], SH->srcb[p], um == DC_PRED ? (const LDS uint16_t *)S->dcp : (const LDS uint16_t *)(S->pred + g * nn), p, BS, txtype,
+      if (dealt) eval_group<n, Tools<TS>::ONLY_2D>(k.cc(), k.cost(), k.ls(), f, &S->grp[g], SH->srcb[p], um == DC_PRED ? (const LDS uint16_t *)S->dcp : (const LDS uint16_t *)(S->pred + g * nn), p, BS, txtype,
                     SH->sctx[p], SH->dctx[p], -1, 0, -1, SH->cact, &gr);
       const long long jp = rd_dist32(f, p, gr.sse) + rd_rate32(f, gr.rate);
       if (GROUP_LANE == 0 && live) SH->cj[ci][p - 1] = jp;
```

Result: no change. 558.2 (-1.0%).
